# LukasHaas/PIGEON

Measured on AMD Instinct MI355X. Metric: images/sec end-to-end (ViT+head+refine), 4x336x336, higher is better.
Workload: dtype f16

## Files before the change

include/pigeon_hip.h:

```cpp
#ifndef PIGEON_HIP_H
#define PIGEON_HIP_H

#include <stddef.h>
#include <stdint.h>

#ifdef __cplusplus
extern "C" {
#endif

#define PG_OK            0
#define PG_EINVAL       -1
#define PG_ENOMEM       -2
#define PG_EHIP         -3
#define PG_ESTATE       -4

#define PG_DTYPE_F32     0
#define PG_DTYPE_BF16    1
#define PG_DTYPE_F16     2
#define PG_DTYPE_F64     3

#define PG_ABI_VERSION   7

const char* pg_last_error(void);
int pg_abi_version(void);
int pg_device_count(void);

typedef struct pg_vit pg_vit;

typedef struct pg_vit_cfg {
    int32_t layers;
    int32_t image_size;
    int32_t patch;
    int32_t hidden;
    int32_t heads;
    int32_t mlp;
    float   ln_eps;
    int32_t max_chunk;
    int32_t mma_dtype;
    int32_t precise;
} pg_vit_cfg;

int pg_vit_create(pg_vit** out, int device, const pg_vit_cfg* cfg);
int pg_vit_load_weight(pg_vit* h, const char* name, const void* data, int dtype,
                       const int64_t* shape, int ndim);
int pg_vit_finalize(pg_vit* h);
int pg_vit_workspace_bytes(const pg_vit* h, int n_images, size_t* bytes);
int pg_vit_forward(pg_vit* h, const void* pixels, int pix_dtype, int n_images, float* emb_out,
                   void* workspace, size_t workspace_bytes, void* stream);
int pg_vit_forward_hidden(pg_vit* h, const void* pixels, int pix_dtype, int n_images, float* emb_out,
                          float* hidden_out, void* workspace, size_t workspace_bytes, void* stream);
int pg_vit_precise_workspace_bytes(const pg_vit* h, int n_images, size_t* bytes);
int pg_vit_precise_plan(int n_images, int32_t out[8]);
int pg_vit_forward_precise(pg_vit* h, const void* pixels, int pix_dtype, int n_images, float* emb_out, float* hidden_out,
                           void* workspace, size_t workspace_bytes, void* stream);
int pg_vit_graph(pg_vit* h, int on, int64_t* replays, int64_t* captures);
int pg_vit_destroy(pg_vit* h);
int pg_vit_mma_dtype(const pg_vit* h);

int pg_fingerprint(const void* data, size_t bytes, uint64_t seed, uint64_t out[2], void* stream);
int pg_vit_fingerprint(const pg_vit* h, uint64_t out[2]);

#define PG_PROF_CLASSES 9
int pg_vit_profile_enable(pg_vit* h, int on);
int pg_vit_profile_read(pg_vit* h, int64_t* launches , double* ms );
int pg_vit_profile_reset(pg_vit* h);

int pg_tune_gemm_stagger(float fraction);
int pg_tune_gemm_tail_rows(int rows);
int pg_tune_gemm_tail_shape(int min_k, int min_n);
int pg_tune_gemm_raster(int gn);
int pg_tune_gemm_mid(int on);
int pg_gemm_plan(int variant, int epi, int M, int N, int K, int* kernel, int* rows_main, int* rest);
int pg_tune_exact_attention(int use_f32_mfma);
int pg_tune_exact_products(int n);
int pg_tune_exact_fusion(int on);
int pg_vit_saturation_check(pg_vit* h, int on);
int pg_vit_saturation_read(pg_vit* h, int64_t* count, int reset);
int pg_vit_range_alarm_read(pg_vit* h, int64_t* rows, int reset);

int pg_head_forward(const float* emb, int B, int P, const float* W, const float* bias,
                    const double* centroids, int C, int k, float* logits,
                    float* topk_val, int64_t* topk_idx, int64_t* argmax, double* pred_llh, void* stream);

int pg_head_margin(const float* logits, int B, int C, const float* emb, int P, const float* W, float* margin, float* sens,
                   int64_t* top2, void* stream);

int pg_head_certainty(const float* logits, int B, int C, const float* emb, int P, const float* W, const int64_t* topk_idx, int kx,
                      const float* beta, const float* wstats, float* tol, int32_t* code, float* margin, float* sens, void* stream);

int pg_aux_heads_forward(const float* emb, int B, int P, const float* W, const float* bias, int n_reg, int n_climate, int n_month,
                         const float* beta, float* preds, int64_t* cls, float* tol, int32_t* code, float* row_tol, void* stream);

typedef struct pg_bank {
    const float*   proto_emb;
    const int64_t* cell_off;
    const float*   proto_lnglat;
    const int32_t* proto_count;
    const int64_t* member_off;
    const int64_t* member_idx;
    const float*   train_emb;
    const float*   train_lnglat;
    int64_t num_cells;
    int64_t num_protos;
    int64_t num_train;
} pg_bank;

int pg_refine_forward(const pg_bank* bank, const float* q, int B, int P, const double* init_llh,
                      const int64_t* cand, const float* cand_prob, int k, int topk,
                      float temperature, double max_refine_km, float* scratch,
                      float* out_llh, int64_t* out_cell, int32_t* out_choice, void* stream);

int pg_refine_forward_ex(const pg_bank* bank, const float* q, int B, int P, const double* init_llh,
                         const int64_t* cand, const float* cand_prob, int k, int topk, int n_eval,
                         float temperature, double max_refine_km, float* scratch12,
                         float* out_llh, int64_t* out_cell, int32_t* out_choice, int32_t* out_refined, void* stream);

int pg_refine_certainty(const pg_bank* bank, const float* q, int B, int P, const int64_t* cand, const float* cand_prob, int k,
                        int topk, int n_eval, const float* scratch12, const float* W, int C, const float* beta,
                        const float* wstats, float temperature, const int32_t* refined, const int32_t* choice,
                        float* tol, int32_t* code, void* stream);

int pg_requeue_append(const float* head_tol, const float* refine_tol, const int32_t* refine_code, int B, float thr, int force_all,
                      int64_t dst_base, int64_t flushed, int64_t cap, int64_t* counters, int64_t* slot_dst, int32_t* row_slot,
                      uint8_t* certain, int32_t* cause, void* stream);
int pg_rows_to_slots(const void* src, int64_t row_bytes, const int32_t* row_slot, int B, void* dst, void* stream);
int pg_requeue_take(const int64_t* slot_dst, int64_t cap, int64_t head, int n_valid, int n_pad, int64_t* dst_out, void* stream);
int pg_scatter_rows(const void* src, int64_t row_bytes, const int64_t* dst_row, int n, void* dst, int64_t dst_rows,
                    int64_t remap_wb, int64_t remap_b, int64_t remap_off, void* stream);
int pg_head_wstats(const float* W, int C, const float* beta, float* out2, void* stream);

int pg_embedding_debias(float* emb, int64_t n, int dim, const float* bias, void* stream);

typedef struct pg_prep pg_prep;
int pg_prep_create(pg_prep** out, int device, int in_h, int in_w);
int pg_prep_destroy(pg_prep* h);
int pg_prep_geometry(const pg_prep* h, int32_t* out6);
int pg_prep_workspace_bytes(const pg_prep* h, int n_images, size_t* bytes);
int pg_prep_forward(pg_prep* h, const void* images_u8, int n_images, void* out, int out_dtype, void* workspace,
                    size_t workspace_bytes, void* stream);

#define PG_PREP_ITEM_BYTES 80
#define PG_PREP_RAGGED_MAX_IMAGES 65535
typedef struct pg_prep_item {
    uint64_t src_off;
    int32_t in_h, in_w;
    int32_t new_h, new_w, top, left;
    int32_t ksize_h, ksize_v;
    int32_t row0, nrows;
    int32_t tmp_row;
    uint32_t bounds_h_off, kk_h_off, bounds_v_off, kk_v_off;
    int32_t reserved[3];
} pg_prep_item;
int pg_prep_ragged_plan(int n, const int32_t* hw, pg_prep_item* items_out, size_t* packed_bytes, size_t* workspace_bytes);
typedef struct pg_prep_ragged pg_prep_ragged;
int pg_prep_ragged_create(pg_prep_ragged** out, int device);
int pg_prep_ragged_destroy(pg_prep_ragged* h);
int pg_prep_ragged_forward(pg_prep_ragged* h, const void* packed_dev, size_t packed_bytes, const pg_prep_item* items_host, int n,
                           void* out, int out_dtype, void* workspace, size_t workspace_bytes, void* stream);

#define PG_COMM_ID_BYTES 128
int pg_comm_unique_id(void* id_out );
int pg_comm_init_rank(void** comm, int nranks, const void* unique_id , int rank);
int pg_comm_count(void* comm, int* nranks);
int pg_allgather(void* comm, const void* send, void* recv, size_t bytes_per_rank, void* stream);
int pg_allgather_many(void* comm, int count, const void* const* send, void* const* recv, const size_t* bytes_per_rank,
                      void* stream);
int pg_comm_destroy(void* comm);
int pg_comm_rccl_version(void);

int pg_proto_build(const float* train_emb, int panels, int64_t num_train, const int64_t* member_off,
                   const int64_t* member_idx, int64_t num_protos, float* proto_emb, void* stream);
int pg_haversine_matrix(const void* x, int x_dtype, const double* y, int N, int M, double* out, void* stream);
int pg_haversine_pairs(const double* x, const void* y, int y_dtype, int64_t N, double* out, void* stream);
int pg_smooth_labels(const double* distances, int N, int M, double constant, double* out, void* stream);

int pg_haversine_blocks(const double* pts, const int64_t* cell_off, const int64_t* mat_off, int C, double zero_as, double* out,
                        void* stream);
int pg_optics_graph(const double* dist, const int64_t* cell_off, const int64_t* mat_off, int C, int min_samples, int64_t* ordering,
                    double* core, double* reach, int64_t* pred, void* stream);
int pg_optics_plan(int64_t n, int min_samples, int32_t out[4]);
int pg_tune_optics_lds_points(int max_points);

int pg_op_gemm16(int dtype, const void* A, int64_t lda, const void* W, const float* bias, void* out, int64_t ldc,
                 int M, int N, int K, int epi, float qscale, int qcols, const float* aux,
                 int variant, void* stream);
int pg_op_gemm16_ld(int dtype, const void* A, int64_t lda, const void* W, int64_t ldw, const float* bias, void* out,
                    int64_t ldc, int M, int N, int K, int epi, float qscale, int qcols, const float* aux,
                    int variant, void* stream);
int pg_op_rowstat_cast(const float* x, void* x16, int dtype, float* rowstat, int64_t rows, float eps, void* stream);
int pg_op_gemm16_resid_stat(int dtype, const void* A, int64_t lda, const void* W, int64_t ldw, const float* bias, float* X,
                            int64_t ldc, void* x16, int64_t ldx, float* statpart, int M, int N, int K, int variant, void* stream);
int pg_op_rowstat_finalize(const float* statpart, int slots, float* rowstat, int64_t rows, float eps, void* stream);
int pg_op_gemm16_ln(int dtype, const void* A, int64_t lda, const void* W, int64_t ldw, const float* bias, const float* colsum,
                    const float* rowstat, void* out, int64_t ldc, int M, int N, int K, int epi, float qscale, int qcols,
                    int variant, void* stream);
int pg_op_layernorm(const float* x, const float* gamma, const float* beta, void* y, int out_dtype,
                    int64_t rows, float eps, void* stream);
int pg_op_attention(int dtype, const void* qkv, void* out, int n_images, void* stream);
int pg_op_im2col(const void* pixels, int pix_dtype, void* out, int out_dtype, int n_images, void* stream);
int pg_op_token_mean(const float* x, float* out, int n_images, void* stream);
int pg_op_cast_f32(const float* x, void* y, int out_dtype, int64_t n, void* stream);
int pg_op_preln(float* x, const float* cls, const float* pos0, const float* gamma, const float* beta, int64_t rows, float eps,
                void* x16, int x16_dtype, float* rowstat, void* stream);
int pg_op_gemm16_parts(int dtype, const void* A, int64_t lda, const void* W, int64_t ldw, const float* bias, float* parts,
                       int M, int N, int Kp, int S, void* stream);
int pg_op_x3_split(const float* x, void* y3, int64_t rows, int cols, int gelu, void* stream);
int pg_op_x3_layernorm(const float* x, const float* gamma, const float* beta, void* y3, int64_t rows, float eps, void* stream);
int pg_op_attention_f32(const float* qkv, float* out, int n_images, void* stream);
int pg_op_attention_x3(const float* qkv, void* out3, int n_images, void* stream);
int pg_op_x3_im2col(const void* pixels, int pix_dtype, void* out3, int n_images, void* stream);
int pg_op_sum_parts(const float* parts, int S, int64_t part_elems, float* dst, int64_t n, int resid, void* stream);

#ifdef __cplusplus
}
#endif
#endif
```

pigeon_amd/_lib.py:

```python
from __future__ import annotations

import ctypes as C
import os

_HERE = os.path.dirname(os.path.abspath(__file__))
LIB_PATH = os.environ.get("PIGEON_HIP_LIB") or os.path.join(_HERE, "libpigeon_hip.so")

PG_DTYPE_F32, PG_DTYPE_BF16, PG_DTYPE_F16, PG_DTYPE_F64 = 0, 1, 2, 3
EPI_QKV, EPI_GELU, EPI_RESID, EPI_PATCH, EPI_F32, EPI_RESID_STAT, EPI_QKV_LN, EPI_GELU_LN, EPI_GELU_X3 = 0, 1, 2, 3, 4, 5, 6, 7, 8
PROF_CLASSES = ["gemm_qkv", "gemm_out", "gemm_fc1", "gemm_fc2", "gemm_patch", "attention", "layernorm",
                "im2col", "token_mean"]


class PigeonHipError(RuntimeError):
    pass


class VitCfg(C.Structure):
    _fields_ = [("layers", C.c_int32), ("image_size", C.c_int32), ("patch", C.c_int32), ("hidden", C.c_int32),
                ("heads", C.c_int32), ("mlp", C.c_int32), ("ln_eps", C.c_float), ("max_chunk", C.c_int32),
                ("mma_dtype", C.c_int32), ("precise", C.c_int32)]


class Bank(C.Structure):
    _fields_ = [("proto_emb", C.c_void_p), ("cell_off", C.c_void_p), ("proto_lnglat", C.c_void_p),
                ("proto_count", C.c_void_p), ("member_off", C.c_void_p), ("member_idx", C.c_void_p),
                ("train_emb", C.c_void_p), ("train_lnglat", C.c_void_p),
                ("num_cells", C.c_int64), ("num_protos", C.c_int64), ("num_train", C.c_int64)]


class PrepItem(C.Structure):
    _fields_ = [("src_off", C.c_uint64), ("in_h", C.c_int32), ("in_w", C.c_int32), ("new_h", C.c_int32), ("new_w", C.c_int32),
                ("top", C.c_int32), ("left", C.c_int32), ("ksize_h", C.c_int32), ("ksize_v", C.c_int32), ("row0", C.c_int32),
                ("nrows", C.c_int32), ("tmp_row", C.c_int32), ("bounds_h_off", C.c_uint32), ("kk_h_off", C.c_uint32),
                ("bounds_v_off", C.c_uint32), ("kk_v_off", C.c_uint32), ("reserved", C.c_int32 * 3)]


PREP_ITEM_BYTES = 80
assert C.sizeof(PrepItem) == PREP_ITEM_BYTES


_P, _I, _I64, _F, _D, _SZ = C.c_void_p, C.c_int, C.c_int64, C.c_float, C.c_double, C.c_size_t
SIGNATURES = {
    "pg_last_error": (C.c_char_p, []),
    "pg_abi_version": (_I, []),
    "pg_device_count": (_I, []),
    "pg_vit_create": (_I, [C.POINTER(_P), _I, C.POINTER(VitCfg)]),
    "pg_vit_load_weight": (_I, [_P, C.c_char_p, _P, _I, C.POINTER(_I64), _I]),
    "pg_vit_finalize": (_I, [_P]),
    "pg_vit_workspace_bytes": (_I, [_P, _I, C.POINTER(_SZ)]),
    "pg_vit_forward": (_I, [_P, _P, _I, _I, _P, _P, _SZ, _P]),
    "pg_vit_forward_hidden": (_I, [_P, _P, _I, _I, _P, _P, _P, _SZ, _P]),
    "pg_vit_precise_workspace_bytes": (_I, [_P, _I, C.POINTER(_SZ)]),
    "pg_vit_forward_precise": (_I, [_P, _P, _I, _I, _P, _P, _P, _SZ, _P]),
    "pg_vit_graph": (_I, [_P, _I, C.POINTER(_I64), C.POINTER(_I64)]),
    "pg_vit_destroy": (_I, [_P]),
    "pg_vit_mma_dtype": (_I, [_P]),
    "pg_fingerprint": (_I, [_P, _SZ, C.c_uint64, C.POINTER(C.c_uint64), _P]),
    "pg_vit_fingerprint": (_I, [_P, C.POINTER(C.c_uint64)]),
    "pg_vit_profile_enable": (_I, [_P, _I]),
    "pg_vit_profile_read": (_I, [_P, C.POINTER(_I64), C.POINTER(_D)]),
    "pg_vit_profile_reset": (_I, [_P]),
    "pg_tune_gemm_stagger": (_I, [_F]),
    "pg_tune_gemm_tail_rows": (_I, [_I]),
    "pg_tune_gemm_tail_shape": (_I, [_I, _I]),
    "pg_tune_gemm_raster": (_I, [_I]),
    "pg_tune_gemm_mid": (_I, [_I]),
    "pg_tune_exact_attention": (_I, [_I]),
    "pg_tune_exact_products": (_I, [_I]),
    "pg_tune_exact_fusion": (_I, [_I]),
    "pg_gemm_plan": (_I, [_I, _I, _I, _I, _I, _P, _P, _P]),
    "pg_vit_saturation_check": (_I, [_P, _I]),
    "pg_vit_saturation_read": (_I, [_P, C.POINTER(_I64), _I]),
    "pg_vit_range_alarm_read": (_I, [_P, C.POINTER(_I64), _I]),
    "pg_comm_unique_id": (_I, [_P]),
    "pg_comm_init_rank": (_I, [C.POINTER(_P), _I, _P, _I]),
    "pg_comm_count": (_I, [_P, C.POINTER(_I)]),
    "pg_allgather": (_I, [_P, _P, _P, _SZ, _P]),
    "pg_allgather_many": (_I, [_P, _I, C.POINTER(_P), C.POINTER(_P), C.POINTER(_SZ), _P]),
    "pg_comm_destroy": (_I, [_P]),
    "pg_comm_rccl_version": (_I, []),
    "pg_prep_create": (_I, [C.POINTER(_P), _I, _I, _I]),
    "pg_prep_destroy": (_I, [_P]),
    "pg_prep_geometry": (_I, [_P, C.POINTER(C.c_int32)]),
    "pg_prep_workspace_bytes": (_I, [_P, _I, C.POINTER(_SZ)]),
    "pg_prep_forward": (_I, [_P, _P, _I, _P, _I, _P, _SZ, _P]),
    "pg_prep_ragged_plan": (_I, [_I, C.POINTER(C.c_int32), C.POINTER(PrepItem), C.POINTER(_SZ), C.POINTER(_SZ)]),
    "pg_prep_ragged_create": (_I, [C.POINTER(_P), _I]),
    "pg_prep_ragged_destroy": (_I, [_P]),
    "pg_prep_ragged_forward": (_I, [_P, _P, _SZ, C.POINTER(PrepItem), _I, _P, _I, _P, _SZ, _P]),
    "pg_proto_build": (_I, [_P, _I, _I64, _P, _P, _I64, _P, _P]),
    "pg_haversine_matrix": (_I, [_P, _I, _P, _I, _I, _P, _P]),
    "pg_haversine_pairs": (_I, [_P, _P, _I, _I64, _P, _P]),
    "pg_smooth_labels": (_I, [_P, _I, _I, _D, _P, _P]),
    "pg_haversine_blocks": (_I, [_P, _P, _P, _I, _D, _P, _P]),
    "pg_optics_graph": (_I, [_P, _P, _P, _I, _I, _P, _P, _P, _P, _P]),
    "pg_optics_plan": (_I, [_I64, _I, C.POINTER(C.c_int32)]),
    "pg_tune_optics_lds_points": (_I, [_I]),
    "pg_head_forward": (_I, [_P, _I, _I, _P, _P, _P, _I, _I, _P, _P, _P, _P, _P, _P]),
    "pg_head_margin": (_I, [_P, _I, _I, _P, _I, _P, _P, _P, _P, _P]),
    "pg_head_certainty": (_I, [_P, _I, _I, _P, _I, _P, _P, _I, _P, _P, _P, _P, _P, _P, _P]),
    "pg_aux_heads_forward": (_I, [_P, _I, _I, _P, _P, _I, _I, _I, _P, _P, _P, _P, _P, _P, _P]),
    "pg_refine_forward": (_I, [C.POINTER(Bank), _P, _I, _I, _P, _P, _P, _I, _I, _F, _D, _P, _P, _P, _P, _P]),
    "pg_refine_forward_ex": (_I, [C.POINTER(Bank), _P, _I, _I, _P, _P, _P, _I, _I, _I, _F, _D, _P, _P, _P, _P, _P, _P]),
    "pg_refine_certainty": (_I, [C.POINTER(Bank), _P, _I, _I, _P, _P, _I, _I, _I, _P, _P, _I, _P, _P, _F, _P, _P, _P, _P, _P]),
    "pg_requeue_append": (_I, [_P, _P, _P, _I, _F, _I, _I64, _I64, _I64, _P, _P, _P, _P, _P, _P]),
    "pg_rows_to_slots": (_I, [_P, _I64, _P, _I, _P, _P]),
    "pg_requeue_take": (_I, [_P, _I64, _I64, _I, _I, _P, _P]),
    "pg_scatter_rows": (_I, [_P, _I64, _P, _I, _P, _I64, _I64, _I64, _I64, _P]),
    "pg_head_wstats": (_I, [_P, _I, _P, _P, _P]),
    "pg_embedding_debias": (_I, [_P, _I64, _I, _P, _P]),
    "pg_op_gemm16": (_I, [_I, _P, _I64, _P, _P, _P, _I64, _I, _I, _I, _I, _F, _I, _P, _I, _P]),
    "pg_op_gemm16_ld": (_I, [_I, _P, _I64, _P, _I64, _P, _P, _I64, _I, _I, _I, _I, _F, _I, _P, _I, _P]),
    "pg_op_rowstat_cast": (_I, [_P, _P, _I, _P, _I64, _F, _P]),
    "pg_op_gemm16_resid_stat": (_I, [_I, _P, _I64, _P, _I64, _P, _P, _I64, _P, _I64, _P, _I, _I, _I, _I, _P]),
    "pg_op_rowstat_finalize": (_I, [_P, _I, _P, _I64, _F, _P]),
    "pg_op_gemm16_ln": (_I, [_I, _P, _I64, _P, _I64, _P, _P, _P, _P, _I64, _I, _I, _I, _I, _F, _I, _I, _P]),
    "pg_op_layernorm": (_I, [_P, _P, _P, _P, _I, _I64, _F, _P]),
    "pg_op_attention": (_I, [_I, _P, _P, _I, _P]),
    "pg_op_im2col": (_I, [_P, _I, _P, _I, _I, _P]),
    "pg_op_token_mean": (_I, [_P, _P, _I, _P]),
    "pg_op_cast_f32": (_I, [_P, _P, _I, _I64, _P]),
    "pg_op_gemm16_parts": (_I, [_I, _P, _I64, _P, _I64, _P, _P, _I, _I, _I, _I, _P]),
    "pg_op_x3_split": (_I, [_P, _P, _I64, _I, _I, _P]),
    "pg_op_x3_layernorm": (_I, [_P, _P, _P, _P, _I64, _F, _P]),
    "pg_op_attention_f32": (_I, [_P, _P, _I, _P]),
    "pg_op_attention_x3": (_I, [_P, _P, _I, _P]),
    "pg_op_x3_im2col": (_I, [_P, _I, _P, _I, _P]),
    "pg_op_sum_parts": (_I, [_P, _I, _I64, _P, _I64, _I, _P]),
    "pg_op_preln": (_I, [_P, _P, _P, _P, _P, _I64, _F, _P, _I, _P, _P]),
    "pg_vit_precise_plan": (_I, [_I, C.POINTER(C.c_int32)]),
}

_lib = None


def load():
    global _lib
    if _lib is not None:
        return _lib
    if not os.path.exists(LIB_PATH):
        raise PigeonHipError(
            f"{LIB_PATH} not found: build it with `python -m pigeon_amd.build` (hipcc, gfx950). "
            "pigeon_amd has no CPU/PyTorch fallback for its hot path.")
    import torch
    lib = C.CDLL(LIB_PATH)
    for name, (res, args) in SIGNATURES.items():
        fn = getattr(lib, name)
        fn.restype = res
        fn.argtypes = args
    _lib = lib
    return lib


def check(rc: int, what: str = ""):
    if rc != 0:
        msg = load().pg_last_error()
        raise PigeonHipError(f"{what} failed (code {rc}): {msg.decode() if msg else ''}")


def require_gpu():
    lib = load()
    n = lib.pg_device_count()
    if n <= 0:
        raise PigeonHipError("pigeon_amd needs an AMD GPU (gfx950) visible to HIP; found none. "
                             "There is no CPU fallback for the hot path.")
    return n
```

pigeon_amd/csrc/abi.hip:

```cpp
#include "pigeon_internal.h"
#include <cstdarg>
#include <cstdio>

static thread_local char g_err[512] = "";

void pg_set_error(const char* fmt, ...) {
    va_list ap;
    va_start(ap, fmt);
    vsnprintf(g_err, sizeof(g_err), fmt, ap);
    va_end(ap);
}
int pg_check_launch(const char* what) {
    hipError_t e = hipGetLastError();
    if (e != hipSuccess) { pg_set_error("launch of %s failed: %s", what, hipGetErrorString(e)); return PG_EHIP; }
    return PG_OK;
}

extern "C" const char* pg_last_error(void) { return g_err; }
extern "C" int pg_abi_version(void) { return PG_ABI_VERSION; }
extern "C" int pg_device_count(void) {
    int n = 0;
    hipError_t e = hipGetDeviceCount(&n);
    if (e != hipSuccess) { pg_set_error("hipGetDeviceCount: %s", hipGetErrorString(e)); return PG_EHIP; }
    return n;
}

extern "C" int pg_op_gemm16(int dtype, const void* A, int64_t lda, const void* W, const float* bias, void* out, int64_t ldc,
                            int M, int N, int K, int epi, float qscale, int qcols, const float* aux, int variant,
                            void* stream) {
    if (!A || !W || !out) { pg_set_error("op_gemm16: null argument"); return PG_EINVAL; }
    return pg_gemm_launch(dtype, A, lda, W, K, bias, out, ldc, M, N, K, epi, qscale, qcols, aux, variant, (hipStream_t)stream);
}
extern "C" int pg_op_gemm16_ld(int dtype, const void* A, int64_t lda, const void* W, int64_t ldw, const float* bias, void* out,
                               int64_t ldc, int M, int N, int K, int epi, float qscale, int qcols, const float* aux,
                               int variant, void* stream) {
    if (!A || !W || !out) { pg_set_error("op_gemm16_ld: null argument"); return PG_EINVAL; }
    return pg_gemm_launch(dtype, A, lda, W, ldw, bias, out, ldc, M, N, K, epi, qscale, qcols, aux, variant, (hipStream_t)stream);
}
extern "C" int pg_op_rowstat_cast(const float* x, void* x16, int dtype, float* rowstat, int64_t rows, float eps, void* stream) {
    if (!x || !x16 || !rowstat) { pg_set_error("op_rowstat_cast: null argument"); return PG_EINVAL; }
    return pg_rowstat_cast_launch(x, x16, dtype, rowstat, rows, eps, (hipStream_t)stream);
}
extern "C" int pg_op_rowstat_finalize(const float* statpart, int slots, float* rowstat, int64_t rows, float eps, void* stream) {
    if (!statpart || !rowstat || slots <= 0) { pg_set_error("op_rowstat_finalize: bad argument"); return PG_EINVAL; }
    return pg_rowstat_finalize_launch(statpart, slots, rowstat, rows, eps, (hipStream_t)stream);
}
extern "C" int pg_op_gemm16_resid_stat(int dtype, const void* A, int64_t lda, const void* W, int64_t ldw, const float* bias, float* X,
                                       int64_t ldc, void* x16, int64_t ldx, float* statpart, int M, int N, int K, int variant,
                                       void* stream) {
    if (!A || !W || !X || !x16 || !statpart) { pg_set_error("op_gemm16_resid_stat: null argument"); return PG_EINVAL; }
    PgGemmExtra ex; ex.x16 = x16; ex.ldx = ldx; ex.statpart = statpart;
    return pg_gemm_launch(dtype, A, lda, W, ldw, bias, X, ldc, M, N, K, EPI_RESID_STAT, 1.f, 0, nullptr, variant ? variant : PG_GEMM_V_PP,
                          (hipStream_t)stream, &ex);
}
extern "C" int pg_op_gemm16_ln(int dtype, const void* A, int64_t lda, const void* W, int64_t ldw, const float* bias,
                               const float* colsum, const float* rowstat, void* out, int64_t ldc, int M, int N, int K, int epi,
                               float qscale, int qcols, int variant, void* stream) {
    if (!A || !W || !out || !colsum || !rowstat) { pg_set_error("op_gemm16_ln: null argument"); return PG_EINVAL; }
    if (epi != EPI_QKV_LN && epi != EPI_GELU_LN) { pg_set_error("op_gemm16_ln: epi must be 6 or 7"); return PG_EINVAL; }
    PgGemmExtra ex; ex.colsum = colsum; ex.rowstat = rowstat;
    return pg_gemm_launch(dtype, A, lda, W, ldw, bias, out, ldc, M, N, K, epi, qscale, qcols, nullptr, variant ? variant : PG_GEMM_V_PP,
                          (hipStream_t)stream, &ex);
}
extern "C" int pg_op_layernorm(const float* x, const float* gamma, const float* beta, void* y, int out_dtype,
                               int64_t rows, float eps, void* stream) {
    if (!x || !gamma || !beta || !y) { pg_set_error("op_layernorm: null argument"); return PG_EINVAL; }
    return pg_layernorm_launch(x, gamma, beta, y, out_dtype, rows, eps, (hipStream_t)stream);
}
extern "C" int pg_op_attention(int dtype, const void* qkv, void* out, int n_images, void* stream) {
    if (!qkv || !out) { pg_set_error("op_attention: null argument"); return PG_EINVAL; }
    return pg_attention_launch(dtype, qkv, out, n_images, (hipStream_t)stream);
}
extern "C" int pg_op_im2col(const void* pixels, int pix_dtype, void* out, int out_dtype, int n_images, void* stream) {
    if (!pixels || !out) { pg_set_error("op_im2col: null argument"); return PG_EINVAL; }
    return pg_im2col_launch(pixels, pix_dtype, out, out_dtype, n_images, (hipStream_t)stream);
}
extern "C" int pg_op_token_mean(const float* x, float* out, int n_images, void* stream) {
    if (!x || !out) { pg_set_error("op_token_mean: null argument"); return PG_EINVAL; }
    return pg_token_mean_launch(x, out, n_images, (hipStream_t)stream);
}
extern "C" int pg_op_cast_f32(const float* x, void* y, int out_dtype, int64_t n, void* stream) {
    if (!x || !y) { pg_set_error("op_cast_f32: null argument"); return PG_EINVAL; }
    return pg_cast_f32_launch(x, y, out_dtype, n, (hipStream_t)stream);
}

extern "C" int pg_op_gemm16_parts(int dtype, const void* A, int64_t lda, const void* W, int64_t ldw, const float* bias, float* parts,
                                  int M, int N, int Kp, int S, void* stream) {
    if (!A || !W || !parts) { pg_set_error("op_gemm16_parts: null argument"); return PG_EINVAL; }
    if (S < 1 || S > 8) { pg_set_error("op_gemm16_parts: 1 <= S <= 8"); return PG_EINVAL; }
    PgGemmExtra ex;
    ex.parts = S; ex.a_part = Kp; ex.w_part = Kp; ex.c_part = (int64_t)M * N;
    return pg_gemm_launch(dtype, A, lda, W, ldw, bias, parts, N, M, N, Kp, EPI_F32, 1.f, 0, nullptr, PG_GEMM_V_PP, (hipStream_t)stream, &ex);
}

extern "C" int pg_op_x3_split(const float* x, void* y3, int64_t rows, int cols, int gelu, void* stream) {
    if (!x || !y3) { pg_set_error("op_x3_split: null argument"); return PG_EINVAL; }
    return pg_x3_split_launch(x, y3, rows, cols, gelu, (hipStream_t)stream);
}
extern "C" int pg_op_x3_layernorm(const float* x, const float* gamma, const float* beta, void* y3, int64_t rows, float eps, void* stream) {
    if (!x || !gamma || !beta || !y3) { pg_set_error("op_x3_layernorm: null argument"); return PG_EINVAL; }
    return pg_x3_ln_launch(x, gamma, beta, y3, rows, eps, (hipStream_t)stream);
}
extern "C" int pg_op_attention_f32(const float* qkv, float* out, int n_images, void* stream) {
    if (!qkv || !out) { pg_set_error("op_attention_f32: null argument"); return PG_EINVAL; }
    return pg_attention_f32_launch(qkv, out, n_images, (hipStream_t)stream);
}
extern "C" int pg_op_x3_im2col(const void* pixels, int pix_dtype, void* out3, int n_images, void* stream) {
    if (!pixels || !out3 || n_images < 0) { pg_set_error("op_x3_im2col: bad argument"); return PG_EINVAL; }
    return pg_x3_im2col_launch(pixels, pix_dtype, out3, n_images, (hipStream_t)stream);
}
extern "C" int pg_op_sum_parts(const float* parts, int S, int64_t part_elems, float* dst, int64_t n, int resid, void* stream) {
    if (!parts || !dst) { pg_set_error("op_sum_parts: null argument"); return PG_EINVAL; }
    if (S < 1 || S > 8 || n < 0 || n > part_elems) { pg_set_error("op_sum_parts: 1 <= S <= 8, 0 <= n <= part_elems"); return PG_EINVAL; }
    return pg_sum_parts_launch(parts, S, part_elems, dst, n, resid, (hipStream_t)stream);
}
extern "C" int pg_op_preln(float* x, const float* cls, const float* pos0, const float* gamma, const float* beta, int64_t rows, float eps,
                           void* x16, int x16_dtype, float* rowstat, void* stream) {
    if (!x || !cls || !pos0 || !gamma || !beta) { pg_set_error("op_preln: null argument"); return PG_EINVAL; }
    if ((x16 == nullptr) != (rowstat == nullptr)) { pg_set_error("op_preln: x16 and rowstat go together"); return PG_EINVAL; }
    return pg_preln_launch(x, cls, pos0, gamma, beta, rows, eps, (hipStream_t)stream, x16, x16_dtype, rowstat);
}
extern "C" int pg_op_attention_x3(const float* qkv, void* out3, int n_images, void* stream) {
    if (!qkv || !out3) { pg_set_error("op_attention_x3: null argument"); return PG_EINVAL; }
    return pg_attention_x3out_launch(qkv, out3, n_images, (hipStream_t)stream);
}
```

pigeon_amd/csrc/gemm_device.h:

```cpp
#pragma once
#include "common.h"
#include "pigeon_internal.h"

#define BK 64
#define ROWB 128

struct GemmArgs {
    const uint16_t* A; int64_t lda;
    const uint16_t* W; int64_t ldw;
    const float* bias;
    void* out; int64_t ldc;
    int M, N, K;
    float qscale; int qcols;
    const float* aux;
    int tilesM, tilesN, ntiles;
    int part_tiles;
    int gn;
    int stagger;
    int xcd_stagger_ticks;
    PgGemmExtra ex;
};

int pg_gemm_one_tile_bn(int variant);
int pg_gemm_one_tile_launch(int dtype, GemmArgs g, int epi, int variant, hipStream_t s);
int pg_gemm_pp_launch(int dtype, GemmArgs g, int epi, int variant, hipStream_t s);
bool pg_gemm_pp6_supported(int epi, int N, int K);
int pg_gemm_pp6_launch(int dtype, GemmArgs g, int epi, hipStream_t s);
bool pg_gemm_tail_supported(int epi, int N, int K);
int pg_gemm_tail_launch(int dtype, GemmArgs g, int epi, int m_begin, hipStream_t s);
bool pg_gemm_mid_supported(int epi, int N, int K);
int pg_gemm_mid_launch(int dtype, GemmArgs g, int epi, hipStream_t s, int m_begin = 0);

constexpr bool epi_is_ln(int epi) { return epi == EPI_QKV_LN || epi == EPI_GELU_LN; }
constexpr bool epi_is_qkv(int epi) { return epi == EPI_QKV || epi == EPI_QKV_LN; }
constexpr bool epi_is_out16(int epi) { return epi == EPI_QKV || epi == EPI_GELU || epi_is_ln(epi); }
constexpr bool epi_is_resid(int epi) { return epi == EPI_RESID || epi == EPI_RESID_STAT; }

__device__ __forceinline__ void xcd_stagger_wait(int ticks) {
    if (ticks <= 0) return;
    const int xcd = blockIdx.x & 7;
    if (xcd == 0) return;
    const unsigned long long until = __builtin_amdgcn_s_memrealtime() + (unsigned long long)ticks * xcd / 8;
    while (__builtin_amdgcn_s_memrealtime() < until) __builtin_amdgcn_s_sleep(16);
}

#ifdef PIGEON_PROBES
#define PG_TS(g, iter, wave, slot)                                                                                             \
    do {                                                                                                                       \
        if ((g).stagger == -7 && (blockIdx.x == 0 || blockIdx.x == 100) && (threadIdx.x & 63) == 0 && (iter) < 16)             \
            ((unsigned long long*)(g).aux)[(((blockIdx.x ? 1 : 0) * 16 + (iter)) * 8 + (wave)) * 12 + (slot)] =                \
                __builtin_amdgcn_s_memrealtime();                                                                              \
    } while (0)
#else
#define PG_TS(g, iter, wave, slot) do {} while (0)
#endif

typedef __attribute__((address_space(3))) void lds_void;

__device__ __forceinline__ void glds16(const void* gptr, void* lds_base_uniform) {
    __builtin_amdgcn_global_load_lds((const __attribute__((address_space(1))) void*)gptr,
                                     (__attribute__((address_space(3))) void*)lds_base_uniform, 16, 0, 0);
}
__device__ __forceinline__ __amdgpu_buffer_rsrc_t make_rsrc(const void* base, uint32_t bytes) {
    return __builtin_amdgcn_make_buffer_rsrc(const_cast<void*>(base), (short)0, (int)bytes, 0x00020000);
}
__device__ __forceinline__ void dma16(__amdgpu_buffer_rsrc_t rsrc, char* lds_wave_uniform, int voff, int soff) {
    __builtin_amdgcn_raw_ptr_buffer_load_lds(rsrc, (lds_void*)lds_wave_uniform, 16, voff, soff, 0, 0);
}
__device__ __forceinline__ int wave_valid_rows(int left, int cap) {
    int rv = left; rv = rv < 0 ? 0 : (rv > cap ? cap : rv);
    rv = __builtin_amdgcn_readfirstlane(rv);
    return rv;
}

template <int OFF, typename V>
__device__ __forceinline__ void lds_read_b128(V& dst, uint32_t addr) {
    asm volatile("ds_read_b128 %0, %1 offset:%2" : "=v"(dst) : "v"(addr), "n"(OFF));
}

__device__ __forceinline__ void wait_lgkm0() {
    asm volatile("s_waitcnt lgkmcnt(0)" ::: "memory");
    __builtin_amdgcn_sched_barrier(0);
}
__device__ __forceinline__ void wait_vm0() {
    asm volatile("s_waitcnt vmcnt(0)" ::: "memory");
    __builtin_amdgcn_sched_barrier(0);
}
__device__ __forceinline__ void raw_barrier() {
    __builtin_amdgcn_sched_barrier(0);
    __builtin_amdgcn_s_barrier();
    __builtin_amdgcn_sched_barrier(0);
}
__device__ __forceinline__ void wave_lds_fence() {
    asm volatile("s_waitcnt lgkmcnt(0)" ::: "memory");
    __builtin_amdgcn_wave_barrier();
}

template <typename KFN>
static int launch_kernel(KFN kfn, bool& attr_set, size_t lds, dim3 grid, dim3 block, const GemmArgs& g, hipStream_t s,
                         const char* name, const char* attr_what) {
    if (!attr_set) {
        hipError_t e = hipFuncSetAttribute((const void*)kfn, hipFuncAttributeMaxDynamicSharedMemorySize, (int)lds);
        if (e != hipSuccess) { pg_set_error("%s: %s", attr_what, hipGetErrorString(e)); return PG_EHIP; }
        attr_set = true;
    }
    hipLaunchKernelGGL(kfn, grid, block, lds, s, g);
    return pg_check_launch(name);
}
static inline int pg_gemm_panel_check(const char* kernel, int64_t lda, int64_t ldw, int bm, int bn) {
    if ((int64_t)lda * 2 * bm >= (1ll << 31) || (int64_t)ldw * 2 * bn >= (1ll << 31)) {
        pg_set_error("%s: operand panel exceeds the 2 GB buffer-descriptor range", kernel);
        return PG_EINVAL;
    }
    return PG_OK;
}
```

pigeon_amd/csrc/gemm_plan.hip:

```cpp
#include "common.h"
#include "pigeon_internal.h"

#include "gemm_epi.h"

#include <cmath>
#include <cstdlib>
#include <type_traits>

#ifndef PG_DEFAULT_GEMM_STAGGER
#define PG_DEFAULT_GEMM_STAGGER 0.0f
#endif
#define PG_DEFAULT_GEMM_TAIL_ROWS 768
#define PG_DEFAULT_GEMM_TAIL_MIN_K 2048
#define PG_DEFAULT_GEMM_TAIL_MIN_N 4096
#ifndef PG_DEFAULT_GEMM_RESID6
#define PG_DEFAULT_GEMM_RESID6 1
#endif
#define PG_ROUTE_MAX_ROWS 40000
#ifndef PG_EXACT_MID_US_KT
#define PG_EXACT_MID_US_KT 0.6
#endif

static unsigned long long g_tune_epoch = 1;
unsigned long long pg_tune_epoch() { return g_tune_epoch; }

template <typename T>
static T env_knob(const char* name, T dflt) {
    const char* e = getenv(name);
    if (!e) return dflt;
    if constexpr (std::is_integral<T>::value) return (T)atoi(e);
    else if constexpr (std::is_floating_point<T>::value) return (T)atof(e);
    else return e;
}

int pg_default_gemm_variant() {
    static int v = -1;
    if (v < 0) {
        v = env_knob("PIGEON_GEMM_VARIANT", (int)PG_GEMM_V_PP6);
        if (v <= 0) v = PG_GEMM_V_PP6;
    }
    return v;
}
static int block_cap() {
    static int v = -1;
    if (v < 0) { v = env_knob("PIGEON_GEMM_BLOCKS", 0); if (v < 0) v = 0; }
    return v;
}
static int route_max_rows() {
    static int v = -1;
    if (v < 0) { v = env_knob("PIGEON_GEMM_ROUTE_MAX_ROWS", PG_ROUTE_MAX_ROWS); if (v < 0) v = 0; }
    return v;
}
static bool resid6_enabled(int K) {
    static int mask = -1;
    if (mask < 0) { mask = env_knob("PIGEON_GEMM_RESID6", PG_DEFAULT_GEMM_RESID6); if (mask < 0) mask = 0; }
    return (mask & (K >= 2048 ? 1 : 2)) != 0;
}
static double precise_mid_us_kt() {
    static double v = -1.0;
    if (v < 0.0) { v = env_knob("PIGEON_EXACT_MID_US", PG_EXACT_MID_US_KT); if (!(v > 0.0)) v = PG_EXACT_MID_US_KT; }
    return v;
}

static int g_raster_gn = -2;
int pg_gemm_raster_gn() {
    if (g_raster_gn == -2) { g_raster_gn = env_knob("PIGEON_GEMM_RASTER_GN", 0); if (g_raster_gn < -1) g_raster_gn = 0; }
    return g_raster_gn;
}
extern "C" int pg_tune_gemm_raster(int gn) {
    if (gn < -1 || gn > 64) { pg_set_error("tune_gemm_raster: gn must be -1 (all N tiles), 0 (default) or 1..64"); return PG_EINVAL; }
    g_raster_gn = gn; ++g_tune_epoch;
    return PG_OK;
}

static int g_tail_rows = -1, g_tail_min_k = -1, g_tail_min_n = -1;
static int env_count(const char* name, int dflt) { const int v = env_knob(name, dflt); return v < 0 ? 0 : v; }
static int tail_rows() { if (g_tail_rows < 0) g_tail_rows = env_count("PIGEON_GEMM_TAIL_ROWS", PG_DEFAULT_GEMM_TAIL_ROWS); return g_tail_rows; }
static int tail_min_k() { if (g_tail_min_k < 0) g_tail_min_k = env_count("PIGEON_GEMM_TAIL_MIN_K", PG_DEFAULT_GEMM_TAIL_MIN_K); return g_tail_min_k; }
static int tail_min_n() { if (g_tail_min_n < 0) g_tail_min_n = env_count("PIGEON_GEMM_TAIL_MIN_N", PG_DEFAULT_GEMM_TAIL_MIN_N); return g_tail_min_n; }
extern "C" int pg_tune_gemm_tail_rows(int rows) {
    if (rows < 0 || rows > (1 << 20)) { pg_set_error("tune_gemm_tail_rows: rows must be in [0, 2^20]"); return PG_EINVAL; }
    g_tail_rows = rows; ++g_tune_epoch;
    return PG_OK;
}
extern "C" int pg_tune_gemm_tail_shape(int min_k, int min_n) {
    if (min_k < 0 || min_n < 0) { pg_set_error("tune_gemm_tail_shape: negative threshold"); return PG_EINVAL; }
    g_tail_min_k = min_k; g_tail_min_n = min_n; ++g_tune_epoch;
    return PG_OK;
}

static int g_gemm_mid = -1;
static bool mid_on() {
    if (g_gemm_mid < 0) { const char* e = env_knob<const char*>("PIGEON_GEMM_MID", "1"); g_gemm_mid = e[0] == '0' ? 0 : (e[0] == '2' ? 2 : 1); }
    return g_gemm_mid != 0;
}
static bool route_pp256() { return mid_on() && g_gemm_mid != 2; }
extern "C" int pg_tune_gemm_mid(int on) {
    g_gemm_mid = on == 2 ? 2 : (on ? 1 : 0); ++g_tune_epoch;
    return PG_OK;
}

static float g_stagger = -1.f;
static float stagger_fraction() {
    if (g_stagger < 0.f) {
        g_stagger = env_knob("PIGEON_GEMM_STAGGER", PG_DEFAULT_GEMM_STAGGER);
        if (!(g_stagger >= 0.f && g_stagger <= 4.f)) g_stagger = 0.f;
    }
    return g_stagger;
}
extern "C" int pg_tune_gemm_stagger(float fraction) {
    if (!(fraction >= 0.f && fraction <= 4.f)) { pg_set_error("tune_gemm_stagger: fraction must be in [0, 4]"); return PG_EINVAL; }
    g_stagger = fraction; ++g_tune_epoch;
    return PG_OK;
}

static int num_cus() {
    static int n = 0;
    if (n == 0) {
        int dev = 0;
        hipDeviceProp_t p;
        if (hipGetDevice(&dev) == hipSuccess && hipGetDeviceProperties(&p, dev) == hipSuccess) n = p.multiProcessorCount;
        if (n <= 0) n = 256;
    }
    return n;
}
int pg_gemm_grid_cus() {
    const int ncu = num_cus(), cap = block_cap();
    return cap > 0 && cap < ncu ? cap : ncu;
}


struct PersistentFit { double ci, cf, e1_resid, e1_gelu, e1_other, e2; };
constexpr PersistentFit SMALL_PP6 = {1.6, 3.0, 7.0, 9.0, 6.0, 3.0};
constexpr PersistentFit SMALL_PP = {1.1, 1.8, 12.0, 9.0, 7.0, 6.0};
constexpr double SMALL_MID_US_KT = 0.44;
constexpr double SMALL_MID_EPI_RESID = 8.0, SMALL_MID_EPI = 5.5;
constexpr double SMALL_PP_MARGIN = 0.90;

static double gemm_model_us(int kernel, int M, int N, int K, int epi, int ncu) {
    const bool resid = epi == EPI_RESID || epi == EPI_RESID_STAT;
    const bool gelu = epi == EPI_GELU || epi == EPI_GELU_LN;
    const double kt = K / 64;
    if (kernel == PG_GK_MID) {
        const int64_t tiles = (int64_t)((M + 127) / 128) * (N / 128);
        return (double)((tiles + ncu - 1) / ncu) * (kt * SMALL_MID_US_KT + (resid ? SMALL_MID_EPI_RESID : SMALL_MID_EPI));
    }
    const PersistentFit& c = kernel == PG_GK_PP6 ? SMALL_PP6 : SMALL_PP;
    const int bm = kernel == PG_GK_PP6 ? 384 : 256;
    const double e1 = resid ? c.e1_resid : (gelu ? c.e1_gelu : c.e1_other);
    const int64_t tiles = (int64_t)((M + bm - 1) / bm) * (N / 256);
    const int64_t full = tiles / ncu;
    const double f = (double)(tiles % ncu) / (double)ncu;
    double t = 0.0;
    if (full > 0) t += kt * c.cf + e1 + (double)(full - 1) * (kt * c.cf + c.e2);
    if (f > 0.0) t += kt * (c.ci + (c.cf - c.ci) * f * f) + (full > 0 ? c.e2 : e1);
    return t;
}

constexpr double TAIL_US = 36.0;
constexpr double ROUND_US_KT_PP6 = 1.75, ROUND_US_KT_PP = 1.25;
constexpr double ROUND_EPI_PP6_RESID = 14.0, ROUND_EPI_PP6 = 9.0;
constexpr double ROUND_EPI_PP_RESID = 20.0, ROUND_EPI_PP = 8.0;
constexpr double TAIL_MID_EPI_RESID = 6.0, TAIL_MID_EPI = 5.0, TAIL_MID_LAUNCH_US = 3.0;

constexpr float STAGGER_PP6_EPI = 8.f, STAGGER_PP6_EPI_GELU = 12.f, STAGGER_PP6_US_KT = 2.44f;
constexpr float STAGGER_PP_EPI = 10.f, STAGGER_PP_EPI_RESID = 25.f, STAGGER_PP_US_KT = 1.63f;
constexpr float TICKS_PER_US = 100.f;

constexpr double EXACT_US_KT = 1.7;
constexpr double EXACT_EPI_RESID_WHOLE = 25.0, EXACT_EPI = 12.0;
constexpr double EXACT_SUM_LAUNCH_US = 4.0, EXACT_SUM_BYTES_PER_US = 4.0e6;
constexpr double EXACT_MID_EPI_RESID = 6.0, EXACT_MID_EPI = 5.0;

static int precise_parts(int M, int N, int Ktot, bool resid, const int* cand, int ncand, double* best_us_out) {
    const double ncu = (double)num_cus();
    const double tiles = (double)((M + 255) / 256) * (N / 256);
    int best = 1; double best_us = 1e30;
    for (int i = 0; i < ncand; ++i) {
        const int S = cand[i];
        if (Ktot % S || (Ktot / S) % 128) continue;
        const double rounds = ceil(S * tiles / ncu);
        const double epi = (S == 1 && resid) ? EXACT_EPI_RESID_WHOLE : EXACT_EPI;
        double us = rounds * ((Ktot / S / 64) * EXACT_US_KT + epi);
        if (S > 1) us += EXACT_SUM_LAUNCH_US + (double)(S + (resid ? 2 : 1)) * M * N * 4.0 / EXACT_SUM_BYTES_PER_US;
        if (us < best_us) { best_us = us; best = S; }
    }
    if (best_us_out) *best_us_out = best_us;
    return best;
}
int pg_gemm_precise_route(int M, int N, int Ktot, bool resid, const int* cand, int ncand) {
    double parts_us = 0.0;
    const int S = precise_parts(M, N, Ktot, resid, cand, ncand, &parts_us);
    if (mid_on() && N % 128 == 0) {
        const double rounds_m = ceil((double)((M + 127) / 128) * (N / 128) / (double)num_cus());
        const double mid_us = rounds_m * ((Ktot / 64) * precise_mid_us_kt() + (resid ? EXACT_MID_EPI_RESID : EXACT_MID_EPI));
        if (mid_us < parts_us) return 0;
    }
    return S;
}

struct GemmPlan {
    int kernel;
    int variant;
    int rows;
    int rest;
    int stagger_ticks;
};

static bool is_pp_variant(int v) { return v == 33 || v == PG_GEMM_V_PP; }
static bool use_pp6(int variant, int epi, int N, int K) {
    return variant == PG_GEMM_V_PP6 && pg_gemm_pp6_supported(epi, N, K) && (epi != EPI_RESID_STAT || resid6_enabled(K));
}

static int small_batch_route(int own, int epi, int M, int N, int K) {
    if (!(mid_on() && M <= route_max_rows() && epi != EPI_PATCH && epi >= EPI_QKV && epi <= EPI_GELU_LN)) return own;
    const int ncu = pg_gemm_grid_cus();
    const double t_own = gemm_model_us(own, M, N, K, epi, ncu);
    const double t_pp = (own == PG_GK_PP6 && route_pp256()) ? gemm_model_us(PG_GK_PP, M, N, K, epi, ncu) : 1e30;
    const double t_mid = pg_gemm_mid_supported(epi, N, K) ? gemm_model_us(PG_GK_MID, M, N, K, epi, ncu) : 1e30;
    if (t_pp < SMALL_PP_MARGIN * t_own && t_pp < SMALL_PP_MARGIN * t_mid) return PG_GK_PP;
    return t_mid < t_own ? PG_GK_MID : own;
}

static bool tail_split(int own, int epi, int M, int N, int K, GemmPlan& p) {
    const int tail_max = tail_rows();
    if (tail_max <= 0) return false;
    const bool six = own == PG_GK_PP6;
    const int bm = six ? 384 : 256;
    const int ncu = pg_gemm_grid_cus();
    const int tilesN = N / 256;
    const int64_t ntiles = (int64_t)((M + bm - 1) / bm) * tilesN;
    const int64_t rounds = ntiles / ncu;
    if (rounds < 1 || ntiles % ncu == 0) return false;
    const int64_t m_main = (rounds * ncu / tilesN) * bm;
    if (!(m_main > 0 && m_main < M && M - m_main <= tail_max)) return false;
    const bool resid = epi == EPI_RESID || epi == EPI_RESID_STAT;
    const double kt = K / 64;
    const double t_round = six ? kt * ROUND_US_KT_PP6 + (resid ? ROUND_EPI_PP6_RESID : ROUND_EPI_PP6)
                               : kt * ROUND_US_KT_PP + (resid ? ROUND_EPI_PP_RESID : ROUND_EPI_PP);
    const int64_t tiles_m = (int64_t)((M - m_main + 127) / 128) * (N / 128);
    const double t_mid = (double)((tiles_m + ncu - 1) / ncu) * (kt * SMALL_MID_US_KT + (resid ? TAIL_MID_EPI_RESID : TAIL_MID_EPI)) + TAIL_MID_LAUNCH_US;
    const bool cut = K >= tail_min_k() || N >= tail_min_n();
    const bool by_mid = cut && mid_on() && pg_gemm_mid_supported(epi, N, K) && t_mid < TAIL_US && t_mid < t_round;
    const bool by_tail = cut && !by_mid && pg_gemm_tail_supported(epi, N, K);
    if (!by_mid && !by_tail) return false;
    p.rows = (int)m_main;
    p.rest = by_mid ? PG_GK_MID : PG_GK_TAIL;
    return true;
}

static int stagger_ticks(bool six, int epi, int M, int K) {
    const float f = stagger_fraction();
    if (!(f > 0.f && M >= 256 * 64)) return 0;
    const float period_us = six ? ((epi == EPI_GELU || epi == EPI_GELU_LN ? STAGGER_PP6_EPI_GELU : STAGGER_PP6_EPI) + STAGGER_PP6_US_KT * (K / 64))
                                : ((epi == EPI_RESID || epi == EPI_RESID_STAT ? STAGGER_PP_EPI_RESID : STAGGER_PP_EPI) + STAGGER_PP_US_KT * (K / 64));
    return (int)(f * period_us * TICKS_PER_US);
}

static int gemm_plan(int variant, int epi, int M, int N, int K, GemmPlan& p) {
    if (epi < EPI_QKV || epi > EPI_GELU_X3) { pg_set_error("gemm: bad epilogue %d", epi); return PG_EINVAL; }
    if (variant == 0) variant = pg_default_gemm_variant();
    const bool six = use_pp6(variant, epi, N, K);
    const bool pp = !six && (variant == PG_GEMM_V_PP6 || is_pp_variant(variant)) && N % 256 == 0 && K % 128 == 0;
    const int own = six ? PG_GK_PP6 : PG_GK_PP;
    const int pp_variant = variant == PG_GEMM_V_PP6 ? PG_GEMM_V_PP : variant;
    p = GemmPlan{own, pp_variant, M, PG_GK_NONE, stagger_ticks(six, epi, M, K)};
    if (variant == PG_GEMM_V_MID || variant == PG_GEMM_V_TAIL) {
        const bool mid = variant == PG_GEMM_V_MID;
        if (!(mid ? pg_gemm_mid_supported(epi, N, K) : pg_gemm_tail_supported(epi, N, K))) {
            pg_set_error("gemm: variant %d (%s) does not support epi=%d N=%d K=%d", variant, mid ? "gemm_mid" : "gemm_tail", epi, N, K);
            return PG_EINVAL;
        }
        p.kernel = mid ? PG_GK_MID : PG_GK_TAIL;
        return PG_OK;
    }
    if (six || pp) {
        const int kind = small_batch_route(own, epi, M, N, K);
        if (kind != own) {
            p.kernel = kind;
            p.variant = PG_GEMM_V_PP;
            return PG_OK;
        }
        tail_split(own, epi, M, N, K, p);
        return PG_OK;
    }
    if (epi >= EPI_RESID_STAT) { pg_set_error("gemm: epilogue %d exists only in the persistent kernels (variants 33, 36, 56, N %% 256 == 0, K %% 128 == 0)", epi); return PG_EINVAL; }
    p.kernel = PG_GK_ONE_TILE;
    p.variant = (variant == PG_GEMM_V_PP6 || is_pp_variant(variant)) ? PG_GEMM_V_ONE_TILE : variant;
    const int bn = pg_gemm_one_tile_bn(p.variant);
    if (bn == 0) {
        pg_set_error("gemm: variant %d does not exist (variants: 8, 33, 36, 56, 70, 71)", p.variant);
        return PG_EINVAL;
    }
    if (N % bn != 0 || K % BK != 0) { pg_set_error("gemm: N %% %d or K %% 64 != 0 (N=%d K=%d)", bn, N, K); return PG_EINVAL; }
    return PG_OK;
}

extern "C" int pg_gemm_plan(int variant, int epi, int M, int N, int K, int* kernel, int* rows_main, int* rest) {
    if (!kernel || !rows_main || !rest || M <= 0 || N <= 0 || K <= 0) { pg_set_error("gemm_plan: bad argument"); return PG_EINVAL; }
    GemmPlan p;
    const int rc = gemm_plan(variant, epi, M, N, K, p);
    if (rc != PG_OK) return rc;
    *kernel = p.kernel; *rows_main = p.rows; *rest = p.rest;
    return PG_OK;
}

#ifdef PIGEON_PROBES
static void* g_dbg_ts = nullptr;
extern "C" int pg_dbg_timestamps(void* buf) { g_dbg_ts = buf; return PG_OK; }
#endif

static int launch_one(int kernel, int variant, int dtype, const GemmArgs& g, int epi, int m_begin, hipStream_t s) {
    switch (kernel) {
        case PG_GK_PP6: return pg_gemm_pp6_launch(dtype, g, epi, s);
        case PG_GK_PP: return pg_gemm_pp_launch(dtype, g, epi, variant, s);
        case PG_GK_MID: return pg_gemm_mid_launch(dtype, g, epi, s, m_begin);
        case PG_GK_TAIL: return pg_gemm_tail_launch(dtype, g, epi, m_begin, s);
        default: return pg_gemm_one_tile_launch(dtype, g, epi, variant, s);
    }
}

int pg_gemm_launch(int dtype, const void* A, int64_t lda, const void* W, int64_t ldw, const float* bias, void* out, int64_t ldc,
                   int M, int N, int K, int epi, float qscale, int qcols, const float* aux, int variant,
                   hipStream_t s, const PgGemmExtra* extra) {
    if (M <= 0) return PG_OK;
    GemmArgs g;
    g.A = (const uint16_t*)A; g.lda = lda; g.W = (const uint16_t*)W; g.ldw = ldw > 0 ? ldw : K; g.bias = bias; g.out = out; g.ldc = ldc;
    g.M = M; g.N = N; g.K = K; g.qscale = qscale; g.qcols = qcols; g.aux = aux;
    g.tilesM = 0; g.tilesN = 0; g.ntiles = 0; g.part_tiles = 0; g.gn = 0; g.stagger = 0; g.xcd_stagger_ticks = 0;
    if (extra) g.ex = *extra;
    if (g.ex.parts > 1) {
        if (epi != EPI_F32 || N % 256 != 0 || K % 128 != 0) { pg_set_error("gemm: parts > 1 needs EPI_F32, N %% 256 == 0, K %% 128 == 0"); return PG_EINVAL; }
        return pg_gemm_pp_launch(dtype, g, epi, PG_GEMM_V_PP, s);
    }
    if ((epi == EPI_GELU || epi == EPI_RESID || epi >= EPI_RESID_STAT) && !bias) { pg_set_error("gemm: epilogue %d needs a bias", epi); return PG_EINVAL; }
    if (epi == EPI_RESID_STAT && (!g.ex.x16 || !g.ex.statpart || g.ex.ldx != ldc)) { pg_set_error("gemm: EPI_RESID_STAT needs x16 / statpart and ldx == ldc"); return PG_EINVAL; }
    if (epi_is_ln(epi) && (!g.ex.colsum || !g.ex.rowstat)) { pg_set_error("gemm: LN epilogue needs colsum / rowstat"); return PG_EINVAL; }
    if (epi == EPI_PATCH && !aux) { pg_set_error("gemm: patch epilogue needs aux"); return PG_EINVAL; }
    if (epi == EPI_GELU_X3 && (ldc != 3 * (int64_t)N || dtype != PG_DTYPE_F16 || N % 256 != 0 || K % 128 != 0)) {
        pg_set_error("gemm: EPI_GELU_X3 writes the fp16 triple [M][3N]: ldc == 3 N, fp16 operands, N %% 256 == 0, K %% 128 == 0 (ldc=%lld N=%d K=%d)",
                     (long long)ldc, N, K);
        return PG_EINVAL;
    }
    if ((lda % 8) || (ldc % 8) || (qcols % 8) || (g.ldw % 8) || g.ldw < K) { pg_set_error("gemm: lda/ldw/ldc/qcols must be multiples of 8, ldw >= K"); return PG_EINVAL; }
    GemmPlan p;
    const int rc = gemm_plan(variant, epi, M, N, K, p);
    if (rc != PG_OK) return rc;
    g.xcd_stagger_ticks = p.stagger_ticks;
    if (g.ex.stat_rows <= 0) g.ex.stat_rows = M;
#ifdef PIGEON_PROBES
    if (g_dbg_ts && epi != EPI_PATCH) { g.aux = (const float*)g_dbg_ts; g.stagger = -7; }
#endif
    GemmArgs gm = g;
    gm.M = p.rows;
    const int rc_main = launch_one(p.kernel, p.variant, dtype, gm, epi, 0, s);
    if (rc_main != PG_OK || p.rest == PG_GK_NONE) return rc_main;
    return launch_one(p.rest, 0, dtype, g, epi, p.rows, s);
}
```

pigeon_amd/csrc/gemm_tail.hip:

```cpp
#include "gemm_epi.h"

namespace {

constexpr int TL_BM = 32, TL_BN = 64;
constexpr int TL_DEPTH = 8;

template <typename T> struct FragTL { typename T::v8 a[2], b[4]; };

template <typename T>
__device__ __forceinline__ void load_frag_tl(FragTL<T>& f, __amdgpu_buffer_rsrc_t ra, __amdgpu_buffer_rsrc_t rw,
                                             const int (&va)[2], const int (&vw)[4], int kbytes) {
#pragma unroll
    for (int i = 0; i < 2; ++i) f.a[i] = __builtin_bit_cast(typename T::v8, __builtin_amdgcn_raw_buffer_load_b128(ra, va[i], kbytes, 0));
#pragma unroll
    for (int j = 0; j < 4; ++j) f.b[j] = __builtin_bit_cast(typename T::v8, __builtin_amdgcn_raw_buffer_load_b128(rw, vw[j], kbytes, 0));
}

template <typename T, int EPI>
__global__ __launch_bounds__(64) void gemm_tail_kernel(GemmArgs g, int m_begin) {
    __shared__ __attribute__((aligned(16))) float slab[TL_BM * EPI_SLAB_ROWPF];
    const int lane = threadIdx.x;
    int tn, tm;
    if (g.tilesN % 8 == 0) {
        const int xcd = blockIdx.x & 7, idx = blockIdx.x >> 3, per = g.tilesN >> 3;
        tn = xcd + 8 * (idx % per); tm = idx / per;
    } else {
        tn = blockIdx.x % g.tilesN; tm = blockIdx.x / g.tilesN;
    }
    const int row0 = m_begin + tm * TL_BM, col0 = tn * TL_BN;
    const int l15 = lane & 15, lq = lane >> 4;
    const int rows = min(TL_BM, g.M - row0);
    const __amdgpu_buffer_rsrc_t ra = make_rsrc(g.A + (int64_t)row0 * g.lda, (uint32_t)rows * (uint32_t)g.lda * 2u);
    const __amdgpu_buffer_rsrc_t rw = make_rsrc(g.W + (int64_t)col0 * g.ldw, (uint32_t)TL_BN * (uint32_t)g.ldw * 2u);
    int va[2], vw[4];
#pragma unroll
    for (int i = 0; i < 2; ++i) va[i] = (i * 16 + l15) * (int)g.lda * 2 + lq * 16;
#pragma unroll
    for (int j = 0; j < 4; ++j) vw[j] = (j * 16 + l15) * (int)g.ldw * 2 + lq * 16;

    const int nks = g.K / 32;
    FragTL<T> fr[TL_DEPTH];
#pragma unroll
    for (int d = 0; d < TL_DEPTH; ++d) {
        load_frag_tl<T>(fr[d], ra, rw, va, vw, d * 64);
        __builtin_amdgcn_sched_barrier(0);
    }
    f32x4 acc[2][4];
#pragma unroll
    for (int i = 0; i < 2; ++i)
#pragma unroll
        for (int j = 0; j < 4; ++j) acc[i][j] = f32x4{0.f, 0.f, 0.f, 0.f};
    for (int ks = 0; ks < nks; ks += TL_DEPTH) {
#pragma unroll
        for (int d = 0; d < TL_DEPTH; ++d) {
#pragma unroll
            for (int i = 0; i < 2; ++i)
#pragma unroll
                for (int j = 0; j < 4; ++j) acc[i][j] = T::mfma16(fr[d].b[j], fr[d].a[i], acc[i][j]);
            const int kn = min(ks + d + TL_DEPTH, nks - 1);
            load_frag_tl<T>(fr[d], ra, rw, va, vw, kn * 64);
            __builtin_amdgcn_sched_barrier(0);
        }
    }

    constexpr bool OUT16 = epi_is_out16(EPI);
    constexpr bool LN = epi_is_ln(EPI);
    constexpr bool STAT = (EPI == EPI_RESID_STAT);
    constexpr bool RESID = epi_is_resid(EPI);
#pragma unroll
    for (int ib = 0; ib < 2; ++ib)
#pragma unroll
        for (int j = 0; j < 4; ++j) *(f32x4*)(slab + (ib * 16 + l15) * EPI_SLAB_ROWPF + j * 16 + 4 * lq) = acc[ib][j];
    wave_lds_fence();

    constexpr int HOFF = STAT ? 32 : 4;
    const int rr = lane >> 3, cc = STAT ? (lane & 7) * 4 : (lane & 7) * 8;
    const int col = col0 + cc;
    const f32x4 zero4 = {0.f, 0.f, 0.f, 0.f};
    f32x4 b_lo = zero4, b_hi = zero4, s_lo = zero4, s_hi = zero4;
    if (g.bias) { b_lo = *(const f32x4*)(g.bias + col); b_hi = *(const f32x4*)(g.bias + col + HOFF); }
    if constexpr (LN) { s_lo = *(const f32x4*)(g.ex.colsum + col); s_hi = *(const f32x4*)(g.ex.colsum + col + 4); }
    const float qsc = (epi_is_qkv(EPI) && col < g.qcols) ? g.qscale : 1.f;

#pragma unroll
    for (int it = 0; it < 4; ++it) {
        const int r = it * 8 + rr;
        const int row = row0 + r;
        if (row >= g.M) continue;
        f32x4 lo = *(const f32x4*)(slab + r * EPI_SLAB_ROWPF + cc);
        f32x4 hi = *(const f32x4*)(slab + r * EPI_SLAB_ROWPF + cc + HOFF);
        if constexpr (OUT16) {
            float rstd = 0.f, mrs = 0.f;
            if constexpr (LN) {
                const u32x2 rs = *(const u32x2*)(g.ex.rowstat + (int64_t)row * 2);
                asm("v_mov_b32 %0, %1" : "=v"(rstd) : "v"(rs[0]));
                asm("v_mov_b32 %0, %1" : "=v"(mrs) : "v"(rs[1]));
            }
            *(u32x4*)((uint16_t*)g.out + (int64_t)row * g.ldc + col) =
                epi16_finish<T, EPI>(lo, hi, b_lo, b_hi, s_lo, s_hi, rstd, mrs, col0 < g.qcols, qsc);
        } else if constexpr (RESID) {
            float* p = (float*)g.out + (int64_t)row * g.ldc + col;
            const f32x4 x = epi_resid4(*(const f32x4*)p, lo, b_lo);
            const f32x4 y = epi_resid4(*(const f32x4*)(p + HOFF), hi, b_hi);
            *(f32x4*)p = x;
            *(f32x4*)(p + HOFF) = y;
            if constexpr (STAT) {
                uint16_t* p16 = (uint16_t*)g.ex.x16 + (int64_t)row * g.ldc + col;
                *(u32x2*)p16 = epi_copy16x4<T>(x);
                *(u32x2*)(p16 + HOFF) = epi_copy16x4<T>(y);
                float s1, s2;
                epi_stat8(x, y, s1, s2);
                s1 = row8_sum(s1);
                s2 = row8_sum(s2);
                if ((lane & 7) == 0) {
                    float* sp = g.ex.statpart + ((int64_t)(col0 / 64) * g.ex.stat_rows + row) * 2;
                    sp[0] = s1; sp[1] = s2;
                }
            }
        } else {
            float* p = (float*)g.out + (int64_t)row * g.ldc + col;
            *(f32x4*)p = lo + b_lo;
            *(f32x4*)(p + 4) = hi + b_hi;
        }
    }
}

template <typename T, int EPI>
int launch_tail(const GemmArgs& g, int m_begin, int nblk, hipStream_t s) {
    hipLaunchKernelGGL((gemm_tail_kernel<T, EPI>), dim3(nblk), dim3(64), 0, s, g, m_begin);
    return pg_check_launch("gemm_tail");
}

template <typename T>
int dispatch_tail(const GemmArgs& g, int epi, int m_begin, int nblk, hipStream_t s) {
    switch (epi) {
        case EPI_QKV: return launch_tail<T, EPI_QKV>(g, m_begin, nblk, s);
        case EPI_GELU: return launch_tail<T, EPI_GELU>(g, m_begin, nblk, s);
        case EPI_RESID: return launch_tail<T, EPI_RESID>(g, m_begin, nblk, s);
        case EPI_F32: return launch_tail<T, EPI_F32>(g, m_begin, nblk, s);
        case EPI_RESID_STAT: return launch_tail<T, EPI_RESID_STAT>(g, m_begin, nblk, s);
        case EPI_QKV_LN: return launch_tail<T, EPI_QKV_LN>(g, m_begin, nblk, s);
        case EPI_GELU_LN: return launch_tail<T, EPI_GELU_LN>(g, m_begin, nblk, s);
        default: pg_set_error("gemm_tail: epilogue %d not supported", epi); return PG_EINVAL;
    }
}

}

bool pg_gemm_tail_supported(int epi, int N, int K) {
    return epi != EPI_PATCH && epi >= EPI_QKV && epi <= EPI_GELU_LN && N % TL_BN == 0 && K % (32 * TL_DEPTH) == 0;
}

int pg_gemm_tail_launch(int dtype, GemmArgs g, int epi, int m_begin, hipStream_t s) {
    if (!pg_gemm_tail_supported(epi, g.N, g.K)) { pg_set_error("gemm_tail: unsupported epilogue / shape (epi=%d N=%d K=%d)", epi, g.N, g.K); return PG_EINVAL; }
    if (m_begin < 0 || m_begin >= g.M) return PG_OK;
    if (int rc = pg_gemm_panel_check("gemm_tail", g.lda, g.ldw, TL_BM, TL_BN)) return rc;
    g.tilesM = (g.M - m_begin + TL_BM - 1) / TL_BM;
    g.tilesN = g.N / TL_BN;
    g.ntiles = g.tilesM * g.tilesN;
    if (dtype == PG_DTYPE_F16) return dispatch_tail<T_F16>(g, epi, m_begin, g.ntiles, s);
    if (dtype == PG_DTYPE_BF16) return dispatch_tail<T_BF16>(g, epi, m_begin, g.ntiles, s);
    pg_set_error("gemm_tail: operand dtype must be PG_DTYPE_F16 or PG_DTYPE_BF16 (got %d)", dtype);
    return PG_EINVAL;
}
```

pigeon_amd/csrc/pigeon_internal.h:

```cpp
#pragma once
#include <hip/hip_runtime.h>
#include <stdint.h>
#include "../../include/pigeon_hip.h"

enum { EPI_QKV = 0, EPI_GELU = 1, EPI_RESID = 2, EPI_PATCH = 3, EPI_F32 = 4, EPI_RESID_STAT = 5, EPI_QKV_LN = 6, EPI_GELU_LN = 7,
       EPI_GELU_X3 = 8 };

struct PgGemmExtra {
    const float* colsum = nullptr;
    const float* rowstat = nullptr;
    void* x16 = nullptr;
    int64_t ldx = 0;
    float* statpart = nullptr;
    int64_t stat_rows = 0;
    int parts = 1;
    int64_t a_part = 0, w_part = 0, c_part = 0;
};

void pg_set_error(const char* fmt, ...) __attribute__((format(printf, 1, 2)));
int pg_check_launch(const char* what);
int pg_default_gemm_variant();
int pg_gemm_grid_cus();
int pg_gemm_raster_gn();
unsigned long long pg_tune_epoch();
int pg_gemm_precise_route(int M, int N, int Ktot, bool resid, const int* cand, int ncand);

enum { PG_GEMM_V_ONE_TILE = 8, PG_GEMM_V_PP = 36, PG_GEMM_V_PP6 = 56, PG_GEMM_V_TAIL = 70, PG_GEMM_V_MID = 71 };
enum PgGemmKernel { PG_GK_NONE = -1, PG_GK_PP6 = 0, PG_GK_PP = 1, PG_GK_MID = 2, PG_GK_TAIL = 3, PG_GK_ONE_TILE = 4 };

#define PG_HIP(call)                                                                          \
    do {                                                                                      \
        hipError_t e__ = (call);                                                              \
        if (e__ != hipSuccess) {                                                              \
            pg_set_error("%s failed: %s (%s:%d)", #call, hipGetErrorString(e__), __FILE__, __LINE__); \
            return PG_EHIP;                                                                   \
        }                                                                                     \
    } while (0)

struct PgFpBuf { const void* data; size_t bytes; uint64_t seed; };
int pg_fingerprint_many(const PgFpBuf* bufs, int n, uint64_t* out, hipStream_t stream);
void pg_fingerprint_host(const void* data, size_t bytes, uint64_t seed, uint64_t out[2]);

int pg_gemm_launch(int dtype, const void* A, int64_t lda, const void* W, int64_t ldw, const float* bias, void* out, int64_t ldc,
                   int M, int N, int K, int epi, float qscale, int qcols, const float* aux, int variant,
                   hipStream_t s, const PgGemmExtra* extra = nullptr);
int pg_layernorm_launch(const float* x, const float* gamma, const float* beta, void* y, int out_dtype,
                        int64_t rows, float eps, hipStream_t s);
int pg_preln_launch(float* x, const float* cls, const float* pos0, const float* gamma, const float* beta,
                    int64_t rows, float eps, hipStream_t s, void* x16 = nullptr, int x16_dtype = 0, float* rowstat = nullptr);
int pg_im2col_launch(const void* pixels, int pix_dtype, void* out, int out_dtype, int n_images, hipStream_t s);
int pg_token_mean_launch(const float* x, float* out, int n_images, hipStream_t s);
int pg_cast_f32_launch(const float* x, void* y, int out_dtype, int64_t n, hipStream_t s);
int pg_rowstat_cast_launch(const float* x, void* x16, int out_dtype, float* rowstat, int64_t rows, float eps, hipStream_t s);
int pg_rowstat_finalize_launch(const float* statpart, int slots, float* rowstat, int64_t rows, float eps, hipStream_t s,
                               unsigned long long* alarm = nullptr, float alarm_sumsq = 0.f);
int pg_count_sat16_launch(const void* buf, int64_t rows, int cols, int64_t ld, int dtype, unsigned long long* counter, hipStream_t s);
int pg_attention_launch(int dtype, const void* qkv, void* out, int n_images, hipStream_t s);
int pg_x3_ln_launch(const float* x, const float* gamma, const float* beta, void* y3, int64_t rows, float eps, hipStream_t s);
int pg_x3_split_launch(const float* x, void* y3, int64_t rows, int C, int gelu, hipStream_t s);
int pg_x3_im2col_launch(const void* pixels, int pix_dtype, void* out3, int n_images, hipStream_t s);
int pg_attention_f32_launch(const float* qkv, float* out, int n_images, hipStream_t s);
bool pg_attention_x3out_available();
int pg_attention_x3out_launch(const float* qkv, void* out3, int n_images, hipStream_t s);
int pg_sum_parts_launch(const float* parts, int S, int64_t part_elems, float* dst, int64_t n, int resid, hipStream_t s);
```

pigeon_amd/csrc/rowops.hip:

```cpp
#include "common.h"
#include "pigeon_internal.h"

template <int OUT>
__global__ __launch_bounds__(256) void layernorm_kernel(const float* __restrict__ x, const float* __restrict__ gamma,
                                                        const float* __restrict__ beta, void* __restrict__ y,
                                                        int64_t rows, float eps) {
    const int lane = threadIdx.x & 63;
    const int64_t row = (int64_t)blockIdx.x * 4 + (threadIdx.x >> 6);
    if (row >= rows) return;
    const float* xr = x + row * VIT_HIDDEN;
    f32x4 v[4];
#pragma unroll
    for (int i = 0; i < 4; ++i) v[i] = *(const f32x4*)(xr + i * 256 + lane * 4);
    float s = 0.f;
#pragma unroll
    for (int i = 0; i < 4; ++i) s += (v[i][0] + v[i][1]) + (v[i][2] + v[i][3]);
    const float mean = wave_sum(s) * (1.0f / VIT_HIDDEN);
    float q = 0.f;
#pragma unroll
    for (int i = 0; i < 4; ++i)
#pragma unroll
        for (int e = 0; e < 4; ++e) { const float d = v[i][e] - mean; q += d * d; }
    const float var = wave_sum(q) * (1.0f / VIT_HIDDEN);
    const float rstd = 1.0f / sqrtf(var + eps);
#pragma unroll
    for (int i = 0; i < 4; ++i) {
        const int c = i * 256 + lane * 4;
        const f32x4 g4 = *(const f32x4*)(gamma + c);
        const f32x4 b4 = *(const f32x4*)(beta + c);
        f32x4 o;
#pragma unroll
        for (int e = 0; e < 4; ++e) o[e] = (v[i][e] - mean) * rstd * g4[e] + b4[e];
        if (OUT != 0) {
            u32x2 pk;
            if (OUT == 1) { pk[0] = pack16x2<T_BF16>(o[0], o[1]); pk[1] = pack16x2<T_BF16>(o[2], o[3]); }
            else { pk[0] = pack16x2<T_F16>(o[0], o[1]); pk[1] = pack16x2<T_F16>(o[2], o[3]); }
            *(u32x2*)((uint16_t*)y + row * VIT_HIDDEN + c) = pk;
        } else {
            *(f32x4*)((float*)y + row * VIT_HIDDEN + c) = o;
        }
    }
}

int pg_layernorm_launch(const float* x, const float* gamma, const float* beta, void* y, int out_dtype,
                        int64_t rows, float eps, hipStream_t s) {
    if (rows <= 0) return PG_OK;
    dim3 grid((unsigned)((rows + 3) / 4)), block(256);
    if (out_dtype == PG_DTYPE_BF16) hipLaunchKernelGGL(layernorm_kernel<1>, grid, block, 0, s, x, gamma, beta, y, rows, eps);
    else if (out_dtype == PG_DTYPE_F16) hipLaunchKernelGGL(layernorm_kernel<2>, grid, block, 0, s, x, gamma, beta, y, rows, eps);
    else if (out_dtype == PG_DTYPE_F32) hipLaunchKernelGGL(layernorm_kernel<0>, grid, block, 0, s, x, gamma, beta, y, rows, eps);
    else { pg_set_error("layernorm: bad output dtype %d", out_dtype); return PG_EINVAL; }
    return pg_check_launch("layernorm");
}

template <typename T, bool STAT>
__global__ __launch_bounds__(256) void preln_kernel(float* __restrict__ x, const float* __restrict__ cls,
                                                    const float* __restrict__ pos0, const float* __restrict__ gamma,
                                                    const float* __restrict__ beta, int64_t rows, float eps,
                                                    uint16_t* __restrict__ x16, float* __restrict__ rowstat) {
    const int lane = threadIdx.x & 63;
    const int64_t row = (int64_t)blockIdx.x * 4 + (threadIdx.x >> 6);
    if (row >= rows) return;
    const bool is_cls = (row % VIT_TOKENS) == 0;
    float* xr = x + row * VIT_HIDDEN;
    f32x4 v[4];
#pragma unroll
    for (int i = 0; i < 4; ++i) {
        const int c = i * 256 + lane * 4;
        if (is_cls) v[i] = *(const f32x4*)(cls + c) + *(const f32x4*)(pos0 + c);
        else v[i] = *(const f32x4*)(xr + c);
    }
    float s = 0.f;
#pragma unroll
    for (int i = 0; i < 4; ++i) s += (v[i][0] + v[i][1]) + (v[i][2] + v[i][3]);
    const float mean = wave_sum(s) * (1.0f / VIT_HIDDEN);
    float q = 0.f;
#pragma unroll
    for (int i = 0; i < 4; ++i)
#pragma unroll
        for (int e = 0; e < 4; ++e) { const float d = v[i][e] - mean; q += d * d; }
    const float rstd = 1.0f / sqrtf(wave_sum(q) * (1.0f / VIT_HIDDEN) + eps);
#pragma unroll
    for (int i = 0; i < 4; ++i) {
        const int c = i * 256 + lane * 4;
        const f32x4 g4 = *(const f32x4*)(gamma + c);
        const f32x4 b4 = *(const f32x4*)(beta + c);
        f32x4 o;
#pragma unroll
        for (int e = 0; e < 4; ++e) o[e] = (v[i][e] - mean) * rstd * g4[e] + b4[e];
        *(f32x4*)(xr + c) = o;
        v[i] = o;
    }
    if (STAT) {
        float s2 = 0.f;
#pragma unroll
        for (int i = 0; i < 4; ++i) s2 += (v[i][0] + v[i][1]) + (v[i][2] + v[i][3]);
        const float mean2 = wave_sum(s2) * (1.0f / VIT_HIDDEN);
        float q2 = 0.f;
#pragma unroll
        for (int i = 0; i < 4; ++i)
#pragma unroll
            for (int e = 0; e < 4; ++e) { const float d = v[i][e] - mean2; q2 += d * d; }
        const float rstd2 = 1.0f / sqrtf(wave_sum(q2) * (1.0f / VIT_HIDDEN) + eps);
#pragma unroll
        for (int i = 0; i < 4; ++i) {
            u32x2 pk;
            pk[0] = pack16x2<T>(v[i][0], v[i][1]); pk[1] = pack16x2<T>(v[i][2], v[i][3]);
            *(u32x2*)(x16 + row * VIT_HIDDEN + i * 256 + lane * 4) = pk;
        }
        if (lane == 0) { rowstat[2 * row] = rstd2; rowstat[2 * row + 1] = mean2 * rstd2; }
    }
}

int pg_preln_launch(float* x, const float* cls, const float* pos0, const float* gamma, const float* beta,
                    int64_t rows, float eps, hipStream_t s, void* x16, int x16_dtype, float* rowstat) {
    if (rows <= 0) return PG_OK;
    dim3 grid((unsigned)((rows + 3) / 4)), block(256);
    if (!x16) hipLaunchKernelGGL((preln_kernel<T_F16, false>), grid, block, 0, s, x, cls, pos0, gamma, beta, rows, eps, nullptr, nullptr);
    else if (!rowstat) { pg_set_error("pre_layernorm: x16 without rowstat"); return PG_EINVAL; }
    else if (x16_dtype == PG_DTYPE_F16) hipLaunchKernelGGL((preln_kernel<T_F16, true>), grid, block, 0, s, x, cls, pos0, gamma, beta, rows, eps, (uint16_t*)x16, rowstat);
    else if (x16_dtype == PG_DTYPE_BF16) hipLaunchKernelGGL((preln_kernel<T_BF16, true>), grid, block, 0, s, x, cls, pos0, gamma, beta, rows, eps, (uint16_t*)x16, rowstat);
    else { pg_set_error("pre_layernorm: bad 16-bit dtype %d", x16_dtype); return PG_EINVAL; }
    return pg_check_launch("pre_layernorm");
}

template <typename T>
__global__ __launch_bounds__(256) void rowstat_cast_kernel(const float* __restrict__ x, uint16_t* __restrict__ x16,
                                                           float* __restrict__ rowstat, int64_t rows, float eps) {
    const int lane = threadIdx.x & 63;
    const int64_t row = (int64_t)blockIdx.x * 4 + (threadIdx.x >> 6);
    if (row >= rows) return;
    const float* xr = x + row * VIT_HIDDEN;
    f32x4 v[4];
#pragma unroll
    for (int i = 0; i < 4; ++i) v[i] = *(const f32x4*)(xr + i * 256 + lane * 4);
    float s = 0.f;
#pragma unroll
    for (int i = 0; i < 4; ++i) s += (v[i][0] + v[i][1]) + (v[i][2] + v[i][3]);
    const float mean = wave_sum(s) * (1.0f / VIT_HIDDEN);
    float q = 0.f;
#pragma unroll
    for (int i = 0; i < 4; ++i)
#pragma unroll
        for (int e = 0; e < 4; ++e) { const float d = v[i][e] - mean; q += d * d; }
    const float rstd = 1.0f / sqrtf(wave_sum(q) * (1.0f / VIT_HIDDEN) + eps);
#pragma unroll
    for (int i = 0; i < 4; ++i) {
        u32x2 pk;
        pk[0] = pack16x2<T>(v[i][0], v[i][1]); pk[1] = pack16x2<T>(v[i][2], v[i][3]);
        *(u32x2*)(x16 + row * VIT_HIDDEN + i * 256 + lane * 4) = pk;
    }
    if (lane == 0) { rowstat[2 * row] = rstd; rowstat[2 * row + 1] = mean * rstd; }
}

int pg_rowstat_cast_launch(const float* x, void* x16, int out_dtype, float* rowstat, int64_t rows, float eps, hipStream_t s) {
    if (rows <= 0) return PG_OK;
    dim3 grid((unsigned)((rows + 3) / 4)), block(256);
    if (out_dtype == PG_DTYPE_F16) hipLaunchKernelGGL(rowstat_cast_kernel<T_F16>, grid, block, 0, s, x, (uint16_t*)x16, rowstat, rows, eps);
    else if (out_dtype == PG_DTYPE_BF16) hipLaunchKernelGGL(rowstat_cast_kernel<T_BF16>, grid, block, 0, s, x, (uint16_t*)x16, rowstat, rows, eps);
    else { pg_set_error("rowstat_cast: bad dtype %d", out_dtype); return PG_EINVAL; }
    return pg_check_launch("rowstat_cast");
}

__global__ __launch_bounds__(256) void rowstat_finalize_kernel(const float* __restrict__ part, int slots, float* __restrict__ rowstat,
                                                               int64_t rows, float eps, unsigned long long* __restrict__ alarm,
                                                               float alarm_sumsq) {
    const int64_t row = (int64_t)blockIdx.x * 256 + threadIdx.x;
    if (row >= rows) return;
    float s1 = 0.f, s2 = 0.f;
    for (int i = 0; i < slots; ++i) {
        const f32x2 v = *(const f32x2*)(part + ((int64_t)i * rows + row) * 2);
        s1 += v[0]; s2 += v[1];
    }
    const float mean = s1 * (1.0f / VIT_HIDDEN);
    const float var = fmaxf(s2 * (1.0f / VIT_HIDDEN) - mean * mean, 0.f);
    const float rstd = 1.0f / sqrtf(var + eps);
    rowstat[2 * row] = rstd;
    rowstat[2 * row + 1] = mean * rstd;
    if (alarm && !(s2 < alarm_sumsq)) atomicAdd(alarm, 1ull);
}

int pg_rowstat_finalize_launch(const float* statpart, int slots, float* rowstat, int64_t rows, float eps, hipStream_t s,
                               unsigned long long* alarm, float alarm_sumsq) {
    if (rows <= 0) return PG_OK;
    hipLaunchKernelGGL(rowstat_finalize_kernel, dim3((unsigned)((rows + 255) / 256)), dim3(256), 0, s, statpart, slots, rowstat, rows, eps,
                       alarm, alarm_sumsq);
    return pg_check_launch("rowstat_finalize");
}

template <typename PIX, typename T, bool PIX_F16 = false>
__global__ __launch_bounds__(256) void im2col_kernel(const PIX* __restrict__ pix, uint16_t* __restrict__ out) {
    const int img = blockIdx.x / 24, py = blockIdx.x % 24;
    const PIX* src = pix + (int64_t)img * 3 * VIT_IMG * VIT_IMG;
    uint16_t* dst = out + ((int64_t)img * VIT_PATCHES + py * 24) * VIT_PATCH_KPAD;
    for (int idx = threadIdx.x; idx < 42 * VIT_IMG; idx += 256) {
        const int line = idx / VIT_IMG, xcol = idx - line * VIT_IMG;
        const int c = line / 14, ky = line - c * 14;
        const int px = xcol / 14, kx = xcol - px * 14;
        float v;
        if (sizeof(PIX) == 4) v = (float)src[((int64_t)c * VIT_IMG + py * 14 + ky) * VIT_IMG + xcol];
        else if (PIX_F16) v = f16_bits_to_f32((uint16_t)src[((int64_t)c * VIT_IMG + py * 14 + ky) * VIT_IMG + xcol]);
        else v = bf16_bits_to_f32((uint16_t)src[((int64_t)c * VIT_IMG + py * 14 + ky) * VIT_IMG + xcol]);
        dst[px * VIT_PATCH_KPAD + c * 196 + ky * 14 + kx] = T::bits(v);
    }
    for (int idx = threadIdx.x; idx < 24 * (VIT_PATCH_KPAD - VIT_PATCH_K); idx += 256) {
        const int px = idx / (VIT_PATCH_KPAD - VIT_PATCH_K), k = idx % (VIT_PATCH_KPAD - VIT_PATCH_K);
        dst[px * VIT_PATCH_KPAD + VIT_PATCH_K + k] = 0;
    }
}

int pg_im2col_launch(const void* pixels, int pix_dtype, void* out, int out_dtype, int n_images, hipStream_t s) {
    if (n_images <= 0) return PG_OK;
    dim3 grid(n_images * 24), block(256);
    if (out_dtype != PG_DTYPE_F16 && out_dtype != PG_DTYPE_BF16) { pg_set_error("im2col: bad output dtype %d", out_dtype); return PG_EINVAL; }
    const bool h = out_dtype == PG_DTYPE_F16;
    if (pix_dtype == PG_DTYPE_F32) {
        if (h) hipLaunchKernelGGL((im2col_kernel<float, T_F16>), grid, block, 0, s, (const float*)pixels, (uint16_t*)out);
        else hipLaunchKernelGGL((im2col_kernel<float, T_BF16>), grid, block, 0, s, (const float*)pixels, (uint16_t*)out);
    } else if (pix_dtype == PG_DTYPE_BF16) {
        if (h) hipLaunchKernelGGL((im2col_kernel<uint16_t, T_F16>), grid, block, 0, s, (const uint16_t*)pixels, (uint16_t*)out);
        else hipLaunchKernelGGL((im2col_kernel<uint16_t, T_BF16>), grid, block, 0, s, (const uint16_t*)pixels, (uint16_t*)out);
    } else if (pix_dtype == PG_DTYPE_F16) {
        if (h) hipLaunchKernelGGL((im2col_kernel<uint16_t, T_F16, true>), grid, block, 0, s, (const uint16_t*)pixels, (uint16_t*)out);
        else hipLaunchKernelGGL((im2col_kernel<uint16_t, T_BF16, true>), grid, block, 0, s, (const uint16_t*)pixels, (uint16_t*)out);
    } else { pg_set_error("im2col: unsupported pixel dtype %d", pix_dtype); return PG_EINVAL; }
    return pg_check_launch("im2col");
}

__global__ __launch_bounds__(256) void token_mean_kernel(const float* __restrict__ x, float* __restrict__ out) {
    const int img = blockIdx.x >> 2, col = (blockIdx.x & 3) * 256 + threadIdx.x;
    const float* p = x + (int64_t)img * VIT_TOKENS * VIT_HIDDEN + col;
    float s0 = 0.f, s1 = 0.f, s2 = 0.f, s3 = 0.f;
    int t = 0;
    for (; t + 16 <= VIT_TOKENS; t += 16) {
        float v[16];
#pragma unroll
        for (int i = 0; i < 16; ++i) v[i] = p[(int64_t)(t + i) * VIT_HIDDEN];
#pragma unroll
        for (int i = 0; i < 16; i += 4) { s0 += v[i]; s1 += v[i + 1]; s2 += v[i + 2]; s3 += v[i + 3]; }
    }
    for (; t + 4 <= VIT_TOKENS; t += 4) {
        s0 += p[(int64_t)(t + 0) * VIT_HIDDEN];
        s1 += p[(int64_t)(t + 1) * VIT_HIDDEN];
        s2 += p[(int64_t)(t + 2) * VIT_HIDDEN];
        s3 += p[(int64_t)(t + 3) * VIT_HIDDEN];
    }
    for (; t < VIT_TOKENS; ++t) s0 += p[(int64_t)t * VIT_HIDDEN];
    out[(int64_t)img * VIT_HIDDEN + col] = ((s0 + s1) + (s2 + s3)) / (float)VIT_TOKENS;
}

int pg_token_mean_launch(const float* x, float* out, int n_images, hipStream_t s) {
    if (n_images <= 0) return PG_OK;
    hipLaunchKernelGGL(token_mean_kernel, dim3(n_images * 4), dim3(256), 0, s, x, out);
    return pg_check_launch("token_mean");
}

template <typename T>
__global__ __launch_bounds__(256) void f32_to_16_kernel(const float* __restrict__ x, uint16_t* __restrict__ y, int64_t n) {
    int64_t i = ((int64_t)blockIdx.x * 256 + threadIdx.x) * 4;
    const int64_t stride = (int64_t)gridDim.x * 256 * 4;
    for (; i + 3 < n; i += stride) {
        const f32x4 v = *(const f32x4*)(x + i);
        u32x2 pk;
        pk[0] = pack16x2<T>(v[0], v[1]);
        pk[1] = pack16x2<T>(v[2], v[3]);
        *(u32x2*)(y + i) = pk;
    }
    if (i < n) for (int64_t j = i; j < n; ++j) y[j] = T::bits(x[j]);
}

int pg_cast_f32_launch(const float* x, void* y, int out_dtype, int64_t n, hipStream_t s) {
    if (n <= 0) return PG_OK;
    int64_t blocks = (n / 4 + 255) / 256;
    if (blocks > 4096) blocks = 4096;
    if (blocks < 1) blocks = 1;
    if (out_dtype == PG_DTYPE_F16) hipLaunchKernelGGL(f32_to_16_kernel<T_F16>, dim3((unsigned)blocks), dim3(256), 0, s, x, (uint16_t*)y, n);
    else if (out_dtype == PG_DTYPE_BF16) hipLaunchKernelGGL(f32_to_16_kernel<T_BF16>, dim3((unsigned)blocks), dim3(256), 0, s, x, (uint16_t*)y, n);
    else { pg_set_error("cast: bad output dtype %d", out_dtype); return PG_EINVAL; }
    return pg_check_launch("cast_f32");
}

__global__ __launch_bounds__(256) void count_sat16_kernel(const uint16_t* __restrict__ buf, int64_t rows, int cols, int64_t ld,
                                                          int is_f16, unsigned long long* __restrict__ counter) {
    const int64_t vec_per_row = cols / 8;
    const int64_t total = rows * vec_per_row;
    unsigned long long n = 0;
    for (int64_t i = (int64_t)blockIdx.x * 256 + threadIdx.x; i < total; i += (int64_t)gridDim.x * 256) {
        const int64_t r = i / vec_per_row, c = (i - r * vec_per_row) * 8;
        const u32x4 v = *(const u32x4*)(buf + r * ld + c);
#pragma unroll
        for (int e = 0; e < 4; ++e) {
            const uint32_t lo = v[e] & 0x7fffu, hi = (v[e] >> 16) & 0x7fffu;
            if (is_f16) { n += (lo == 0x7bffu) + (hi == 0x7bffu); }
            else { n += (lo == 0x7f80u) + (hi == 0x7f80u); }
        }
    }
#pragma unroll
    for (int o = 32; o >= 1; o >>= 1) n += __shfl_xor(n, o, 64);
    if ((threadIdx.x & 63) == 0 && n) atomicAdd(counter, n);
}

int pg_count_sat16_launch(const void* buf, int64_t rows, int cols, int64_t ld, int dtype, unsigned long long* counter, hipStream_t s) {
    if (rows <= 0 || cols <= 0) return PG_OK;
    if (cols % 8 || ld % 8) { pg_set_error("count_sat16: cols / ld must be multiples of 8"); return PG_EINVAL; }
    hipLaunchKernelGGL(count_sat16_kernel, dim3(2048), dim3(256), 0, s, (const uint16_t*)buf, rows, cols, ld,
                       dtype == PG_DTYPE_F16 ? 1 : 0, counter);
    return pg_check_launch("count_sat16");
}
```

pigeon_amd/csrc/vit.hip:

```cpp
#include "vit_handle.h"

static const float kQScale = 0.125f * 1.4426950408889634f;
static size_t ws_bytes_for(int chunk, bool ln_fold) { return fast_ws((size_t)chunk * VIT_TOKENS, ln_fold).total; }
static size_t part_ws_bytes(const pg_vit* h, int n_images, int* parts) {
    *parts = (h->streams > 1 && n_images >= 32 * h->streams) ? h->streams : 1;
    const int per = (n_images + *parts - 1) / *parts;
    const int chunk = per < h->cfg.max_chunk ? per : h->cfg.max_chunk;
    return align_up(ws_bytes_for(chunk > 0 ? chunk : 1, h->ln_fold), 256);
}
extern "C" int pg_vit_workspace_bytes(const pg_vit* h, int n_images, size_t* bytes) {
    if (!h || !bytes || n_images < 0) { pg_set_error("vit_workspace_bytes: bad argument"); return PG_EINVAL; }
    int parts = 1;
    const size_t per_part = part_ws_bytes(h, n_images, &parts);
    *bytes = (size_t)parts * per_part;
    return PG_OK;
}
#define SAT(buf, rows, cols, ld) do { if (h->sat_check) RC(pg_count_sat16_launch((buf), (rows), (cols), (ld), dt, h->sat_counter, s)); } while (0)

static int vit_forward_body(pg_vit* h, int n, char* ws, hipStream_t s) {
    const int64_t M = (int64_t)n * VIT_TOKENS;
    const FastWs w = fast_ws((size_t)M, h->ln_fold);
    float* X = (float*)(ws + w.X);
    uint16_t *Xn = (uint16_t*)(ws + w.Xn), *big = (uint16_t*)(ws + w.big);
    const float eps = h->cfg.ln_eps;
    const int dt = h->cfg.mma_dtype, D = VIT_HIDDEN, F = VIT_MLP;
    auto gemm = [&](const void* A, const uint16_t* W, const float* bias, void* out, int N, int K, int epi, const PgGemmExtra* ex = nullptr) -> int {
        const bool qkv = epi == EPI_QKV || epi == EPI_QKV_LN;
        return pg_gemm_launch(dt, A, K, W, K, bias, out, N, (int)M, N, K, epi, qkv ? kQScale : 1.f, qkv ? D : 0, nullptr, 0, s, ex);
    };
    SAT(big, (int64_t)n * VIT_PATCHES, VIT_PATCH_KPAD, VIT_PATCH_KPAD);
    { ProfScope p(h, s, PROF_GEMM_PATCH);
      RC(pg_gemm_launch(dt, big, VIT_PATCH_KPAD, h->wpatch, VIT_PATCH_KPAD, nullptr, X, VIT_HIDDEN, n * VIT_PATCHES, VIT_HIDDEN, VIT_PATCH_KPAD,
                        EPI_PATCH, 1.f, 0, h->pos, 0, s)); }
    if (!h->ln_fold) { ProfScope p(h, s, PROF_LAYERNORM); RC(pg_preln_launch(X, h->cls, h->pos, h->preg, h->preb, M, eps, s)); }
    if (h->ln_fold) {
        uint16_t* Xn2 = (uint16_t*)(ws + w.Xn2);
        float *statpart = (float*)(ws + w.statpart), *rsA = (float*)(ws + w.rsA), *rsB = (float*)(ws + w.rsB);
        const int slots = VIT_HIDDEN / 64;
        { ProfScope p(h, s, PROF_LAYERNORM); RC(pg_preln_launch(X, h->cls, h->pos, h->preg, h->preb, M, eps, s, Xn, dt, rsA)); }
        SAT(Xn, M, VIT_HIDDEN, VIT_HIDDEN);
        for (int l = 0; l < h->cfg.layers; ++l) {
            const LayerW& L = h->layers[l];
            const bool last = l + 1 == h->cfg.layers;
            PgGemmExtra ex;
            { ProfScope p(h, s, PROF_GEMM_QKV); ex = PgGemmExtra(); ex.colsum = L.sqkv; ex.rowstat = rsA;
              RC(gemm(Xn, L.wqkv, L.bqkv, big, 3 * D, D, EPI_QKV_LN, &ex)); }
            SAT(big, M, 3 * VIT_HIDDEN, 3 * VIT_HIDDEN);
            { ProfScope p(h, s, PROF_ATTENTION); RC(pg_attention_launch(dt, big, Xn, n, s)); }
            SAT(Xn, M, VIT_HIDDEN, VIT_HIDDEN);
            { ProfScope p(h, s, PROF_GEMM_OUT); ex = PgGemmExtra(); ex.x16 = Xn2; ex.ldx = VIT_HIDDEN; ex.statpart = statpart;
              RC(gemm(Xn, L.wo, L.bo, X, D, D, EPI_RESID_STAT, &ex)); }
            SAT(Xn2, M, VIT_HIDDEN, VIT_HIDDEN);
            { ProfScope p(h, s, PROF_LAYERNORM); RC(pg_rowstat_finalize_launch(statpart, slots, rsB, M, eps, s, h->range_alarm, h->range_alarm_sumsq)); }
            { ProfScope p(h, s, PROF_GEMM_FC1); ex = PgGemmExtra(); ex.colsum = L.s1; ex.rowstat = rsB;
              RC(gemm(Xn2, L.w1, L.b1, big, F, D, EPI_GELU_LN, &ex)); }
            SAT(big, M, VIT_MLP, VIT_MLP);
            { ProfScope p(h, s, PROF_GEMM_FC2);
              if (last) RC(gemm(big, L.w2, L.b2, X, D, F, EPI_RESID));
              else { ex = PgGemmExtra(); ex.x16 = Xn; ex.ldx = VIT_HIDDEN; ex.statpart = statpart;
                     RC(gemm(big, L.w2, L.b2, X, D, F, EPI_RESID_STAT, &ex)); } }
            if (!last) SAT(Xn, M, VIT_HIDDEN, VIT_HIDDEN);
            if (!last) { ProfScope p(h, s, PROF_LAYERNORM); RC(pg_rowstat_finalize_launch(statpart, slots, rsA, M, eps, s, h->range_alarm, h->range_alarm_sumsq)); }
        }
    } else
    for (int l = 0; l < h->cfg.layers; ++l) {
        const LayerW& L = h->layers[l];
        { ProfScope p(h, s, PROF_LAYERNORM); RC(pg_layernorm_launch(X, L.ln1g, L.ln1b, Xn, dt, M, eps, s)); }
        SAT(Xn, M, VIT_HIDDEN, VIT_HIDDEN);
        { ProfScope p(h, s, PROF_GEMM_QKV); RC(gemm(Xn, L.wqkv, L.bqkv, big, 3 * D, D, EPI_QKV)); }
        SAT(big, M, 3 * VIT_HIDDEN, 3 * VIT_HIDDEN);
        { ProfScope p(h, s, PROF_ATTENTION); RC(pg_attention_launch(dt, big, Xn, n, s)); }
        SAT(Xn, M, VIT_HIDDEN, VIT_HIDDEN);
        { ProfScope p(h, s, PROF_GEMM_OUT); RC(gemm(Xn, L.wo, L.bo, X, D, D, EPI_RESID)); }
        { ProfScope p(h, s, PROF_LAYERNORM); RC(pg_layernorm_launch(X, L.ln2g, L.ln2b, Xn, dt, M, eps, s)); }
        SAT(Xn, M, VIT_HIDDEN, VIT_HIDDEN);
        { ProfScope p(h, s, PROF_GEMM_FC1); RC(gemm(Xn, L.w1, L.b1, big, F, D, EPI_GELU)); }
        SAT(big, M, VIT_MLP, VIT_MLP);
        { ProfScope p(h, s, PROF_GEMM_FC2); RC(gemm(big, L.w2, L.b2, X, D, F, EPI_RESID)); }
    }
    return PG_OK;
}

void vit_graph_entry_free(pg_vit::GraphEntry& e) {
    if (e.done) { (void)hipEventSynchronize(e.done); (void)hipEventDestroy(e.done); }
    if (e.exec) (void)hipGraphExecDestroy(e.exec);
    if (e.graph) (void)hipGraphDestroy(e.graph);
    e.exec = nullptr; e.graph = nullptr; e.done = nullptr;
}
static int graph_replay(pg_vit* h, pg_vit::GraphEntry* ent, hipStream_t s) {
    PG_HIP(hipGraphLaunch(ent->exec, s));
    if (ent->done) (void)hipEventRecord(ent->done, s);
    ++h->graph_replays;
    return PG_OK;
}
static int vit_forward_body_graphed(pg_vit* h, int n, char* ws, hipStream_t s) {
    const bool ok = h->use_graph && !h->prof && !h->sat_check && h->streams == 1;
    if (!ok) return vit_forward_body(h, n, ws, s);
    pg_vit::GraphEntry* ent = nullptr;
    for (auto& e : h->graphs) if (e.ws == ws && e.n == n) { ent = &e; break; }
    if (!ent) {
        if (h->graphs.size() >= 8) {
            size_t lru = 0;
            for (size_t i = 1; i < h->graphs.size(); ++i) if (h->graphs[i].last_use < h->graphs[lru].last_use) lru = i;
            vit_graph_entry_free(h->graphs[lru]);
            h->graphs.erase(h->graphs.begin() + lru);
        }
        h->graphs.push_back({ws, n, 0, nullptr, nullptr, 0, pg_tune_epoch(), nullptr});
        ent = &h->graphs.back();
    }
    ent->last_use = ++h->graph_clock;
    if (ent->exec && ent->epoch != pg_tune_epoch()) {
        vit_graph_entry_free(*ent);
        ent->seen = 1;
    }
    if (ent->exec) return graph_replay(h, ent, s);
    if (ent->seen++ == 0) return vit_forward_body(h, n, ws, s);
    if (!h->capture_stream) PG_HIP(hipStreamCreateWithFlags(&h->capture_stream, hipStreamNonBlocking));
    hipGraph_t graph = nullptr;
    hipError_t e = hipStreamBeginCapture(h->capture_stream, hipStreamCaptureModeThreadLocal);
    if (e != hipSuccess) { (void)hipGetLastError(); h->use_graph = false; return vit_forward_body(h, n, ws, s); }
    const int rc = vit_forward_body(h, n, ws, h->capture_stream);
    e = hipStreamEndCapture(h->capture_stream, &graph);
    if (rc != PG_OK || e != hipSuccess || !graph) {
        (void)hipGetLastError();
        if (graph) (void)hipGraphDestroy(graph);
        h->use_graph = false;
        return vit_forward_body(h, n, ws, s);
    }
    hipGraphExec_t exec = nullptr;
    e = hipGraphInstantiate(&exec, graph, nullptr, nullptr, 0);
    if (e != hipSuccess || !exec) { (void)hipGetLastError(); (void)hipGraphDestroy(graph); h->use_graph = false; return vit_forward_body(h, n, ws, s); }
    ent->graph = graph; ent->exec = exec; ent->epoch = pg_tune_epoch();
    if (!ent->done) (void)hipEventCreateWithFlags(&ent->done, hipEventDisableTiming);
    ++h->graph_captures;
    return graph_replay(h, ent, s);
}

static int vit_forward_chunk(pg_vit* h, const void* pixels, int pix_dtype, int n, float* emb_out, float* hidden_out, char* ws, hipStream_t s) {
    const int64_t M = (int64_t)n * VIT_TOKENS;
    const FastWs w = fast_ws((size_t)M, h->ln_fold);
    float* X = (float*)(ws + w.X);
    uint16_t* big = (uint16_t*)(ws + w.big);
    { ProfScope p(h, s, PROF_IM2COL); RC(pg_im2col_launch(pixels, pix_dtype, big, h->cfg.mma_dtype, n, s)); }
    RC(vit_forward_body_graphed(h, n, ws, s));
    { ProfScope p(h, s, PROF_TOKEN_MEAN); RC(pg_token_mean_launch(X, emb_out, n, s)); }
    if (hidden_out) PG_HIP(hipMemcpyAsync(hidden_out, X, (size_t)M * VIT_HIDDEN * 4, hipMemcpyDeviceToDevice, s));
    return PG_OK;
}

extern "C" int pg_vit_forward_hidden(pg_vit* h, const void* pixels, int pix_dtype, int n_images, float* emb_out,
                                     float* hidden_out, void* workspace, size_t workspace_bytes, void* stream) {
    int parts = 1;
    const size_t wsp = (h && n_images > 0) ? part_ws_bytes(h, n_images, &parts) : 0;
    RC(vit_forward_check("vit_forward", h, false, pixels, pix_dtype, n_images, emb_out, workspace, workspace_bytes, (size_t)parts * wsp));
    if (n_images == 0) return PG_OK;
    hipStream_t s = (hipStream_t)stream;
    auto run_range = [&](int first, int last, char* ws, hipStream_t st) -> int {
        for (int s0 = first; s0 < last; s0 += h->cfg.max_chunk) {
            const int n = (last - s0) < h->cfg.max_chunk ? (last - s0) : h->cfg.max_chunk;
            const ChunkIO io = chunk_io(pixels, pix_dtype, emb_out, hidden_out, s0);
            RC(vit_forward_chunk(h, io.pixels, pix_dtype, n, io.emb, io.hidden, ws, st));
        }
        return PG_OK;
    };
    if (parts > 1) {
        const int per = (n_images + parts - 1) / parts;
        PG_HIP(hipEventRecord(h->ev_fork, s));
        for (int i = 0; i + 1 < parts; ++i) PG_HIP(hipStreamWaitEvent(h->sx[i], h->ev_fork, 0));
        int rc = PG_OK;
        for (int i = 0; i < parts && rc == PG_OK; ++i) {
            const int first = i * per, last = (i + 1) * per < n_images ? (i + 1) * per : n_images;
            if (first >= last) continue;
            rc = run_range(first, last, (char*)workspace + (size_t)i * wsp, i == 0 ? s : h->sx[i - 1]);
        }
        for (int i = 0; i + 1 < parts; ++i) {
            hipError_t e = hipEventRecord(h->ev_join[i], h->sx[i]);
            if (e == hipSuccess) e = hipStreamWaitEvent(s, h->ev_join[i], 0);
            if (e != hipSuccess && rc == PG_OK) { pg_set_error("vit_forward: joining side stream %d failed: %s", i, hipGetErrorString(e)); rc = PG_EHIP; }
        }
        return rc;
    }
    return run_range(0, n_images, (char*)workspace, s);
}

extern "C" int pg_vit_forward(pg_vit* h, const void* pixels, int pix_dtype, int n_images, float* emb_out, void* workspace, size_t workspace_bytes, void* stream) {
    return pg_vit_forward_hidden(h, pixels, pix_dtype, n_images, emb_out, nullptr, workspace, workspace_bytes, stream);
}

static int read_counter(pg_vit* h, unsigned long long* ptr, int reset, const char* who, int64_t* out) {
    if (!h || !out) { pg_set_error("%s: null argument", who); return PG_EINVAL; }
    *out = 0;
    if (!ptr) return PG_OK;
    int cur = 0; PG_HIP(hipGetDevice(&cur));
    PG_HIP(hipSetDevice(h->device));
    hipError_t e = hipDeviceSynchronize();
    unsigned long long v = 0;
    if (e == hipSuccess) e = hipMemcpy(&v, ptr, sizeof(v), hipMemcpyDeviceToHost);
    if (e == hipSuccess && reset) e = hipMemset(ptr, 0, sizeof(v));
    (void)hipSetDevice(cur);
    if (e != hipSuccess) { pg_set_error("%s: %s", who, hipGetErrorString(e)); return PG_EHIP; }
    *out = (int64_t)v;
    return PG_OK;
}
extern "C" int pg_vit_range_alarm_read(pg_vit* h, int64_t* rows, int reset) {
    return read_counter(h, h ? h->range_alarm : nullptr, reset, "range_alarm_read", rows);
}
extern "C" int pg_vit_saturation_check(pg_vit* h, int on) {
    if (!h) { pg_set_error("saturation_check: null handle"); return PG_EINVAL; }
    if (on && !h->sat_counter) {
        PG_HIP(hipSetDevice(h->device));
        PG_HIP(hipMalloc((void**)&h->sat_counter, sizeof(unsigned long long)));
        h->allocs.push_back(h->sat_counter);
        PG_HIP(hipMemset(h->sat_counter, 0, sizeof(unsigned long long)));
    }
    h->sat_check = on != 0;
    return PG_OK;
}
extern "C" int pg_vit_saturation_read(pg_vit* h, int64_t* count, int reset) {
    return read_counter(h, h ? h->sat_counter : nullptr, reset, "saturation_read", count);
}
extern "C" int pg_vit_graph(pg_vit* h, int on, int64_t* replays, int64_t* captures) {
    if (!h) { pg_set_error("vit_graph: null handle"); return PG_EINVAL; }
    if (on == 0 || on == 1) h->use_graph = on != 0;
    if (replays) *replays = h->graph_replays;
    if (captures) *captures = h->graph_captures;
    return PG_OK;
}

extern "C" int pg_vit_profile_enable(pg_vit* h, int on) {
    if (!h) { pg_set_error("profile_enable: null handle"); return PG_EINVAL; }
    h->prof = on != 0;
    h->prof_mask = (on == 1 || on == 0) ? 0xFFFFFFFFu : ((unsigned)on >> 1);
    return PG_OK;
}
static int prof_drain(pg_vit* h) {
    for (auto& e : h->evs) {
        PG_HIP(hipEventSynchronize(e.b));
        float ms = 0.f;
        PG_HIP(hipEventElapsedTime(&ms, e.a, e.b));
        h->prof_ms[e.cls] += ms;
        h->prof_launches[e.cls] += 1;
        (void)hipEventDestroy(e.a); (void)hipEventDestroy(e.b);
    }
    h->evs.clear();
    return PG_OK;
}
extern "C" int pg_vit_profile_read(pg_vit* h, int64_t* launches, double* ms) {
    if (!h || !launches || !ms) { pg_set_error("profile_read: null argument"); return PG_EINVAL; }
    RC(prof_drain(h));
    for (int i = 0; i < PG_PROF_CLASSES; ++i) { launches[i] = h->prof_launches[i]; ms[i] = h->prof_ms[i]; }
    return PG_OK;
}
extern "C" int pg_vit_profile_reset(pg_vit* h) {
    if (!h) { pg_set_error("profile_reset: null handle"); return PG_EINVAL; }
    RC(prof_drain(h));
    for (int i = 0; i < PG_PROF_CLASSES; ++i) { h->prof_launches[i] = 0; h->prof_ms[i] = 0; }
    return PG_OK;
}
```

pigeon_amd/csrc/vit_handle.h:

```cpp
#pragma once
#include "common.h"
#include "pigeon_internal.h"
#include <map>
#include <string>
#include <vector>

struct LayerW {
    uint16_t *wqkv = nullptr, *wo = nullptr, *w1 = nullptr, *w2 = nullptr;
    float *bqkv = nullptr, *bo = nullptr, *b1 = nullptr, *b2 = nullptr;
    float *ln1g = nullptr, *ln1b = nullptr, *ln2g = nullptr, *ln2b = nullptr;
    float *sqkv = nullptr, *s1 = nullptr;
    uint16_t *wqkv3 = nullptr, *wo3 = nullptr, *w13 = nullptr, *w23 = nullptr;
    float *bqkv_raw = nullptr, *b1_raw = nullptr;
};

struct pg_vit {
    pg_vit_cfg cfg;
    int device = 0;
    bool finalized = false;
    bool ln_fold = true;
    std::map<std::string, std::vector<float>> host;
    std::vector<void*> allocs;
    std::map<const void*, size_t> alloc_bytes;
    uint16_t* wpatch = nullptr;
    uint16_t* wpatch3 = nullptr;
    float *cls = nullptr, *pos = nullptr, *preg = nullptr, *preb = nullptr;
    std::vector<LayerW> layers;
    int streams = 1;
    hipStream_t sx[3] = {nullptr, nullptr, nullptr};
    hipEvent_t ev_fork = nullptr, ev_join[3] = {nullptr, nullptr, nullptr};
    bool sat_check = false;
    unsigned long long* sat_counter = nullptr;
    unsigned long long* range_alarm = nullptr;
    float range_alarm_sumsq = 0.f;
    struct GraphEntry { const void* ws; int n; int seen; hipGraph_t graph; hipGraphExec_t exec; unsigned long long last_use, epoch; hipEvent_t done; };
    std::vector<GraphEntry> graphs;
    bool use_graph = true;
    hipStream_t capture_stream = nullptr;
    unsigned long long graph_clock = 0;
    long long graph_replays = 0, graph_captures = 0;
    bool prof = false;
    unsigned prof_mask = 0xFFFFFFFFu;
    struct Ev { hipEvent_t a, b; int cls; };
    std::vector<Ev> evs;
    int64_t prof_launches[PG_PROF_CLASSES] = {0};
    double prof_ms[PG_PROF_CLASSES] = {0};
};

void vit_graph_entry_free(pg_vit::GraphEntry& e);
#define RC(x) do { int rc__ = (x); if (rc__) return rc__; } while (0)
static inline size_t align_up(size_t x, size_t a) { return (x + a - 1) / a * a; }

enum ProfClass { PROF_GEMM_QKV = 0, PROF_GEMM_OUT = 1, PROF_GEMM_FC1 = 2, PROF_GEMM_FC2 = 3, PROF_GEMM_PATCH = 4, PROF_ATTENTION = 5,
                 PROF_LAYERNORM = 6, PROF_IM2COL = 7, PROF_TOKEN_MEAN = 8 };
static_assert(PROF_TOKEN_MEAN + 1 == PG_PROF_CLASSES, "one name per profile class");
struct ProfScope {
    pg_vit* h; hipStream_t s; int cls; hipEvent_t a = nullptr, b = nullptr;
    ProfScope(pg_vit* h_, hipStream_t s_, ProfClass c) : h(h_), s(s_), cls(c) {
        if (h->prof && ((h->prof_mask >> c) & 1u)) { (void)hipEventCreate(&a); (void)hipEventCreate(&b); (void)hipEventRecord(a, s); }
    }
    ~ProfScope() { if (a) { (void)hipEventRecord(b, s); h->evs.push_back({a, b, cls}); } }
};
static inline size_t ws_take(size_t* at, size_t bytes) { const size_t o = *at; *at += align_up(bytes, 256); return o; }

struct FastWs {
    size_t X;
    size_t Xn;
    size_t big;
    size_t Xn2, statpart, rsA, rsB;
    size_t total;
};
static inline FastWs fast_ws(size_t M, bool ln_fold) {
    FastWs w = {}; size_t at = 0;
    w.X = ws_take(&at, M * VIT_HIDDEN * 4); w.Xn = ws_take(&at, M * VIT_HIDDEN * 2); w.big = ws_take(&at, M * VIT_MLP * 2);
    if (ln_fold) {
        w.Xn2 = ws_take(&at, M * VIT_HIDDEN * 2); w.statpart = ws_take(&at, M * (VIT_HIDDEN / 64) * 8);
        w.rsA = ws_take(&at, M * 8); w.rsB = ws_take(&at, M * 8);
    }
    w.total = at + 256;
    return w;
}
struct PreciseWs {
    size_t X;
    size_t T3;
    size_t F;
    size_t G3;
    size_t PP;
    size_t total;
};
static inline PreciseWs precise_ws(size_t M) {
    PreciseWs w = {}; size_t at = 0;
    w.X = ws_take(&at, M * VIT_HIDDEN * 4); w.T3 = ws_take(&at, M * 3 * VIT_HIDDEN * 2); w.F = ws_take(&at, M * VIT_MLP * 4);
    w.G3 = ws_take(&at, M * 3 * VIT_MLP * 2); w.PP = ws_take(&at, M * 3 * VIT_MLP * 4);
    w.total = at + 256;
    return w;
}

static inline int vit_forward_check(const char* who, const pg_vit* h, bool precise, const void* pixels, int pix_dtype, int n_images,
                                    const float* emb_out, const void* workspace, size_t workspace_bytes, size_t needb) {
    if (!h) { pg_set_error("%s: null handle", who); return PG_EINVAL; }
    if (!h->finalized) { pg_set_error("%s: handle not finalized", who); return PG_ESTATE; }
    if (precise && !h->cfg.precise) { pg_set_error("%s: the handle was created without cfg.precise (no split-weight copy)", who); return PG_ESTATE; }
    if (n_images < 0) { pg_set_error("%s: n_images = %d", who, n_images); return PG_EINVAL; }
    if (n_images == 0) return PG_OK;
    if (!pixels || !emb_out || !workspace) { pg_set_error("%s: null argument", who); return PG_EINVAL; }
    if (pix_dtype != PG_DTYPE_F32 && pix_dtype != PG_DTYPE_BF16 && pix_dtype != PG_DTYPE_F16) { pg_set_error("%s: bad pixel dtype", who); return PG_EINVAL; }
    if (workspace_bytes < needb) { pg_set_error("%s: workspace %zu < required %zu bytes", who, workspace_bytes, needb); return PG_ENOMEM; }
    if (((uintptr_t)workspace & 255) != 0) { pg_set_error("%s: workspace must be 256-byte aligned", who); return PG_EINVAL; }
    return PG_OK;
}

struct ChunkIO { const void* pixels; float *emb, *hidden; };
static inline ChunkIO chunk_io(const void* pixels, int pix_dtype, float* emb_out, float* hidden_out, int first) {
    const size_t img_bytes = (size_t)3 * VIT_IMG * VIT_IMG * (pix_dtype == PG_DTYPE_F32 ? 4 : 2);
    return {(const char*)pixels + (size_t)first * img_bytes, emb_out + (size_t)first * VIT_HIDDEN,
            hidden_out ? hidden_out + (size_t)first * VIT_TOKENS * VIT_HIDDEN : nullptr};
}
```

pigeon_amd/csrc/vit_weights.hip:

```cpp
#include "vit_handle.h"
#include <cstdlib>
#include <cstring>
#include <type_traits>
#ifndef PG_DEFAULT_VIT_STREAMS
#define PG_DEFAULT_VIT_STREAMS 1
#endif

static std::string canon(const char* name) {
    std::string s(name);
    const std::string pre = "vision_model.";
    if (s.compare(0, pre.size(), pre) == 0) s = s.substr(pre.size());
    return s;
}

extern "C" int pg_vit_create(pg_vit** out, int device, const pg_vit_cfg* cfg) {
    if (!out || !cfg) { pg_set_error("vit_create: null argument"); return PG_EINVAL; }
    if (cfg->image_size != 336 || cfg->patch != 14 || cfg->hidden != 1024 || cfg->heads != 16 || cfg->mlp != 4096 ||
        cfg->layers < 1) {
        pg_set_error("vit_create: only the ViT-L/14-336 geometry is supported (336/14/1024/16/4096, layers>=1)");
        return PG_EINVAL;
    }
    int n = 0;
    PG_HIP(hipGetDeviceCount(&n));
    if (device < 0 || device >= n) { pg_set_error("vit_create: device %d of %d", device, n); return PG_EINVAL; }
    pg_vit* h = new pg_vit();
    h->cfg = *cfg;
    if (h->cfg.ln_eps <= 0) h->cfg.ln_eps = 1e-5f;
    if (h->cfg.max_chunk <= 0) h->cfg.max_chunk = 512;
    if (h->cfg.mma_dtype == 0) {
        const char* e = getenv("PIGEON_MMA_DTYPE");
        h->cfg.mma_dtype = (e && (!strcmp(e, "bf16") || !strcmp(e, "BF16"))) ? PG_DTYPE_BF16 : PG_DTYPE_F16;
    }
    if (h->cfg.mma_dtype != PG_DTYPE_F16 && h->cfg.mma_dtype != PG_DTYPE_BF16) {
        delete h;
        pg_set_error("vit_create: mma_dtype must be 0 (default), PG_DTYPE_F16 or PG_DTYPE_BF16");
        return PG_EINVAL;
    }
    h->device = device;
    { const char* e = getenv("PIGEON_LN_FOLD"); h->ln_fold = !(e && e[0] == '0'); }
    if (pg_default_gemm_variant() < 30) h->ln_fold = false;
    h->layers.resize(cfg->layers);
    if (h->ln_fold && h->cfg.mma_dtype == PG_DTYPE_F16) {
        PG_HIP(hipSetDevice(device));
        PG_HIP(hipMalloc((void**)&h->range_alarm, sizeof(unsigned long long)));
        h->allocs.push_back(h->range_alarm);
        PG_HIP(hipMemset(h->range_alarm, 0, sizeof(unsigned long long)));
        h->range_alarm_sumsq = 65504.0f * 65504.0f;
    }
    { const char* e = getenv("PIGEON_VIT_GRAPH"); h->use_graph = !(e && e[0] == '0'); }
    { const char* e = getenv("PIGEON_VIT_STREAMS"); h->streams = e ? atoi(e) : PG_DEFAULT_VIT_STREAMS; }
    if (h->streams < 1 || h->streams > 4) h->streams = 1;
    if (h->streams > 1) {
        PG_HIP(hipSetDevice(device));
        PG_HIP(hipEventCreateWithFlags(&h->ev_fork, hipEventDisableTiming));
        for (int i = 0; i + 1 < h->streams; ++i) {
            PG_HIP(hipStreamCreateWithFlags(&h->sx[i], hipStreamNonBlocking));
            PG_HIP(hipEventCreateWithFlags(&h->ev_join[i], hipEventDisableTiming));
        }
    }
    *out = h;
    return PG_OK;
}

extern "C" int pg_vit_load_weight(pg_vit* h, const char* name, const void* data, int dtype, const int64_t* shape, int ndim) {
    if (!h || !name || !data || !shape) { pg_set_error("vit_load_weight: null argument"); return PG_EINVAL; }
    if (dtype != PG_DTYPE_F32) { pg_set_error("vit_load_weight: only fp32 host data is accepted"); return PG_EINVAL; }
    if (h->finalized) { pg_set_error("vit_load_weight: handle already finalized"); return PG_ESTATE; }
    int64_t n = 1;
    for (int i = 0; i < ndim; ++i) n *= shape[i];
    std::string key = canon(name);
    const float* f = (const float*)data;
    h->host[key] = std::vector<float>(f, f + n);
    return PG_OK;
}

static uint16_t host_bf16(float f) {
    uint32_t u;
    memcpy(&u, &f, 4);
    if ((u & 0x7fffffffu) > 0x7f800000u) return (uint16_t)((u >> 16) | 0x40);
    u += 0x7fffu + ((u >> 16) & 1u);
    return (uint16_t)(u >> 16);
}
static uint16_t host_f16(float f) {
    if (f > 65504.f) f = 65504.f;
    if (f < -65504.f) f = -65504.f;
    _Float16 h = (_Float16)f;
    uint16_t b;
    memcpy(&b, &h, 2);
    return b;
}
static uint16_t host_cvt(int dtype, float f) { return dtype == PG_DTYPE_F16 ? host_f16(f) : host_bf16(f); }
static float host_uncvt(int dtype, uint16_t b) {
    if (dtype == PG_DTYPE_F16) { _Float16 h; memcpy(&h, &b, 2); return (float)h; }
    uint32_t u = (uint32_t)b << 16; float f; memcpy(&f, &u, 4); return f;
}
static void fold_ln(int dt, const float* W, const float* b, const float* gamma, const float* beta, size_t N, size_t K,
                    std::vector<uint16_t>& w16, std::vector<float>& colsum, std::vector<float>& cbias) {
    w16.resize(N * K); colsum.resize(N); cbias.resize(N);
    for (size_t n = 0; n < N; ++n) {
        double s = 0.0, c = 0.0;
        for (size_t k = 0; k < K; ++k) {
            const uint16_t q = host_cvt(dt, W[n * K + k] * gamma[k]);
            w16[n * K + k] = q;
            s += (double)host_uncvt(dt, q);
            c += (double)beta[k] * (double)W[n * K + k];
        }
        colsum[n] = (float)s;
        cbias[n] = (float)(c + (double)b[n]);
    }
}

static void pack_x3(const float* W, size_t N, size_t K, size_t Kpad, std::vector<uint16_t>& w3) {
    w3.assign(N * 3 * Kpad, 0);
    for (size_t n = 0; n < N; ++n) {
        uint16_t* r = w3.data() + n * 3 * Kpad;
        for (size_t k = 0; k < K; ++k) {
            const float w = W[n * K + k];
            const uint16_t hb = host_f16(w);
            const float hf = host_uncvt(PG_DTYPE_F16, hb);
            r[k] = hb; r[Kpad + k] = hb;
            r[2 * Kpad + k] = host_f16((w - hf) * 256.0f);
        }
    }
}

static int need(pg_vit* h, const std::string& k, size_t n, const std::vector<float>** out) {
    auto it = h->host.find(k);
    if (it == h->host.end()) { pg_set_error("vit_finalize: missing parameter %s", k.c_str()); return PG_ESTATE; }
    if (it->second.size() != n) {
        pg_set_error("vit_finalize: parameter %s has %zu elements, expected %zu", k.c_str(), it->second.size(), n);
        return PG_EINVAL;
    }
    *out = &it->second;
    return PG_OK;
}

template <class T> static int upload(pg_vit* h, const T* src, size_t n, T** dst) {
    PG_HIP(hipMalloc((void**)dst, n * sizeof(T)));
    h->allocs.push_back(*dst);
    h->alloc_bytes[*dst] = n * sizeof(T);
    PG_HIP(hipMemcpy(*dst, src, n * sizeof(T), hipMemcpyHostToDevice));
    return PG_OK;
}
static int upload(pg_vit* h, const std::vector<uint16_t>& src, uint16_t** dst) { return upload(h, src.data(), src.size(), dst); }

template <class T> static int put(pg_vit* h, const std::string& k, size_t N, size_t K, T** dst, bool x3 = false) {
    const std::vector<float>* q;
    RC(need(h, k, N * K, &q));
    if constexpr (std::is_same<T, float>::value) {
        return upload(h, q->data(), N * K, dst);
    } else {
        std::vector<uint16_t> w(x3 ? 0 : N * K);
        if (x3) pack_x3(q->data(), N, K, K, w);
        else for (size_t i = 0; i < N * K; ++i) w[i] = host_cvt(h->cfg.mma_dtype, (*q)[i]);
        return upload(h, w, dst);
    }
}

extern "C" int pg_vit_finalize(pg_vit* h) {
    if (!h) { pg_set_error("vit_finalize: null handle"); return PG_EINVAL; }
    if (h->finalized) return PG_OK;
    PG_HIP(hipSetDevice(h->device));
    const size_t D = VIT_HIDDEN, F = VIT_MLP;
    const int dt = h->cfg.mma_dtype;
    const std::vector<float>* p;
    RC(need(h, "embeddings.patch_embedding.weight", D * VIT_PATCH_K, &p));
    {
        std::vector<uint16_t> w(D * VIT_PATCH_KPAD, 0);
        for (size_t n = 0; n < D; ++n)
            for (size_t k = 0; k < VIT_PATCH_K; ++k) w[n * VIT_PATCH_KPAD + k] = host_cvt(dt, (*p)[n * VIT_PATCH_K + k]);
        RC(upload(h, w, &h->wpatch));
        if (h->cfg.precise) { std::vector<uint16_t> w3; pack_x3(p->data(), D, VIT_PATCH_K, VIT_PATCH_KPAD, w3); RC(upload(h, w3, &h->wpatch3)); }
    }
    RC(put(h, "embeddings.class_embedding", 1, D, &h->cls));
    RC(put(h, "embeddings.position_embedding.weight", VIT_TOKENS, D, &h->pos));
    RC(put(h, "pre_layrnorm.weight", 1, D, &h->preg));
    RC(put(h, "pre_layrnorm.bias", 1, D, &h->preb));
    for (int l = 0; l < h->cfg.layers; ++l) {
        LayerW& L = h->layers[l];
        const std::string pre = "encoder.layers." + std::to_string(l) + ".";
        const std::vector<float>*wq, *wk, *wv, *bq, *bk, *bv;
        RC(need(h, pre + "self_attn.q_proj.weight", D * D, &wq)); RC(need(h, pre + "self_attn.k_proj.weight", D * D, &wk));
        RC(need(h, pre + "self_attn.v_proj.weight", D * D, &wv)); RC(need(h, pre + "self_attn.q_proj.bias", D, &bq));
        RC(need(h, pre + "self_attn.k_proj.bias", D, &bk));       RC(need(h, pre + "self_attn.v_proj.bias", D, &bv));
        const std::vector<float>*g1, *be1, *g2, *be2;
        RC(need(h, pre + "layer_norm1.weight", D, &g1)); RC(need(h, pre + "layer_norm1.bias", D, &be1));
        RC(need(h, pre + "layer_norm2.weight", D, &g2)); RC(need(h, pre + "layer_norm2.bias", D, &be2));
        {
            std::vector<float> wf(3 * D * D), b(3 * D);
            for (size_t i = 0; i < D * D; ++i) { wf[i] = (*wq)[i]; wf[D * D + i] = (*wk)[i]; wf[2 * D * D + i] = (*wv)[i]; }
            for (size_t i = 0; i < D; ++i) { b[i] = (*bq)[i]; b[D + i] = (*bk)[i]; b[2 * D + i] = (*bv)[i]; }
            if (h->cfg.precise) {
                std::vector<uint16_t> w3; pack_x3(wf.data(), 3 * D, D, D, w3);
                RC(upload(h, w3, &L.wqkv3)); RC(upload(h, b.data(), 3 * D, &L.bqkv_raw));
            }
            if (h->ln_fold) {
                std::vector<uint16_t> w; std::vector<float> cs, cb;
                fold_ln(dt, wf.data(), b.data(), g1->data(), be1->data(), 3 * D, D, w, cs, cb);
                RC(upload(h, w, &L.wqkv)); RC(upload(h, cb.data(), 3 * D, &L.bqkv)); RC(upload(h, cs.data(), 3 * D, &L.sqkv));
            } else {
// ... 76 lines not shown
```

pigeon_amd/hip_ops.py:

```python
from __future__ import annotations

import ctypes as C
from typing import Dict, Optional

import torch

from . import _lib
from ._lib import Bank, VitCfg, check, load

TOKENS, HIDDEN, MLP, PATCHES, KPAD = 577, 1024, 4096, 576, 640


def _p(t: Optional[torch.Tensor]):
    return C.c_void_p(0) if t is None else C.c_void_p(t.data_ptr())


def _stream():
    return C.c_void_p(torch.cuda.current_stream().cuda_stream)


_T16 = {torch.float16: _lib.PG_DTYPE_F16, torch.bfloat16: _lib.PG_DTYPE_BF16}
_PIXDT = {torch.float32: _lib.PG_DTYPE_F32, torch.float16: _lib.PG_DTYPE_F16, torch.bfloat16: _lib.PG_DTYPE_BF16}
_PG2T = {_lib.PG_DTYPE_F16: torch.float16, _lib.PG_DTYPE_BF16: torch.bfloat16, _lib.PG_DTYPE_F32: torch.float32}


def _dt16(t: torch.Tensor) -> int:
    if t.dtype not in _T16:
        raise _lib.PigeonHipError(f"expected a float16 or bfloat16 tensor, got {t.dtype}")
    return _T16[t.dtype]


def _dev(t: torch.Tensor, dtype=None) -> torch.Tensor:
    if not t.is_cuda:
        raise _lib.PigeonHipError("expected a device tensor")
    if dtype is not None and t.dtype != dtype:
        raise _lib.PigeonHipError(f"expected dtype {dtype}, got {t.dtype}")
    if not t.is_contiguous():
        raise _lib.PigeonHipError("expected a contiguous tensor")
    return t


def _shape(t: torch.Tensor, name: str, *dims):
    if t.dim() != len(dims) or any(d is not None and int(s) != int(d) for s, d in zip(t.shape, dims)):
        want = "(" + ",".join("*" if d is None else str(int(d)) for d in dims) + ")"
        raise _lib.PigeonHipError(f"{name} must have shape {want}, got {tuple(t.shape)}")
    return t


def gemm16(A: torch.Tensor, W: torch.Tensor, bias: Optional[torch.Tensor], out: torch.Tensor, epi: int,
           qscale: float = 1.0, qcols: int = 0, aux: Optional[torch.Tensor] = None, variant: int = 0,
           M: Optional[int] = None):
    for t in (A, W, out):
        if not t.is_cuda or t.stride(1) != 1:
            raise _lib.PigeonHipError("gemm16 expects device tensors with unit inner stride")
    if W.dtype != A.dtype:
        raise _lib.PigeonHipError("gemm16: A and W must have the same 16-bit dtype")
    M = A.shape[0] if M is None else M
    K = A.shape[1]
    N = W.shape[0]
    dst = out
    if epi == _lib.EPI_RESID:
        have = out.untyped_storage().nbytes() - out.storage_offset() * out.element_size()
        if have < (M + 384) * out.stride(0) * out.element_size():
            dst = torch.zeros((max(M, out.shape[0]) + 384, out.shape[1]), dtype=out.dtype, device=out.device)[:out.shape[0]]
            dst.copy_(out)
    check(load().pg_op_gemm16_ld(_dt16(A), _p(A), A.stride(0), _p(W), W.stride(0), _p(bias), _p(dst), dst.stride(0), M, N, K,
                                 epi, float(qscale), int(qcols), _p(aux), variant, _stream()), "pg_op_gemm16_ld")
    if dst is not out:
        out.copy_(dst)
    return out


def tune_gemm_tail_rows(rows: int) -> None:
    check(load().pg_tune_gemm_tail_rows(int(rows)), "pg_tune_gemm_tail_rows")


def tune_gemm_tail_shape(min_k: int, min_n: int) -> None:
    check(load().pg_tune_gemm_tail_shape(int(min_k), int(min_n)), "pg_tune_gemm_tail_shape")


def rowstat_cast(x: torch.Tensor, out_dtype: torch.dtype = torch.float16, eps: float = 1e-5):
    _dev(x, torch.float32)
    rows = x.numel() // HIDDEN
    x16 = torch.empty(x.shape, dtype=out_dtype, device=x.device)
    rs = torch.empty((rows, 2), dtype=torch.float32, device=x.device)
    check(load().pg_op_rowstat_cast(_p(x), _p(x16), _dt16(x16), _p(rs), rows, float(eps), _stream()), "pg_op_rowstat_cast")
    return x16, rs


def gemm16_resid_stat(A: torch.Tensor, W: torch.Tensor, bias: torch.Tensor, X: torch.Tensor, variant: int = 0):
    M, K = A.shape
    N = W.shape[0]
    x16 = torch.empty((M, N), dtype=A.dtype, device=A.device)
    part = torch.empty((N // 64, M, 2), dtype=torch.float32, device=A.device)
    have = X.untyped_storage().nbytes() - X.storage_offset() * X.element_size()
    Xr = X
    if have < (M + 384) * X.stride(0) * X.element_size():
        Xr = torch.zeros((M + 384, N), dtype=X.dtype, device=X.device)[:M]
        Xr.copy_(X)
    check(load().pg_op_gemm16_resid_stat(_dt16(A), _p(A), A.stride(0), _p(W), W.stride(0), _p(bias), _p(Xr), Xr.stride(0), _p(x16),
                                         x16.stride(0), _p(part), M, N, K, variant, _stream()), "pg_op_gemm16_resid_stat")
    if Xr is not X:
        X.copy_(Xr)
    return x16, part


def rowstat_finalize(part: torch.Tensor, eps: float = 1e-5) -> torch.Tensor:
    slots, rows = part.shape[0], part.shape[1]
    rs = torch.empty((rows, 2), dtype=torch.float32, device=part.device)
    check(load().pg_op_rowstat_finalize(_p(part), slots, _p(rs), rows, float(eps), _stream()), "pg_op_rowstat_finalize")
    return rs


def gemm16_ln(A: torch.Tensor, W: torch.Tensor, bias: torch.Tensor, colsum: torch.Tensor, rowstat: torch.Tensor, epi: int,
              qscale: float = 1.0, qcols: int = 0, variant: int = 0) -> torch.Tensor:
    M, K = A.shape
    N = W.shape[0]
    out = torch.empty((M, N), dtype=A.dtype, device=A.device)
    check(load().pg_op_gemm16_ln(_dt16(A), _p(A), A.stride(0), _p(W), W.stride(0), _p(bias), _p(colsum), _p(rowstat), _p(out),
                                 out.stride(0), M, N, K, epi, float(qscale), int(qcols), variant, _stream()), "pg_op_gemm16_ln")
    return out


def layernorm(x: torch.Tensor, gamma: torch.Tensor, beta: torch.Tensor, eps: float = 1e-5,
              out_dtype: torch.dtype = torch.float16, out: Optional[torch.Tensor] = None) -> torch.Tensor:
    _dev(x, torch.float32)
    rows = x.numel() // HIDDEN
    if out is None:
        out = torch.empty(x.shape, dtype=out_dtype, device=x.device)
    pg = _lib.PG_DTYPE_F32 if out.dtype == torch.float32 else _dt16(out)
    check(load().pg_op_layernorm(_p(x), _p(gamma), _p(beta), _p(out), pg, rows, float(eps), _stream()), "pg_op_layernorm")
    return out


def attention(qkv: torch.Tensor, n_images: int) -> torch.Tensor:
    _dev(qkv)
    out = torch.empty((n_images * TOKENS, HIDDEN), dtype=qkv.dtype, device=qkv.device)
    check(load().pg_op_attention(_dt16(qkv), _p(qkv), _p(out), n_images, _stream()), "pg_op_attention")
    return out


def im2col(pixels: torch.Tensor, out_dtype: torch.dtype = torch.float16) -> torch.Tensor:
    _dev(pixels)
    n = pixels.shape[0]
    dt = _PIXDT[pixels.dtype]
    out = torch.empty((n * PATCHES, KPAD), dtype=out_dtype, device=pixels.device)
    check(load().pg_op_im2col(_p(pixels), dt, _p(out), _dt16(out), n, _stream()), "pg_op_im2col")
    return out


def token_mean(x: torch.Tensor) -> torch.Tensor:
    _dev(x, torch.float32)
    n = x.shape[0]
    out = torch.empty((n, HIDDEN), dtype=torch.float32, device=x.device)
    check(load().pg_op_token_mean(_p(x), _p(out), n, _stream()), "pg_op_token_mean")
    return out


def cast_f32(x: torch.Tensor, out_dtype: torch.dtype = torch.float16) -> torch.Tensor:
    _dev(x, torch.float32)
    y = torch.empty(x.shape, dtype=out_dtype, device=x.device)
    check(load().pg_op_cast_f32(_p(x), _p(y), _dt16(y), x.numel(), _stream()), "pg_op_cast_f32")
    return y


def proto_build(train_emb: torch.Tensor, member_off: torch.Tensor, member_idx: torch.Tensor) -> torch.Tensor:
    _dev(train_emb, torch.float32); _dev(member_off, torch.int64); _dev(member_idx, torch.int64)
    if train_emb.dim() not in (2, 3) or train_emb.shape[-1] != HIDDEN:
        raise _lib.PigeonHipError(f"proto_build: embeddings must be (Ntr,{HIDDEN}) or (Ntr,panels,{HIDDEN}), got {tuple(train_emb.shape)}")
    panels = 1 if train_emb.dim() == 2 else int(train_emb.shape[1])
    if member_off.dim() != 1 or member_off.numel() < 1 or member_idx.dim() != 1:
        raise _lib.PigeonHipError("proto_build: member_off (P+1,) and member_idx (n,) expected")
    P = member_off.numel() - 1
    off = member_off.cpu()
    if int(off[0]) != 0 or int(off[-1]) != member_idx.numel() or bool((off[1:] < off[:-1]).any()):
        raise _lib.PigeonHipError("proto_build: member_off must rise from 0 to len(member_idx)")
    if member_idx.numel() and (int(member_idx.min()) < 0 or int(member_idx.max()) >= train_emb.shape[0]):
        raise _lib.PigeonHipError(f"proto_build: member index outside the {train_emb.shape[0]} training rows")
    out = torch.empty((P, HIDDEN), dtype=torch.float32, device=train_emb.device)
    check(load().pg_proto_build(_p(train_emb), panels, train_emb.shape[0], _p(member_off), _p(member_idx), P, _p(out),
                                _stream()), "pg_proto_build")
    return out


def haversine_matrix(x: torch.Tensor, y_rows: torch.Tensor) -> torch.Tensor:
    _dev(x); _dev(y_rows, torch.float64)
    if x.dtype not in (torch.float32, torch.float64):
        raise _lib.PigeonHipError("haversine_matrix: x must be fp32 or fp64")
    _shape(x, "x", None, 2); _shape(y_rows, "y_rows", None, 2)
    N, M = x.shape[0], y_rows.shape[0]
    out = torch.empty((N, M), dtype=torch.float64, device=x.device)
    check(load().pg_haversine_matrix(_p(x), _lib.PG_DTYPE_F64 if x.dtype == torch.float64 else _lib.PG_DTYPE_F32, _p(y_rows),
                                     N, M, _p(out), _stream()), "pg_haversine_matrix")
    return out


def haversine_pairs(x: torch.Tensor, y: torch.Tensor) -> torch.Tensor:
    _dev(x, torch.float64); _dev(y)
    if y.dtype not in (torch.float32, torch.float64) or x.shape != y.shape or x.dim() != 2 or x.shape[1] != 2:
        raise _lib.PigeonHipError("haversine_pairs: x (N,2) fp64 and y (N,2) fp32/fp64 expected")
    out = torch.empty((x.shape[0],), dtype=torch.float64, device=x.device)
    check(load().pg_haversine_pairs(_p(x), _p(y), _lib.PG_DTYPE_F64 if y.dtype == torch.float64 else _lib.PG_DTYPE_F32,
                                    x.shape[0], _p(out), _stream()), "pg_haversine_pairs")
    return out


def smooth_labels(distances: torch.Tensor, constant: float) -> torch.Tensor:
    _dev(distances, torch.float64)
    _shape(distances, "distances", None, None)
    N, M = distances.shape
    out = torch.empty_like(distances)
    check(load().pg_smooth_labels(_p(distances), N, M, float(constant), _p(out), _stream()), "pg_smooth_labels")
    return out


def _cell_tables(who: str, cell_off: torch.Tensor, mat_off: Optional[torch.Tensor]):
    if cell_off.dtype != torch.int64 or cell_off.dim() != 1 or cell_off.numel() < 1:
        raise _lib.PigeonHipError(f"{who}: cell_off must be an int64 vector of C + 1 entries")
    off = cell_off.cpu().contiguous()
    n = off[1:] - off[:-1]
    if int(off[0]) != 0 or bool((n < 0).any()):
        raise _lib.PigeonHipError(f"{who}: cell_off must rise from 0")
    if mat_off is None:
        mo = torch.zeros_like(off)
        torch.cumsum(n * n, 0, out=mo[1:])
    else:
        if mat_off.dtype != torch.int64 or mat_off.shape != cell_off.shape:
            raise _lib.PigeonHipError(f"{who}: mat_off must be an int64 vector as long as cell_off")
        mo = mat_off.cpu().contiguous()
        if int(mo[0]) < 0 or bool(((mo[1:] - mo[:-1]) < n * n).any()):
            raise _lib.PigeonHipError(f"{who}: mat_off must leave every cell room for its n x n matrix")
    return off, mo


def haversine_blocks(pts: torch.Tensor, cell_off: torch.Tensor, zero_as: float = 1e-5):
    _dev(pts, torch.float64)
    _shape(pts, "pts", None, 2)
    off, mo = _cell_tables("haversine_blocks", cell_off, None)
    if int(off[-1]) != pts.shape[0]:
        raise _lib.PigeonHipError(f"haversine_blocks: cell_off ends at {int(off[-1])}, pts has {pts.shape[0]} rows")
    out = torch.empty((int(mo[-1]),), dtype=torch.float64, device=pts.device)
    check(load().pg_haversine_blocks(_p(pts), _p(off), _p(mo), off.numel() - 1, float(zero_as), _p(out), _stream()),
          "pg_haversine_blocks")
    return out, mo


def optics_graph(dist: torch.Tensor, cell_off: torch.Tensor, mat_off: torch.Tensor, min_samples: int) -> Dict[str, torch.Tensor]:
    _dev(dist, torch.float64)
    if dist.dim() != 1:
        raise _lib.PigeonHipError(f"optics_graph: dist must be the flat packed matrices, got shape {tuple(dist.shape)}")
    off, mo = _cell_tables("optics_graph", cell_off, mat_off)
    if int(mo[-1]) > dist.numel():
        raise _lib.PigeonHipError(f"optics_graph: mat_off ends at {int(mo[-1])}, dist has {dist.numel()} elements")
    min_samples = int(min_samples)
    n = off[1:] - off[:-1]
    if min_samples < 2:
        raise _lib.PigeonHipError(f"optics_graph: min_samples must be at least 2 (got {min_samples})")
# ... 101 lines not shown
        if packed_u8.dim() != 1 or packed_u8.numel() != plan.packed_bytes:
            raise _lib.PigeonHipError(f"packed buffer must be 1-D uint8 of {plan.packed_bytes} bytes, got {tuple(packed_u8.shape)}")
        if packed_u8.device.index != self.device:
            raise _lib.PigeonHipError(f"packed buffer is on {packed_u8.device}, the preprocessor on cuda:{self.device}")
        if out_dtype not in (torch.float32, torch.float16):
            raise _lib.PigeonHipError("preprocess output dtype must be float32 or float16")
        out = torch.empty((plan.n, 3, 336, 336), dtype=out_dtype, device=packed_u8.device)
        if plan.n == 0:
            return out
        if self._ws is None or self._ws.numel() < plan.workspace_bytes:
            self._ws = torch.empty(plan.workspace_bytes, dtype=torch.uint8, device=packed_u8.device)
        if not header_written:
            packed_u8[:plan.header_bytes].copy_(torch.from_numpy(plan.header().copy()))
        check(load().pg_prep_ragged_forward(self._h, _p(packed_u8), plan.packed_bytes, plan.items, plan.n, _p(out), _PIXDT[out_dtype],
                                            _p(self._ws), self._ws.numel(), _stream()), "pg_prep_ragged_forward")
        return out

    __call__ = forward

    def close(self):
        if self._h:
            load().pg_prep_ragged_destroy(self._h)
            self._h = C.c_void_p()

    def __del__(self):
        try:
            self.close()
        except Exception:
            pass


class VitEncoder:

    def __init__(self, state_dict: Dict[str, torch.Tensor], device: int = 0, max_chunk: int = 0,
                 layers: Optional[int] = None, mma_dtype: Optional[str] = None, precise: bool = False):
        _lib.require_gpu()
        lib = load()
        keys = [k[len("vision_model."):] if k.startswith("vision_model.") else k for k in state_dict]
        if layers is None:
            layers = 0
            while f"encoder.layers.{layers}.layer_norm1.weight" in keys:
                layers += 1
        if layers < 1:
            raise _lib.PigeonHipError("state dict holds no encoder layers")
        self.layers = layers
        self.device = device
        pgdt = {None: 0, "f16": _lib.PG_DTYPE_F16, "fp16": _lib.PG_DTYPE_F16, "bf16": _lib.PG_DTYPE_BF16}[mma_dtype]
        cfg = VitCfg(layers, 336, 14, 1024, 16, 4096, 1e-5, max_chunk, pgdt, 1 if precise else 0)
        self.precise = bool(precise)
        self._ws_precise = None
        h = C.c_void_p()
        torch.cuda.set_device(device)
        check(lib.pg_vit_create(C.byref(h), device, C.byref(cfg)), "pg_vit_create")
        self._h = h
        for name, t in state_dict.items():
            if not torch.is_tensor(t) or not t.is_floating_point():
                continue
            a = t.detach().to("cpu", torch.float32).contiguous()
            shape = (C.c_int64 * max(a.dim(), 1))(*(list(a.shape) or [1]))
            check(lib.pg_vit_load_weight(h, name.encode(), C.c_void_p(a.data_ptr()), _lib.PG_DTYPE_F32, shape,
                                         max(a.dim(), 1)), f"pg_vit_load_weight({name})")
        check(lib.pg_vit_finalize(h), "pg_vit_finalize")
        self.mma_dtype = {_lib.PG_DTYPE_F16: "f16", _lib.PG_DTYPE_BF16: "bf16"}[lib.pg_vit_mma_dtype(h)]
        self._ws = None
        self.max_chunk = max_chunk if max_chunk > 0 else 512

    def _workspace(self, n: int) -> torch.Tensor:
        need = C.c_size_t()
        check(load().pg_vit_workspace_bytes(self._h, n, C.byref(need)), "pg_vit_workspace_bytes")
        if self._ws is None or self._ws.numel() < need.value:
            self._ws = None
            self._ws = torch.empty(need.value + 256, dtype=torch.uint8, device=f"cuda:{self.device}")
        return self._ws

    def forward(self, pixels: torch.Tensor, return_hidden: bool = False):
        _dev(pixels)
        if pixels.dim() != 4 or tuple(pixels.shape[1:]) != (3, 336, 336):
            raise _lib.PigeonHipError(f"pixels must be (N,3,336,336), got {tuple(pixels.shape)}")
        if pixels.dtype not in _PIXDT:
            raise _lib.PigeonHipError("pixels must be fp32, fp16 or bf16")
        n = pixels.shape[0]
        ws = self._workspace(n)
        off = (-ws.data_ptr()) % 256
        emb = torch.empty((n, HIDDEN), dtype=torch.float32, device=pixels.device)
        hid = torch.empty((n, TOKENS, HIDDEN), dtype=torch.float32, device=pixels.device) if return_hidden else None
        dt = _PIXDT[pixels.dtype]
        check(load().pg_vit_forward_hidden(self._h, _p(pixels), dt, n, _p(emb), _p(hid),
                                           C.c_void_p(ws.data_ptr() + off), ws.numel() - off, _stream()),
              "pg_vit_forward")
        return (emb, hid) if return_hidden else emb

    __call__ = forward

    def forward_precise(self, pixels: torch.Tensor, return_hidden: bool = False, out: Optional[torch.Tensor] = None):
        if not self.precise:
            raise _lib.PigeonHipError("forward_precise: the encoder was built without precise=True (no split-weight copy)")
        _dev(pixels)
        if pixels.dim() != 4 or tuple(pixels.shape[1:]) != (3, 336, 336):
            raise _lib.PigeonHipError(f"pixels must be (N,3,336,336), got {tuple(pixels.shape)}")
        if pixels.dtype not in _PIXDT:
            raise _lib.PigeonHipError("pixels must be fp32, fp16 or bf16")
        n = pixels.shape[0]
        need = C.c_size_t()
        check(load().pg_vit_precise_workspace_bytes(self._h, n, C.byref(need)), "pg_vit_precise_workspace_bytes")
        if self._ws_precise is None or self._ws_precise.numel() < need.value + 256:
            self._ws_precise = None
            self._ws_precise = torch.empty(need.value + 256, dtype=torch.uint8, device=f"cuda:{self.device}")
        ws = self._ws_precise
        off = (-ws.data_ptr()) % 256
        if out is not None:
            _dev(out, torch.float32); _shape(out, "out", n, HIDDEN)
        emb = out if out is not None else torch.empty((n, HIDDEN), dtype=torch.float32, device=pixels.device)
        hid = torch.empty((n, TOKENS, HIDDEN), dtype=torch.float32, device=pixels.device) if return_hidden else None
        check(load().pg_vit_forward_precise(self._h, _p(pixels), _PIXDT[pixels.dtype], n, _p(emb), _p(hid),
                                            C.c_void_p(ws.data_ptr() + off), ws.numel() - off, _stream()), "pg_vit_forward_precise")
        return (emb, hid) if return_hidden else emb

    def fingerprint(self):
        out = (C.c_uint64 * 2)()
        check(load().pg_vit_fingerprint(self._h, out), "pg_vit_fingerprint")
        return int(out[0]), int(out[1])

    def graph(self, on: Optional[bool] = None):
        r, c = C.c_int64(), C.c_int64()
        check(load().pg_vit_graph(self._h, -1 if on is None else int(bool(on)), C.byref(r), C.byref(c)), "pg_vit_graph")
        return int(r.value), int(c.value)

    def profile_enable(self, on: bool = True, classes=None):
        v = 1 if on else 0
        if on and classes is not None:
            v = 0
            for c in classes:
                v |= 1 << (_lib.PROF_CLASSES.index(c) + 1)
        check(load().pg_vit_profile_enable(self._h, v), "pg_vit_profile_enable")

    def profile_reset(self):
        check(load().pg_vit_profile_reset(self._h), "pg_vit_profile_reset")

    def profile_read(self):
        n = len(_lib.PROF_CLASSES)
        launches = (C.c_int64 * n)()
        ms = (C.c_double * n)()
        check(load().pg_vit_profile_read(self._h, launches, ms), "pg_vit_profile_read")
        return {name: (int(launches[i]), float(ms[i])) for i, name in enumerate(_lib.PROF_CLASSES)}

    def saturation_check(self, on: bool = True):
        check(load().pg_vit_saturation_check(self._h, 1 if on else 0), "pg_vit_saturation_check")

    def saturation_read(self, reset: bool = True) -> int:
        n = C.c_int64()
        check(load().pg_vit_saturation_read(self._h, C.byref(n), 1 if reset else 0), "pg_vit_saturation_read")
        return int(n.value)

    def range_alarm_read(self, reset: bool = True) -> int:
        n = C.c_int64()
        check(load().pg_vit_range_alarm_read(self._h, C.byref(n), 1 if reset else 0), "pg_vit_range_alarm_read")
        return int(n.value)

    def close(self):
        if getattr(self, "_h", None) is not None and self._h.value:
            load().pg_vit_destroy(self._h)
            self._h = C.c_void_p()

    def __del__(self):
        try:
            self.close()
        except Exception:
            pass


def head_forward(emb: torch.Tensor, W: torch.Tensor, bias: torch.Tensor, centroids: torch.Tensor, k: int):
    _dev(emb, torch.float32); _dev(W, torch.float32); _dev(bias, torch.float32); _dev(centroids, torch.float64)
    if emb.dim() not in (2, 3):
        raise _lib.PigeonHipError(f"emb must be (B,{HIDDEN}) or (B,P,{HIDDEN}), got {tuple(emb.shape)}")
    B = emb.shape[0]
    P = emb.shape[1] if emb.dim() == 3 else 1
    _shape(emb, "emb", *((B, P, HIDDEN) if emb.dim() == 3 else (B, HIDDEN)))
    Cn = W.shape[0]
    _shape(W, "W", Cn, HIDDEN); _shape(bias, "bias", Cn); _shape(centroids, "centroids", Cn, 2)
    if not 1 <= int(k) <= Cn:
        raise _lib.PigeonHipError(f"head: k = {k} candidates of {Cn} geocells")
    dev = emb.device
    logits = torch.empty((B, Cn), dtype=torch.float32, device=dev)
    tv = torch.empty((B, k), dtype=torch.float32, device=dev)
    ti = torch.empty((B, k), dtype=torch.int64, device=dev)
    am = torch.empty((B,), dtype=torch.int64, device=dev)
    llh = torch.empty((B, 2), dtype=torch.float64, device=dev)
    check(load().pg_head_forward(_p(emb), B, P, _p(W), _p(bias), _p(centroids), Cn, k, _p(logits), _p(tv), _p(ti),
                                 _p(am), _p(llh), _stream()), "pg_head_forward")
    return dict(logits=logits, topk_values=tv, topk_indices=ti, preds_geocell=am, preds_LLH=llh)


def head_margin(logits: torch.Tensor, emb: torch.Tensor, W: torch.Tensor):
    _dev(logits, torch.float32); _dev(emb, torch.float32); _dev(W, torch.float32)
    B, Cn = logits.shape
    P = emb.shape[1] if emb.dim() == 3 else 1
    _shape(emb, "emb", *((B, P, HIDDEN) if emb.dim() == 3 else (B, HIDDEN)))
    _shape(W, "W", Cn, HIDDEN)
    margin = torch.empty((B,), dtype=torch.float32, device=logits.device)
    sens = torch.empty((B,), dtype=torch.float32, device=logits.device)
    top2 = torch.empty((B,), dtype=torch.int64, device=logits.device)
    check(load().pg_head_margin(_p(logits), B, Cn, _p(emb), P, _p(W), _p(margin), _p(sens), _p(top2), _stream()), "pg_head_margin")
    return margin, sens, top2


def head_certainty(logits: torch.Tensor, emb: torch.Tensor, W: torch.Tensor, topk_idx: torch.Tensor,
                   drift: Optional[torch.Tensor], wstats: torch.Tensor):
    _dev(logits, torch.float32); _dev(emb, torch.float32); _dev(W, torch.float32); _dev(topk_idx, torch.int64)
    _dev(wstats, torch.float32)
    B, Cn = logits.shape
    P = emb.shape[1] if emb.dim() == 3 else 1
    _shape(emb, "emb", *((B, P, HIDDEN) if emb.dim() == 3 else (B, HIDDEN)))
    _shape(W, "W", Cn, HIDDEN); _shape(topk_idx, "topk_idx", B, None); _shape(wstats, "wstats", 2)
    kx = topk_idx.shape[1]
    if drift is not None:
        _dev(drift, torch.float32); _shape(drift, "drift", HIDDEN)
    dev = logits.device
    tol = torch.empty((B,), dtype=torch.float32, device=dev)
    code = torch.empty((B,), dtype=torch.int32, device=dev)
    margin = torch.empty((B,), dtype=torch.float32, device=dev)
    sens = torch.empty((B,), dtype=torch.float32, device=dev)
    check(load().pg_head_certainty(_p(logits), B, Cn, _p(emb), P, _p(W), _p(topk_idx), kx, _p(drift), _p(wstats), _p(tol), _p(code),
                                   _p(margin), _p(sens), _stream()), "pg_head_certainty")
    return tol, code, margin, sens


def aux_heads_forward(emb: torch.Tensor, W: torch.Tensor, bias: torch.Tensor, n_reg: int, n_climate: int, n_month: int,
                      drift: Optional[torch.Tensor] = None, row_tol: Optional[torch.Tensor] = None):
    _dev(emb, torch.float32); _dev(W, torch.float32); _dev(bias, torch.float32)
    if emb.dim() not in (2, 3):
        raise _lib.PigeonHipError(f"emb must be (B,{HIDDEN}) or (B,P,{HIDDEN}), got {tuple(emb.shape)}")
    B = emb.shape[0]
    P = emb.shape[1] if emb.dim() == 3 else 1
    _shape(emb, "emb", *((B, P, HIDDEN) if emb.dim() == 3 else (B, HIDDEN)))
    n_reg, n_climate, n_month = int(n_reg), int(n_climate), int(n_month)
    if min(n_reg, n_climate, n_month) < 0:
        raise _lib.PigeonHipError(f"aux_heads: negative output count (n_reg={n_reg} n_climate={n_climate} n_month={n_month})")
    A = n_reg + n_climate + n_month
    _shape(W, "W", A, HIDDEN); _shape(bias, "bias", A)
    if drift is not None:
        _dev(drift, torch.float32); _shape(drift, "drift", HIDDEN)
    if row_tol is not None:
        _dev(row_tol, torch.float32); _shape(row_tol, "row_tol", B)
    dev = emb.device
    preds = torch.empty((B, A), dtype=torch.float32, device=dev)
    cls = torch.empty((B, 2), dtype=torch.int64, device=dev)
    tol = torch.empty((B,), dtype=torch.float32, device=dev)
    code = torch.empty((B,), dtype=torch.int32, device=dev)
    check(load().pg_aux_heads_forward(_p(emb), B, P, _p(W), _p(bias), n_reg, n_climate, n_month, _p(drift), _p(preds), _p(cls),
                                      _p(tol), _p(code), _p(row_tol), _stream()), "pg_aux_heads_forward")
    return dict(preds=preds, cls=cls, tol=tol, code=code)


def embedding_debias(emb: torch.Tensor, bias: torch.Tensor) -> torch.Tensor:
    _dev(emb, torch.float32); _dev(bias, torch.float32); _shape(bias, "bias", HIDDEN)
    if emb.dim() < 1 or emb.shape[-1] != HIDDEN or not emb.is_contiguous():
        raise ValueError(f"embedding_debias: emb must be contiguous (..., {HIDDEN}), got {tuple(emb.shape)}")
    n = emb.numel() // HIDDEN
    check(load().pg_embedding_debias(_p(emb), n, HIDDEN, _p(bias), _stream()), "pg_embedding_debias")
    return emb


def fingerprint(t: torch.Tensor, seed: int = 0):
    _dev(t)
    out = (C.c_uint64 * 2)()
    with torch.cuda.device(t.device):
        check(load().pg_fingerprint(_p(t), t.numel() * t.element_size(), C.c_uint64(int(seed) & 0xFFFFFFFFFFFFFFFF), out, _stream()),
              "pg_fingerprint")
    return int(out[0]), int(out[1])


def head_wstats(W: torch.Tensor, drift: Optional[torch.Tensor]) -> torch.Tensor:
    _dev(W, torch.float32); _shape(W, "W", None, HIDDEN)
    if drift is not None:
        _dev(drift, torch.float32); _shape(drift, "drift", HIDDEN)
    out = torch.empty((2,), dtype=torch.float32, device=W.device)
    check(load().pg_head_wstats(_p(W), W.shape[0], _p(drift), _p(out), _stream()), "pg_head_wstats")
    return out


def requeue_append(head_tol: torch.Tensor, refine_tol: Optional[torch.Tensor], refine_code: Optional[torch.Tensor], thr: float,
                   force_all: bool = False, dst_base: int = 0, flushed: int = 0, cap: int = 0,
                   counters: Optional[torch.Tensor] = None, slot_dst: Optional[torch.Tensor] = None):
    _dev(head_tol, torch.float32)
    B = head_tol.numel()
    if refine_tol is not None:
        _dev(refine_tol, torch.float32); _shape(refine_tol, "refine_tol", B)
    if refine_code is not None:
        _dev(refine_code, torch.int32); _shape(refine_code, "refine_code", B)
    dev = head_tol.device
    certain = torch.empty((B,), dtype=torch.uint8, device=dev)
    cause = torch.empty((B,), dtype=torch.int32, device=dev)
    row_slot = None
    if cap > 0:
        _dev(counters, torch.int64); _shape(counters, "counters", 2)
        _dev(slot_dst, torch.int64); _shape(slot_dst, "slot_dst", cap)
        row_slot = torch.empty((B,), dtype=torch.int32, device=dev)
    check(load().pg_requeue_append(_p(head_tol), _p(refine_tol), _p(refine_code), B, float(thr), 1 if force_all else 0, int(dst_base),
                                   int(flushed), int(cap), _p(counters), _p(slot_dst), _p(row_slot), _p(certain), _p(cause), _stream()),
          "pg_requeue_append")
    return certain, cause, row_slot


def rows_to_slots(src: torch.Tensor, row_slot: torch.Tensor, dst: torch.Tensor) -> None:
    _dev(src); _dev(dst); _dev(row_slot, torch.int32)
    if src.dtype != dst.dtype or tuple(src.shape[1:]) != tuple(dst.shape[1:]):
# ... 253 lines not shown
```

Measured before the change: 2533.

## Fuse rowstat finalize into the residual GEMM tail via arrival counters

Adds a seam path for the residual-plus-row-statistics GEMM. The tail kernel, which takes the last rows or all rows, now finalizes the per-row LayerNorm statistics itself, using per-strip arrival counters once every column tile of a strip has landed. This removes the separate rowstat_finalize launch and its re-read of statpart. The planner can also force a tail split where it would not cut before. The cost is atomic counters that must reset correctly across graph replays, plus extra work in the tail kernel.

```diff
diff --git a/include/pigeon_hip.h b/include/pigeon_hip.h
--- a/include/pigeon_hip.h
+++ b/include/pigeon_hip.h
@@ -71,12 +71,15 @@
 int pg_tune_gemm_raster(int gn);
 int pg_tune_gemm_mid(int on);
 int pg_gemm_plan(int variant, int epi, int M, int N, int K, int* kernel, int* rows_main, int* rest);
+int pg_tune_gemm_seam(int on);
+int pg_gemm_seam_plan(int variant, int M, int N, int K, int* kernel, int* rows_main, int* seam);
 int pg_tune_exact_attention(int use_f32_mfma);
 int pg_tune_exact_products(int n);
 int pg_tune_exact_fusion(int on);
 int pg_vit_saturation_check(pg_vit* h, int on);
 int pg_vit_saturation_read(pg_vit* h, int64_t* count, int reset);
 int pg_vit_range_alarm_read(pg_vit* h, int64_t* rows, int reset);
+int pg_vit_seam_pending(pg_vit* h, int64_t* nonzero);
 
 int pg_head_forward(const float* emb, int B, int P, const float* W, const float* bias,
                     const double* centroids, int C, int k, float* logits,
@@ -191,6 +194,9 @@
 int pg_op_gemm16_resid_stat(int dtype, const void* A, int64_t lda, const void* W, int64_t ldw, const float* bias, float* X,
                             int64_t ldc, void* x16, int64_t ldx, float* statpart, int M, int N, int K, int variant, void* stream);
 int pg_op_rowstat_finalize(const float* statpart, int slots, float* rowstat, int64_t rows, float eps, void* stream);
+int pg_op_gemm16_resid_stat_seam(int dtype, const void* A, int64_t lda, const void* W, int64_t ldw, const float* bias, float* X,
+                                 int64_t ldc, void* x16, int64_t ldx, float* statpart, float* rowstat, float eps, void* alarm,
+                                 float alarm_sumsq, void* arrive, int M, int N, int K, int variant, int all_tail, void* stream);
 int pg_op_gemm16_ln(int dtype, const void* A, int64_t lda, const void* W, int64_t ldw, const float* bias, const float* colsum,
                     const float* rowstat, void* out, int64_t ldc, int M, int N, int K, int epi, float qscale, int qcols,
                     int variant, void* stream);
diff --git a/pigeon_amd/_lib.py b/pigeon_amd/_lib.py
--- a/pigeon_amd/_lib.py
+++ b/pigeon_amd/_lib.py
@@ -66,6 +66,9 @@
     "pg_tune_gemm_tail_shape": (_I, [_I, _I]),
     "pg_tune_gemm_raster": (_I, [_I]),
     "pg_tune_gemm_mid": (_I, [_I]),
+    "pg_tune_gemm_seam": (_I, [_I]),
+    "pg_gemm_seam_plan": (_I, [_I, _I, _I, _I, _P, _P, _P]),
+    "pg_vit_seam_pending": (_I, [_P, C.POINTER(_I64)]),
     "pg_tune_exact_attention": (_I, [_I]),
     "pg_tune_exact_products": (_I, [_I]),
     "pg_tune_exact_fusion": (_I, [_I]),
@@ -115,6 +118,7 @@
     "pg_op_rowstat_cast": (_I, [_P, _P, _I, _P, _I64, _F, _P]),
     "pg_op_gemm16_resid_stat": (_I, [_I, _P, _I64, _P, _I64, _P, _P, _I64, _P, _I64, _P, _I, _I, _I, _I, _P]),
     "pg_op_rowstat_finalize": (_I, [_P, _I, _P, _I64, _F, _P]),
+    "pg_op_gemm16_resid_stat_seam": (_I, [_I, _P, _I64, _P, _I64, _P, _P, _I64, _P, _I64, _P, _P, _F, _P, _F, _P, _I, _I, _I, _I, _I, _P]),
     "pg_op_gemm16_ln": (_I, [_I, _P, _I64, _P, _I64, _P, _P, _P, _P, _I64, _I, _I, _I, _I, _F, _I, _I, _P]),
     "pg_op_layernorm": (_I, [_P, _P, _P, _P, _I, _I64, _F, _P]),
     "pg_op_attention": (_I, [_I, _P, _P, _I, _P]),
diff --git a/pigeon_amd/csrc/abi.hip b/pigeon_amd/csrc/abi.hip
--- a/pigeon_amd/csrc/abi.hip
+++ b/pigeon_amd/csrc/abi.hip
@@ -52,6 +52,14 @@
     PgGemmExtra ex; ex.x16 = x16; ex.ldx = ldx; ex.statpart = statpart;
     return pg_gemm_launch(dtype, A, lda, W, ldw, bias, X, ldc, M, N, K, EPI_RESID_STAT, 1.f, 0, nullptr, variant ? variant : PG_GEMM_V_PP,
                           (hipStream_t)stream, &ex);
+}
+extern "C" int pg_op_gemm16_resid_stat_seam(int dtype, const void* A, int64_t lda, const void* W, int64_t ldw, const float* bias, float* X,
+                                            int64_t ldc, void* x16, int64_t ldx, float* statpart, float* rowstat, float eps, void* alarm,
+                                            float alarm_sumsq, void* arrive, int M, int N, int K, int variant, int all_tail, void* stream) {
+    if (!A || !W || !X || !x16 || !statpart || !rowstat || !arrive) { pg_set_error("op_gemm16_resid_stat_seam: null argument"); return PG_EINVAL; }
+    PgGemmExtra ex; ex.x16 = x16; ex.ldx = ldx; ex.statpart = statpart;
+    return pg_gemm_resid_stat_launch(dtype, A, lda, W, ldw, bias, X, ldc, M, N, K, variant ? variant : PG_GEMM_V_PP, (hipStream_t)stream, ex,
+                                     rowstat, eps, (unsigned long long*)alarm, alarm_sumsq, (unsigned*)arrive, all_tail != 0);
 }
 extern "C" int pg_op_gemm16_ln(int dtype, const void* A, int64_t lda, const void* W, int64_t ldw, const float* bias,
                                const float* colsum, const float* rowstat, void* out, int64_t ldc, int M, int N, int K, int epi,
diff --git a/pigeon_amd/csrc/gemm_device.h b/pigeon_amd/csrc/gemm_device.h
--- a/pigeon_amd/csrc/gemm_device.h
+++ b/pigeon_amd/csrc/gemm_device.h
@@ -28,6 +28,9 @@
 int pg_gemm_pp6_launch(int dtype, GemmArgs g, int epi, hipStream_t s);
 bool pg_gemm_tail_supported(int epi, int N, int K);
 int pg_gemm_tail_launch(int dtype, GemmArgs g, int epi, int m_begin, hipStream_t s);
+bool pg_gemm_seam_supported(int N, int K);
+int pg_gemm_seam_launch(int dtype, GemmArgs g, int m_begin, float* rowstat, float eps, unsigned long long* alarm, float alarm_sumsq,
+                        unsigned* arrive, hipStream_t s);
 bool pg_gemm_mid_supported(int epi, int N, int K);
 int pg_gemm_mid_launch(int dtype, GemmArgs g, int epi, hipStream_t s, int m_begin = 0);
 
diff --git a/pigeon_amd/csrc/gemm_plan.hip b/pigeon_amd/csrc/gemm_plan.hip
--- a/pigeon_amd/csrc/gemm_plan.hip
+++ b/pigeon_amd/csrc/gemm_plan.hip
@@ -97,6 +97,17 @@
 static bool route_pp256() { return mid_on() && g_gemm_mid != 2; }
 extern "C" int pg_tune_gemm_mid(int on) {
     g_gemm_mid = on == 2 ? 2 : (on ? 1 : 0); ++g_tune_epoch;
+    return PG_OK;
+}
+
+#ifndef PG_DEFAULT_GEMM_SEAM
+#define PG_DEFAULT_GEMM_SEAM 3
+#endif
+static int g_gemm_seam = -1;
+static int seam_mask() { if (g_gemm_seam < 0) g_gemm_seam = env_knob("PIGEON_GEMM_SEAM", PG_DEFAULT_GEMM_SEAM) & 3; return g_gemm_seam; }
+extern "C" int pg_tune_gemm_seam(int on) {
+    if (on < 0 || on > 3) { pg_set_error("tune_gemm_seam: 0 (off), 1 (merge an existing tail), 2 (cut where the plan does not), 3 (both)"); return PG_EINVAL; }
+    g_gemm_seam = on; ++g_tune_epoch;
     return PG_OK;
 }
 
@@ -222,7 +233,7 @@
     return t_mid < t_own ? PG_GK_MID : own;
 }
 
-static bool tail_split(int own, int epi, int M, int N, int K, GemmPlan& p) {
+static bool tail_split(int own, int epi, int M, int N, int K, GemmPlan& p, bool force_tail = false) {
     const int tail_max = tail_rows();
     if (tail_max <= 0) return false;
     const bool six = own == PG_GK_PP6;
@@ -240,9 +251,9 @@
                                : kt * ROUND_US_KT_PP + (resid ? ROUND_EPI_PP_RESID : ROUND_EPI_PP);
     const int64_t tiles_m = (int64_t)((M - m_main + 127) / 128) * (N / 128);
     const double t_mid = (double)((tiles_m + ncu - 1) / ncu) * (kt * SMALL_MID_US_KT + (resid ? TAIL_MID_EPI_RESID : TAIL_MID_EPI)) + TAIL_MID_LAUNCH_US;
-    const bool cut = K >= tail_min_k() || N >= tail_min_n();
-    const bool by_mid = cut && mid_on() && pg_gemm_mid_supported(epi, N, K) && t_mid < TAIL_US && t_mid < t_round;
-    const bool by_tail = cut && !by_mid && pg_gemm_tail_supported(epi, N, K);
+    const bool cut = force_tail || K >= tail_min_k() || N >= tail_min_n();
+    const bool by_mid = cut && !force_tail && mid_on() && pg_gemm_mid_supported(epi, N, K) && t_mid < TAIL_US && t_mid < t_round;
+    const bool by_tail = cut && !by_mid && (force_tail ? pg_gemm_seam_supported(N, K) : pg_gemm_tail_supported(epi, N, K));
     if (!by_mid && !by_tail) return false;
     p.rows = (int)m_main;
     p.rest = by_mid ? PG_GK_MID : PG_GK_TAIL;
@@ -320,40 +331,108 @@
     }
 }
 
-int pg_gemm_launch(int dtype, const void* A, int64_t lda, const void* W, int64_t ldw, const float* bias, void* out, int64_t ldc,
-                   int M, int N, int K, int epi, float qscale, int qcols, const float* aux, int variant,
-                   hipStream_t s, const PgGemmExtra* extra) {
-    if (M <= 0) return PG_OK;
+static GemmArgs gemm_args(const void* A, int64_t lda, const void* W, int64_t ldw, const float* bias, void* out, int64_t ldc, int M, int N, int K,
+                          float qscale, int qcols, const float* aux, const PgGemmExtra* extra) {
     GemmArgs g;
     g.A = (const uint16_t*)A; g.lda = lda; g.W = (const uint16_t*)W; g.ldw = ldw > 0 ? ldw : K; g.bias = bias; g.out = out; g.ldc = ldc;
     g.M = M; g.N = N; g.K = K; g.qscale = qscale; g.qcols = qcols; g.aux = aux;
     g.tilesM = 0; g.tilesN = 0; g.ntiles = 0; g.part_tiles = 0; g.gn = 0; g.stagger = 0; g.xcd_stagger_ticks = 0;
     if (extra) g.ex = *extra;
+    return g;
+}
+static int gemm_check(const GemmArgs& g, int dtype, int epi) {
+    const int N = g.N, K = g.K;
+    if ((epi == EPI_GELU || epi == EPI_RESID || epi >= EPI_RESID_STAT) && !g.bias) { pg_set_error("gemm: epilogue %d needs a bias", epi); return PG_EINVAL; }
+    if (epi == EPI_RESID_STAT && (!g.ex.x16 || !g.ex.statpart || g.ex.ldx != g.ldc)) { pg_set_error("gemm: EPI_RESID_STAT needs x16 / statpart and ldx == ldc"); return PG_EINVAL; }
+    if (epi_is_ln(epi) && (!g.ex.colsum || !g.ex.rowstat)) { pg_set_error("gemm: LN epilogue needs colsum / rowstat"); return PG_EINVAL; }
+    if (epi == EPI_PATCH && !g.aux) { pg_set_error("gemm: patch epilogue needs aux"); return PG_EINVAL; }
+    if (epi == EPI_GELU_X3 && (g.ldc != 3 * (int64_t)N || dtype != PG_DTYPE_F16 || N % 256 != 0 || K % 128 != 0)) {
+        pg_set_error("gemm: EPI_GELU_X3 writes the fp16 triple [M][3N]: ldc == 3 N, fp16 operands, N %% 256 == 0, K %% 128 == 0 (ldc=%lld N=%d K=%d)",
+                     (long long)g.ldc, N, K);
+        return PG_EINVAL;
+    }
+    if ((g.lda % 8) || (g.ldc % 8) || (g.qcols % 8) || (g.ldw % 8) || g.ldw < K) { pg_set_error("gemm: lda/ldw/ldc/qcols must be multiples of 8, ldw >= K"); return PG_EINVAL; }
+    return PG_OK;
+}
+static void gemm_args_planned(GemmArgs& g, const GemmPlan& p, int epi) {
+    g.xcd_stagger_ticks = p.stagger_ticks;
+    if (g.ex.stat_rows <= 0) g.ex.stat_rows = g.M;
+#ifdef PIGEON_PROBES
+    if (g_dbg_ts && epi != EPI_PATCH) { g.aux = (const float*)g_dbg_ts; g.stagger = -7; }
+#endif
+}
+
+int pg_gemm_launch(int dtype, const void* A, int64_t lda, const void* W, int64_t ldw, const float* bias, void* out, int64_t ldc,
+                   int M, int N, int K, int epi, float qscale, int qcols, const float* aux, int variant,
+                   hipStream_t s, const PgGemmExtra* extra) {
+    if (M <= 0) return PG_OK;
+    GemmArgs g = gemm_args(A, lda, W, ldw, bias, out, ldc, M, N, K, qscale, qcols, aux, extra);
     if (g.ex.parts > 1) {
         if (epi != EPI_F32 || N % 256 != 0 || K % 128 != 0) { pg_set_error("gemm: parts > 1 needs EPI_F32, N %% 256 == 0, K %% 128 == 0"); return PG_EINVAL; }
         return pg_gemm_pp_launch(dtype, g, epi, PG_GEMM_V_PP, s);
     }
-    if ((epi == EPI_GELU || epi == EPI_RESID || epi >= EPI_RESID_STAT) && !bias) { pg_set_error("gemm: epilogue %d needs a bias", epi); return PG_EINVAL; }
-    if (epi == EPI_RESID_STAT && (!g.ex.x16 || !g.ex.statpart || g.ex.ldx != ldc)) { pg_set_error("gemm: EPI_RESID_STAT needs x16 / statpart and ldx == ldc"); return PG_EINVAL; }
-    if (epi_is_ln(epi) && (!g.ex.colsum || !g.ex.rowstat)) { pg_set_error("gemm: LN epilogue needs colsum / rowstat"); return PG_EINVAL; }
-    if (epi == EPI_PATCH && !aux) { pg_set_error("gemm: patch epilogue needs aux"); return PG_EINVAL; }
-    if (epi == EPI_GELU_X3 && (ldc != 3 * (int64_t)N || dtype != PG_DTYPE_F16 || N % 256 != 0 || K % 128 != 0)) {
-        pg_set_error("gemm: EPI_GELU_X3 writes the fp16 triple [M][3N]: ldc == 3 N, fp16 operands, N %% 256 == 0, K %% 128 == 0 (ldc=%lld N=%d K=%d)",
-                     (long long)ldc, N, K);
-        return PG_EINVAL;
-    }
-    if ((lda % 8) || (ldc % 8) || (qcols % 8) || (g.ldw % 8) || g.ldw < K) { pg_set_error("gemm: lda/ldw/ldc/qcols must be multiples of 8, ldw >= K"); return PG_EINVAL; }
+    if (int rc = gemm_check(g, dtype, epi)) return rc;
     GemmPlan p;
     const int rc = gemm_plan(variant, epi, M, N, K, p);
     if (rc != PG_OK) return rc;
-    g.xcd_stagger_ticks = p.stagger_ticks;
-    if (g.ex.stat_rows <= 0) g.ex.stat_rows = M;
-#ifdef PIGEON_PROBES
-    if (g_dbg_ts && epi != EPI_PATCH) { g.aux = (const float*)g_dbg_ts; g.stagger = -7; }
-#endif
+    gemm_args_planned(g, p, epi);
     GemmArgs gm = g;
     gm.M = p.rows;
     const int rc_main = launch_one(p.kernel, p.variant, dtype, gm, epi, 0, s);
     if (rc_main != PG_OK || p.rest == PG_GK_NONE) return rc_main;
     return launch_one(p.rest, 0, dtype, g, epi, p.rows, s);
 }
+
+static bool seam_plan(int variant, int M, int N, int K, bool all_tail, GemmPlan& p) {
+    if (gemm_plan(variant, EPI_RESID_STAT, M, N, K, p) != PG_OK) return false;
+    if (!pg_gemm_seam_supported(N, K)) return false;
+    bool seam = false;
+    int rows = p.rows;
+    if (all_tail) { seam = true; rows = 0; }
+    else if (p.kernel == PG_GK_PP6 || p.kernel == PG_GK_PP) {
+        const int mask = seam_mask();
+        if (p.rest == PG_GK_TAIL) seam = (mask & 1) != 0;
+        else if (mask & 2) {
+            GemmPlan q = p;
+            const int bm = p.kernel == PG_GK_PP6 ? 384 : 256;
+            const int64_t ntiles = (int64_t)((M + bm - 1) / bm) * (N / 256);
+            if (tail_split(p.kernel, EPI_RESID_STAT, M, N, K, q, true)) { seam = true; rows = q.rows; }
+            else if (ntiles < pg_gemm_grid_cus() && M <= tail_rows()) { seam = true; rows = 0; }
+        }
+    }
+    if (!seam || M - rows > PG_SEAM_MAX_ROWS) return false;
+    p.rows = rows; p.rest = PG_GK_TAIL;
+    return true;
+}
+extern "C" int pg_gemm_seam_plan(int variant, int M, int N, int K, int* kernel, int* rows_main, int* seam) {
+    if (!kernel || !rows_main || !seam || M <= 0 || N <= 0 || K <= 0) { pg_set_error("gemm_seam_plan: bad argument"); return PG_EINVAL; }
+    GemmPlan p;
+    *seam = seam_plan(variant, M, N, K, false, p) ? 1 : 0;
+    if (!*seam) { const int rc = gemm_plan(variant, EPI_RESID_STAT, M, N, K, p); if (rc != PG_OK) return rc; }
+    *kernel = p.kernel; *rows_main = p.rows;
+    return PG_OK;
+}
+
+int pg_gemm_resid_stat_launch(int dtype, const void* A, int64_t lda, const void* W, int64_t ldw, const float* bias, float* X, int64_t ldc,
+                              int M, int N, int K, int variant, hipStream_t s, const PgGemmExtra& ex, float* rowstat, float eps,
+                              unsigned long long* alarm, float alarm_sumsq, unsigned* arrive, bool all_tail) {
+    if (M <= 0) return PG_OK;
+    GemmPlan p;
+    if (!rowstat || N % 64 != 0) { pg_set_error("gemm_resid_stat: rowstat missing or N %% 64 != 0"); return PG_EINVAL; }
+    if (!arrive || !seam_plan(variant, M, N, K, all_tail, p)) {
+        if (all_tail) { pg_set_error("gemm_resid_stat: the seam launch does not take M=%d N=%d K=%d", M, N, K); return PG_EINVAL; }
+        if (int rc = pg_gemm_launch(dtype, A, lda, W, ldw, bias, X, ldc, M, N, K, EPI_RESID_STAT, 1.f, 0, nullptr, variant, s, &ex)) return rc;
+        return pg_rowstat_finalize_launch(ex.statpart, N / 64, rowstat, M, eps, s, alarm, alarm_sumsq);
+    }
+    GemmArgs g = gemm_args(A, lda, W, ldw, bias, X, ldc, M, N, K, 1.f, 0, nullptr, &ex);
+    if (g.ex.parts > 1) { pg_set_error("gemm_resid_stat: one product per launch"); return PG_EINVAL; }
+    if (int rc = gemm_check(g, dtype, EPI_RESID_STAT)) return rc;
+    if (g.ex.stat_rows > 0 && g.ex.stat_rows != M) { pg_set_error("gemm_resid_stat: the finalize reads statpart with stat_rows == M"); return PG_EINVAL; }
+    gemm_args_planned(g, p, EPI_RESID_STAT);
+    if (p.rows > 0) {
+        GemmArgs gm = g;
+        gm.M = p.rows;
+        if (int rc = launch_one(p.kernel, p.variant, dtype, gm, EPI_RESID_STAT, 0, s)) return rc;
+    }
+    return pg_gemm_seam_launch(dtype, g, p.rows, rowstat, eps, alarm, alarm_sumsq, arrive, s);
+}
diff --git a/pigeon_amd/csrc/gemm_tail.hip b/pigeon_amd/csrc/gemm_tail.hip
--- a/pigeon_amd/csrc/gemm_tail.hip
+++ b/pigeon_amd/csrc/gemm_tail.hip
@@ -1,4 +1,5 @@
 #include "gemm_epi.h"
+#include "rowstat.h"
 
 namespace {
 
@@ -16,17 +17,18 @@
     for (int j = 0; j < 4; ++j) f.b[j] = __builtin_bit_cast(typename T::v8, __builtin_amdgcn_raw_buffer_load_b128(rw, vw[j], kbytes, 0));
 }
 
-template <typename T, int EPI>
-__global__ __launch_bounds__(64) void gemm_tail_kernel(GemmArgs g, int m_begin) {
-    __shared__ __attribute__((aligned(16))) float slab[TL_BM * EPI_SLAB_ROWPF];
-    const int lane = threadIdx.x;
-    int tn, tm;
+__device__ __forceinline__ void tail_tile_coords(const GemmArgs& g, unsigned bid, int& tn, int& tm) {
     if (g.tilesN % 8 == 0) {
-        const int xcd = blockIdx.x & 7, idx = blockIdx.x >> 3, per = g.tilesN >> 3;
+        const int xcd = bid & 7, idx = bid >> 3, per = g.tilesN >> 3;
         tn = xcd + 8 * (idx % per); tm = idx / per;
     } else {
-        tn = blockIdx.x % g.tilesN; tm = blockIdx.x / g.tilesN;
-    }
+        tn = bid % g.tilesN; tm = bid / g.tilesN;
+    }
+}
+
+template <typename T, int EPI, int DEPTH = TL_DEPTH>
+__device__ __forceinline__ void tail_tile(const GemmArgs& g, int m_begin, int tm, int tn, float* slab) {
+    const int lane = threadIdx.x;
     const int row0 = m_begin + tm * TL_BM, col0 = tn * TL_BN;
     const int l15 = lane & 15, lq = lane >> 4;
     const int rows = min(TL_BM, g.M - row0);
@@ -39,9 +41,9 @@
     for (int j = 0; j < 4; ++j) vw[j] = (j * 16 + l15) * (int)g.ldw * 2 + lq * 16;
 
     const int nks = g.K / 32;
-    FragTL<T> fr[TL_DEPTH];
-#pragma unroll
-    for (int d = 0; d < TL_DEPTH; ++d) {
+    FragTL<T> fr[DEPTH];
+#pragma unroll
+    for (int d = 0; d < DEPTH; ++d) {
         load_frag_tl<T>(fr[d], ra, rw, va, vw, d * 64);
         __builtin_amdgcn_sched_barrier(0);
     }
@@ -50,14 +52,14 @@
     for (int i = 0; i < 2; ++i)
 #pragma unroll
         for (int j = 0; j < 4; ++j) acc[i][j] = f32x4{0.f, 0.f, 0.f, 0.f};
-    for (int ks = 0; ks < nks; ks += TL_DEPTH) {
-#pragma unroll
-        for (int d = 0; d < TL_DEPTH; ++d) {
+    for (int ks = 0; ks < nks; ks += DEPTH) {
+#pragma unroll
+        for (int d = 0; d < DEPTH; ++d) {
 #pragma unroll
             for (int i = 0; i < 2; ++i)
 #pragma unroll
                 for (int j = 0; j < 4; ++j) acc[i][j] = T::mfma16(fr[d].b[j], fr[d].a[i], acc[i][j]);
-            const int kn = min(ks + d + TL_DEPTH, nks - 1);
+            const int kn = min(ks + d + DEPTH, nks - 1);
             load_frag_tl<T>(fr[d], ra, rw, va, vw, kn * 64);
             __builtin_amdgcn_sched_barrier(0);
         }
@@ -126,6 +128,56 @@
 }
 
 template <typename T, int EPI>
+__global__ __launch_bounds__(64) void gemm_tail_kernel(GemmArgs g, int m_begin) {
+    __shared__ __attribute__((aligned(16))) float slab[TL_BM * EPI_SLAB_ROWPF];
+    int tn, tm;
+    tail_tile_coords(g, blockIdx.x, tn, tm);
+    tail_tile<T, EPI>(g, m_begin, tm, tn, slab);
+}
+
+struct SeamArgs {
+    float* rowstat;
+    float eps;
+    unsigned long long* alarm;
+    float alarm_sumsq;
+    unsigned* arrive;
+    int tail_blocks;
+};
+
+constexpr int SEAM_FIN_ROWS = 4;
+
+template <typename T, int DEPTH>
+__global__ __launch_bounds__(64) void gemm_seam_kernel(GemmArgs g, int m_begin, SeamArgs f) {
+    __shared__ __attribute__((aligned(16))) float slab[TL_BM * EPI_SLAB_ROWPF];
+    const int lane = threadIdx.x;
+    const int slots = g.tilesN;
+    if ((int)blockIdx.x >= f.tail_blocks) {
+        const int64_t row0 = (int64_t)((int)blockIdx.x - f.tail_blocks) * (64 * SEAM_FIN_ROWS) + lane;
+        if (slots == 16) {
+            rowstat_finalize_rows16<SEAM_FIN_ROWS>(g.ex.statpart, g.ex.stat_rows, row0, 64, m_begin, f.rowstat, f.eps, f.alarm, f.alarm_sumsq);
+        } else {
+            for (int r = 0; r < SEAM_FIN_ROWS; ++r)
+                if (row0 + r * 64 < m_begin)
+                    rowstat_finalize_row(g.ex.statpart, slots, g.ex.stat_rows, row0 + r * 64, f.rowstat, f.eps, f.alarm, f.alarm_sumsq);
+        }
+        return;
+    }
+    int tn, tm;
+    tail_tile_coords(g, blockIdx.x, tn, tm);
+    tail_tile<T, EPI_RESID_STAT, DEPTH>(g, m_begin, tm, tn, slab);
+    __syncthreads();
+    __threadfence();
+    unsigned arrived = 0;
+    if (lane == 0) arrived = atomicAdd(f.arrive + tm, 1u);
+    arrived = (unsigned)__builtin_amdgcn_readfirstlane((int)arrived);
+    if (arrived != (unsigned)(slots - 1)) return;
+    if (lane == 0) atomicExch(f.arrive + tm, 0u);
+    __threadfence();
+    const int64_t row = (int64_t)m_begin + tm * TL_BM + lane;
+    if (lane < TL_BM && row < g.M) rowstat_finalize_row(g.ex.statpart, slots, g.ex.stat_rows, row, f.rowstat, f.eps, f.alarm, f.alarm_sumsq);
+}
+
+template <typename T, int EPI>
 int launch_tail(const GemmArgs& g, int m_begin, int nblk, hipStream_t s) {
     hipLaunchKernelGGL((gemm_tail_kernel<T, EPI>), dim3(nblk), dim3(64), 0, s, g, m_begin);
     return pg_check_launch("gemm_tail");
@@ -163,3 +215,28 @@
     pg_set_error("gemm_tail: operand dtype must be PG_DTYPE_F16 or PG_DTYPE_BF16 (got %d)", dtype);
     return PG_EINVAL;
 }
+
+bool pg_gemm_seam_supported(int N, int K) { return N % TL_BN == 0 && K % 128 == 0; }
+
+int pg_gemm_seam_launch(int dtype, GemmArgs g, int m_begin, float* rowstat, float eps, unsigned long long* alarm, float alarm_sumsq,
+                        unsigned* arrive, hipStream_t s) {
+    if (!pg_gemm_seam_supported(g.N, g.K)) { pg_set_error("gemm_seam: unsupported shape (N=%d K=%d)", g.N, g.K); return PG_EINVAL; }
+    if (!rowstat || !arrive || !g.ex.statpart || !g.ex.x16 || g.ex.stat_rows < g.M) { pg_set_error("gemm_seam: bad argument"); return PG_EINVAL; }
+    if (m_begin < 0 || m_begin >= g.M || g.M - m_begin > PG_SEAM_MAX_ROWS) {
+        pg_set_error("gemm_seam: tail rows [%d, %d) out of range (at most %d)", m_begin, g.M, PG_SEAM_MAX_ROWS);
+        return PG_EINVAL;
+    }
+    if (int rc = pg_gemm_panel_check("gemm_seam", g.lda, g.ldw, TL_BM, TL_BN)) return rc;
+    g.tilesM = (g.M - m_begin + TL_BM - 1) / TL_BM;
+    g.tilesN = g.N / TL_BN;
+    g.ntiles = g.tilesM * g.tilesN;
+    const SeamArgs f = {rowstat, eps, alarm, alarm_sumsq, arrive, g.ntiles};
+    const dim3 grid((unsigned)(g.ntiles + (m_begin + 64 * SEAM_FIN_ROWS - 1) / (64 * SEAM_FIN_ROWS))), block(64);
+    const bool deep = g.K % (32 * TL_DEPTH) == 0;
+    if (dtype == PG_DTYPE_F16 && deep) hipLaunchKernelGGL((gemm_seam_kernel<T_F16, TL_DEPTH>), grid, block, 0, s, g, m_begin, f);
+    else if (dtype == PG_DTYPE_F16) hipLaunchKernelGGL((gemm_seam_kernel<T_F16, 4>), grid, block, 0, s, g, m_begin, f);
+    else if (dtype == PG_DTYPE_BF16 && deep) hipLaunchKernelGGL((gemm_seam_kernel<T_BF16, TL_DEPTH>), grid, block, 0, s, g, m_begin, f);
+    else if (dtype == PG_DTYPE_BF16) hipLaunchKernelGGL((gemm_seam_kernel<T_BF16, 4>), grid, block, 0, s, g, m_begin, f);
+    else { pg_set_error("gemm_seam: operand dtype must be PG_DTYPE_F16 or PG_DTYPE_BF16 (got %d)", dtype); return PG_EINVAL; }
+    return pg_check_launch("gemm_seam");
+}
diff --git a/pigeon_amd/csrc/pigeon_internal.h b/pigeon_amd/csrc/pigeon_internal.h
--- a/pigeon_amd/csrc/pigeon_internal.h
+++ b/pigeon_amd/csrc/pigeon_internal.h
@@ -44,6 +44,11 @@
 int pg_gemm_launch(int dtype, const void* A, int64_t lda, const void* W, int64_t ldw, const float* bias, void* out, int64_t ldc,
                    int M, int N, int K, int epi, float qscale, int qcols, const float* aux, int variant,
                    hipStream_t s, const PgGemmExtra* extra = nullptr);
+#define PG_SEAM_MAX_ROWS 8192
+#define PG_SEAM_STRIPS (PG_SEAM_MAX_ROWS / 32)
+int pg_gemm_resid_stat_launch(int dtype, const void* A, int64_t lda, const void* W, int64_t ldw, const float* bias, float* X, int64_t ldc,
+                              int M, int N, int K, int variant, hipStream_t s, const PgGemmExtra& ex, float* rowstat, float eps,
+                              unsigned long long* alarm, float alarm_sumsq, unsigned* arrive, bool all_tail = false);
 int pg_layernorm_launch(const float* x, const float* gamma, const float* beta, void* y, int out_dtype,
                         int64_t rows, float eps, hipStream_t s);
 int pg_preln_launch(float* x, const float* cls, const float* pos0, const float* gamma, const float* beta,
diff --git a/pigeon_amd/csrc/rowops.hip b/pigeon_amd/csrc/rowops.hip
--- a/pigeon_amd/csrc/rowops.hip
+++ b/pigeon_amd/csrc/rowops.hip
@@ -1,5 +1,6 @@
 #include "common.h"
 #include "pigeon_internal.h"
+#include "rowstat.h"
 
 template <int OUT>
 __global__ __launch_bounds__(256) void layernorm_kernel(const float* __restrict__ x, const float* __restrict__ gamma,
@@ -167,17 +168,7 @@
                                                                float alarm_sumsq) {
     const int64_t row = (int64_t)blockIdx.x * 256 + threadIdx.x;
     if (row >= rows) return;
-    float s1 = 0.f, s2 = 0.f;
-    for (int i = 0; i < slots; ++i) {
-        const f32x2 v = *(const f32x2*)(part + ((int64_t)i * rows + row) * 2);
-        s1 += v[0]; s2 += v[1];
-    }
-    const float mean = s1 * (1.0f / VIT_HIDDEN);
-    const float var = fmaxf(s2 * (1.0f / VIT_HIDDEN) - mean * mean, 0.f);
-    const float rstd = 1.0f / sqrtf(var + eps);
-    rowstat[2 * row] = rstd;
-    rowstat[2 * row + 1] = mean * rstd;
-    if (alarm && !(s2 < alarm_sumsq)) atomicAdd(alarm, 1ull);
+    rowstat_finalize_row(part, slots, rows, row, rowstat, eps, alarm, alarm_sumsq);
 }
 
 int pg_rowstat_finalize_launch(const float* statpart, int slots, float* rowstat, int64_t rows, float eps, hipStream_t s,
diff --git a/pigeon_amd/csrc/rowstat.h b/pigeon_amd/csrc/rowstat.h
--- /dev/null
+++ b/pigeon_amd/csrc/rowstat.h
@@ -0,0 +1,43 @@
+#pragma once
+#include "common.h"
+
+__device__ __forceinline__ void rowstat_finish(float s1, float s2, int64_t row, float* rowstat, float eps, unsigned long long* alarm,
+                                               float alarm_sumsq) {
+    const float mean = s1 * (1.0f / VIT_HIDDEN);
+    const float var = fmaxf(s2 * (1.0f / VIT_HIDDEN) - mean * mean, 0.f);
+    const float rstd = 1.0f / sqrtf(var + eps);
+    rowstat[2 * row] = rstd;
+    rowstat[2 * row + 1] = mean * rstd;
+    if (alarm && !(s2 < alarm_sumsq)) atomicAdd(alarm, 1ull);
+}
+
+__device__ __forceinline__ void rowstat_finalize_row(const float* part, int slots, int64_t stride_rows, int64_t row, float* rowstat,
+                                                     float eps, unsigned long long* alarm, float alarm_sumsq) {
+    float s1 = 0.f, s2 = 0.f;
+    for (int i = 0; i < slots; ++i) {
+        const f32x2 v = *(const f32x2*)(part + ((int64_t)i * stride_rows + row) * 2);
+        s1 += v[0]; s2 += v[1];
+    }
+    rowstat_finish(s1, s2, row, rowstat, eps, alarm, alarm_sumsq);
+}
+
+template <int R>
+__device__ __forceinline__ void rowstat_finalize_rows16(const float* part, int64_t stride_rows, int64_t row0, int64_t step, int64_t rows_end,
+                                                        float* rowstat, float eps, unsigned long long* alarm, float alarm_sumsq) {
+    f32x2 v[R][16];
+#pragma unroll
+    for (int r = 0; r < R; ++r) {
+        const int64_t row = row0 + r * step < rows_end ? row0 + r * step : rows_end - 1;
+#pragma unroll
+        for (int i = 0; i < 16; ++i) v[r][i] = *(const f32x2*)(part + ((int64_t)i * stride_rows + row) * 2);
+    }
+#pragma unroll
+    for (int r = 0; r < R; ++r) {
+        const int64_t row = row0 + r * step;
+        if (row >= rows_end) continue;
+        float s1 = 0.f, s2 = 0.f;
+#pragma unroll
+        for (int i = 0; i < 16; ++i) { s1 += v[r][i][0]; s2 += v[r][i][1]; }
+        rowstat_finish(s1, s2, row, rowstat, eps, alarm, alarm_sumsq);
+    }
+}
diff --git a/pigeon_amd/csrc/vit.hip b/pigeon_amd/csrc/vit.hip
--- a/pigeon_amd/csrc/vit.hip
+++ b/pigeon_amd/csrc/vit.hip
@@ -17,7 +17,7 @@
 }
 #define SAT(buf, rows, cols, ld) do { if (h->sat_check) RC(pg_count_sat16_launch((buf), (rows), (cols), (ld), dt, h->sat_counter, s)); } while (0)
 
-static int vit_forward_body(pg_vit* h, int n, char* ws, hipStream_t s) {
+static int vit_forward_body(pg_vit* h, int n, char* ws, hipStream_t s, int part) {
     const int64_t M = (int64_t)n * VIT_TOKENS;
     const FastWs w = fast_ws((size_t)M, h->ln_fold);
     float* X = (float*)(ws + w.X);
@@ -36,7 +36,11 @@
     if (h->ln_fold) {
         uint16_t* Xn2 = (uint16_t*)(ws + w.Xn2);
         float *statpart = (float*)(ws + w.statpart), *rsA = (float*)(ws + w.rsA), *rsB = (float*)(ws + w.rsB);
-        const int slots = VIT_HIDDEN / 64;
+        unsigned* arrive = h->seam_arrive + part * PG_SEAM_STRIPS;
+        auto gemm_resid_stat = [&](const void* A, const uint16_t* W, const float* bias, int K, uint16_t* x16, float* rs) -> int {
+            PgGemmExtra ex; ex.x16 = x16; ex.ldx = VIT_HIDDEN; ex.statpart = statpart;
+            return pg_gemm_resid_stat_launch(dt, A, K, W, K, bias, X, D, (int)M, D, K, 0, s, ex, rs, eps, h->range_alarm, h->range_alarm_sumsq, arrive);
+        };
         { ProfScope p(h, s, PROF_LAYERNORM); RC(pg_preln_launch(X, h->cls, h->pos, h->preg, h->preb, M, eps, s, Xn, dt, rsA)); }
         SAT(Xn, M, VIT_HIDDEN, VIT_HIDDEN);
         for (int l = 0; l < h->cfg.layers; ++l) {
@@ -48,19 +52,15 @@
             SAT(big, M, 3 * VIT_HIDDEN, 3 * VIT_HIDDEN);
             { ProfScope p(h, s, PROF_ATTENTION); RC(pg_attention_launch(dt, big, Xn, n, s)); }
             SAT(Xn, M, VIT_HIDDEN, VIT_HIDDEN);
-            { ProfScope p(h, s, PROF_GEMM_OUT); ex = PgGemmExtra(); ex.x16 = Xn2; ex.ldx = VIT_HIDDEN; ex.statpart = statpart;
-              RC(gemm(Xn, L.wo, L.bo, X, D, D, EPI_RESID_STAT, &ex)); }
+            { ProfScope p(h, s, PROF_GEMM_OUT); RC(gemm_resid_stat(Xn, L.wo, L.bo, D, Xn2, rsB)); }
             SAT(Xn2, M, VIT_HIDDEN, VIT_HIDDEN);
-            { ProfScope p(h, s, PROF_LAYERNORM); RC(pg_rowstat_finalize_launch(statpart, slots, rsB, M, eps, s, h->range_alarm, h->range_alarm_sumsq)); }
             { ProfScope p(h, s, PROF_GEMM_FC1); ex = PgGemmExtra(); ex.colsum = L.s1; ex.rowstat = rsB;
               RC(gemm(Xn2, L.w1, L.b1, big, F, D, EPI_GELU_LN, &ex)); }
             SAT(big, M, VIT_MLP, VIT_MLP);
             { ProfScope p(h, s, PROF_GEMM_FC2);
               if (last) RC(gemm(big, L.w2, L.b2, X, D, F, EPI_RESID));
-              else { ex = PgGemmExtra(); ex.x16 = Xn; ex.ldx = VIT_HIDDEN; ex.statpart = statpart;
-                     RC(gemm(big, L.w2, L.b2, X, D, F, EPI_RESID_STAT, &ex)); } }
+              else RC(gemm_resid_stat(big, L.w2, L.b2, F, Xn, rsA)); }
             if (!last) SAT(Xn, M, VIT_HIDDEN, VIT_HIDDEN);
-            if (!last) { ProfScope p(h, s, PROF_LAYERNORM); RC(pg_rowstat_finalize_launch(statpart, slots, rsA, M, eps, s, h->range_alarm, h->range_alarm_sumsq)); }
         }
     } else
     for (int l = 0; l < h->cfg.layers; ++l) {
@@ -93,9 +93,9 @@
     ++h->graph_replays;
     return PG_OK;
 }
-static int vit_forward_body_graphed(pg_vit* h, int n, char* ws, hipStream_t s) {
+static int vit_forward_body_graphed(pg_vit* h, int n, char* ws, hipStream_t s, int part) {
     const bool ok = h->use_graph && !h->prof && !h->sat_check && h->streams == 1;
-    if (!ok) return vit_forward_body(h, n, ws, s);
+    if (!ok) return vit_forward_body(h, n, ws, s, part);
     pg_vit::GraphEntry* ent = nullptr;
     for (auto& e : h->graphs) if (e.ws == ws && e.n == n) { ent = &e; break; }
     if (!ent) {
@@ -114,35 +114,35 @@
         ent->seen = 1;
     }
     if (ent->exec) return graph_replay(h, ent, s);
-    if (ent->seen++ == 0) return vit_forward_body(h, n, ws, s);
+    if (ent->seen++ == 0) return vit_forward_body(h, n, ws, s, part);
     if (!h->capture_stream) PG_HIP(hipStreamCreateWithFlags(&h->capture_stream, hipStreamNonBlocking));
     hipGraph_t graph = nullptr;
     hipError_t e = hipStreamBeginCapture(h->capture_stream, hipStreamCaptureModeThreadLocal);
-    if (e != hipSuccess) { (void)hipGetLastError(); h->use_graph = false; return vit_forward_body(h, n, ws, s); }
-    const int rc = vit_forward_body(h, n, ws, h->capture_stream);
+    if (e != hipSuccess) { (void)hipGetLastError(); h->use_graph = false; return vit_forward_body(h, n, ws, s, part); }
+    const int rc = vit_forward_body(h, n, ws, h->capture_stream, part);
     e = hipStreamEndCapture(h->capture_stream, &graph);
     if (rc != PG_OK || e != hipSuccess || !graph) {
         (void)hipGetLastError();
         if (graph) (void)hipGraphDestroy(graph);
         h->use_graph = false;
-        return vit_forward_body(h, n, ws, s);
+        return vit_forward_body(h, n, ws, s, part);
     }
     hipGraphExec_t exec = nullptr;
     e = hipGraphInstantiate(&exec, graph, nullptr, nullptr, 0);
-    if (e != hipSuccess || !exec) { (void)hipGetLastError(); (void)hipGraphDestroy(graph); h->use_graph = false; return vit_forward_body(h, n, ws, s); }
+    if (e != hipSuccess || !exec) { (void)hipGetLastError(); (void)hipGraphDestroy(graph); h->use_graph = false; return vit_forward_body(h, n, ws, s, part); }
     ent->graph = graph; ent->exec = exec; ent->epoch = pg_tune_epoch();
     if (!ent->done) (void)hipEventCreateWithFlags(&ent->done, hipEventDisableTiming);
     ++h->graph_captures;
     return graph_replay(h, ent, s);
 }
 
-static int vit_forward_chunk(pg_vit* h, const void* pixels, int pix_dtype, int n, float* emb_out, float* hidden_out, char* ws, hipStream_t s) {
+static int vit_forward_chunk(pg_vit* h, const void* pixels, int pix_dtype, int n, float* emb_out, float* hidden_out, char* ws, hipStream_t s, int part) {
     const int64_t M = (int64_t)n * VIT_TOKENS;
     const FastWs w = fast_ws((size_t)M, h->ln_fold);
     float* X = (float*)(ws + w.X);
     uint16_t* big = (uint16_t*)(ws + w.big);
     { ProfScope p(h, s, PROF_IM2COL); RC(pg_im2col_launch(pixels, pix_dtype, big, h->cfg.mma_dtype, n, s)); }
-    RC(vit_forward_body_graphed(h, n, ws, s));
+    RC(vit_forward_body_graphed(h, n, ws, s, part));
     { ProfScope p(h, s, PROF_TOKEN_MEAN); RC(pg_token_mean_launch(X, emb_out, n, s)); }
     if (hidden_out) PG_HIP(hipMemcpyAsync(hidden_out, X, (size_t)M * VIT_HIDDEN * 4, hipMemcpyDeviceToDevice, s));
     return PG_OK;
@@ -155,11 +155,11 @@
     RC(vit_forward_check("vit_forward", h, false, pixels, pix_dtype, n_images, emb_out, workspace, workspace_bytes, (size_t)parts * wsp));
     if (n_images == 0) return PG_OK;
     hipStream_t s = (hipStream_t)stream;
-    auto run_range = [&](int first, int last, char* ws, hipStream_t st) -> int {
+    auto run_range = [&](int first, int last, char* ws, hipStream_t st, int part) -> int {
         for (int s0 = first; s0 < last; s0 += h->cfg.max_chunk) {
             const int n = (last - s0) < h->cfg.max_chunk ? (last - s0) : h->cfg.max_chunk;
             const ChunkIO io = chunk_io(pixels, pix_dtype, emb_out, hidden_out, s0);
-            RC(vit_forward_chunk(h, io.pixels, pix_dtype, n, io.emb, io.hidden, ws, st));
+            RC(vit_forward_chunk(h, io.pixels, pix_dtype, n, io.emb, io.hidden, ws, st, part));
         }
         return PG_OK;
     };
@@ -171,7 +171,7 @@
         for (int i = 0; i < parts && rc == PG_OK; ++i) {
             const int first = i * per, last = (i + 1) * per < n_images ? (i + 1) * per : n_images;
             if (first >= last) continue;
-            rc = run_range(first, last, (char*)workspace + (size_t)i * wsp, i == 0 ? s : h->sx[i - 1]);
+            rc = run_range(first, last, (char*)workspace + (size_t)i * wsp, i == 0 ? s : h->sx[i - 1], i);
         }
         for (int i = 0; i + 1 < parts; ++i) {
             hipError_t e = hipEventRecord(h->ev_join[i], h->sx[i]);
@@ -180,7 +180,7 @@
         }
         return rc;
     }
-    return run_range(0, n_images, (char*)workspace, s);
+    return run_range(0, n_images, (char*)workspace, s, 0);
 }
 
 extern "C" int pg_vit_forward(pg_vit* h, const void* pixels, int pix_dtype, int n_images, float* emb_out, void* workspace, size_t workspace_bytes, void* stream) {
@@ -205,6 +205,20 @@
 extern "C" int pg_vit_range_alarm_read(pg_vit* h, int64_t* rows, int reset) {
     return read_counter(h, h ? h->range_alarm : nullptr, reset, "range_alarm_read", rows);
 }
+extern "C" int pg_vit_seam_pending(pg_vit* h, int64_t* nonzero) {
+    if (!h || !nonzero) { pg_set_error("seam_pending: null argument"); return PG_EINVAL; }
+    *nonzero = 0;
+    if (!h->seam_arrive) return PG_OK;
+    unsigned host[4 * PG_SEAM_STRIPS];
+    int cur = 0; PG_HIP(hipGetDevice(&cur));
+    PG_HIP(hipSetDevice(h->device));
+    hipError_t e = hipDeviceSynchronize();
+    if (e == hipSuccess) e = hipMemcpy(host, h->seam_arrive, sizeof(host), hipMemcpyDeviceToHost);
+    (void)hipSetDevice(cur);
+    if (e != hipSuccess) { pg_set_error("seam_pending: %s", hipGetErrorString(e)); return PG_EHIP; }
+    for (unsigned v : host) *nonzero += v != 0;
+    return PG_OK;
+}
 extern "C" int pg_vit_saturation_check(pg_vit* h, int on) {
     if (!h) { pg_set_error("saturation_check: null handle"); return PG_EINVAL; }
     if (on && !h->sat_counter) {
diff --git a/pigeon_amd/csrc/vit_handle.h b/pigeon_amd/csrc/vit_handle.h
--- a/pigeon_amd/csrc/vit_handle.h
+++ b/pigeon_amd/csrc/vit_handle.h
@@ -33,6 +33,7 @@
     unsigned long long* sat_counter = nullptr;
     unsigned long long* range_alarm = nullptr;
     float range_alarm_sumsq = 0.f;
+    unsigned* seam_arrive = nullptr;
     struct GraphEntry { const void* ws; int n; int seen; hipGraph_t graph; hipGraphExec_t exec; unsigned long long last_use, epoch; hipEvent_t done; };
     std::vector<GraphEntry> graphs;
     bool use_graph = true;
diff --git a/pigeon_amd/csrc/vit_weights.hip b/pigeon_amd/csrc/vit_weights.hip
--- a/pigeon_amd/csrc/vit_weights.hip
+++ b/pigeon_amd/csrc/vit_weights.hip
@@ -46,6 +46,12 @@
         h->allocs.push_back(h->range_alarm);
         PG_HIP(hipMemset(h->range_alarm, 0, sizeof(unsigned long long)));
         h->range_alarm_sumsq = 65504.0f * 65504.0f;
+    }
+    if (h->ln_fold) {
+        PG_HIP(hipSetDevice(device));
+        PG_HIP(hipMalloc((void**)&h->seam_arrive, 4 * PG_SEAM_STRIPS * sizeof(unsigned)));
+        h->allocs.push_back(h->seam_arrive);
+        PG_HIP(hipMemset(h->seam_arrive, 0, 4 * PG_SEAM_STRIPS * sizeof(unsigned)));
     }
     { const char* e = getenv("PIGEON_VIT_GRAPH"); h->use_graph = !(e && e[0] == '0'); }
     { const char* e = getenv("PIGEON_VIT_STREAMS"); h->streams = e ? atoi(e) : PG_DEFAULT_VIT_STREAMS; }
diff --git a/pigeon_amd/hip_ops.py b/pigeon_amd/hip_ops.py
--- a/pigeon_amd/hip_ops.py
+++ b/pigeon_amd/hip_ops.py
@@ -103,6 +103,45 @@
     if Xr is not X:
         X.copy_(Xr)
     return x16, part
+
+
+SEAM_STRIPS = 256
+
+
+def gemm16_resid_stat_seam(A: torch.Tensor, W: torch.Tensor, bias: torch.Tensor, X: torch.Tensor, variant: int = 0, eps: float = 1e-5,
+                           alarm: Optional[torch.Tensor] = None, alarm_sumsq: float = 0.0, arrive: Optional[torch.Tensor] = None,
+                           all_tail: bool = False):
+    M, K = A.shape
+    N = W.shape[0]
+    x16 = torch.empty((M, N), dtype=A.dtype, device=A.device)
+    part = torch.empty((N // 64, M, 2), dtype=torch.float32, device=A.device)
+    rs = torch.empty((M, 2), dtype=torch.float32, device=A.device)
+    if arrive is None:
+        arrive = torch.zeros(SEAM_STRIPS, dtype=torch.int32, device=A.device)
+    if arrive.numel() < SEAM_STRIPS or arrive.dtype != torch.int32 or (alarm is not None and alarm.dtype != torch.int64):
+        raise _lib.PigeonHipError("gemm16_resid_stat_seam: arrive is SEAM_STRIPS int32, alarm one int64")
+    have = X.untyped_storage().nbytes() - X.storage_offset() * X.element_size()
+    Xr = X
+    if have < (M + 384) * X.stride(0) * X.element_size():
+        Xr = torch.zeros((M + 384, N), dtype=X.dtype, device=X.device)[:M]
+        Xr.copy_(X)
+    check(load().pg_op_gemm16_resid_stat_seam(_dt16(A), _p(A), A.stride(0), _p(W), W.stride(0), _p(bias), _p(Xr), Xr.stride(0), _p(x16),
+                                              x16.stride(0), _p(part), _p(rs), float(eps), _p(alarm) if alarm is not None else None,
+                                              float(alarm_sumsq), _p(arrive), M, N, K, variant, 1 if all_tail else 0, _stream()),
+          "pg_op_gemm16_resid_stat_seam")
+    if Xr is not X:
+        X.copy_(Xr)
+    return x16, part, rs
+
+
+def tune_gemm_seam(on: int) -> None:
+    check(load().pg_tune_gemm_seam(int(on)), "pg_tune_gemm_seam")
+
+
+def gemm_seam_plan(M: int, N: int, K: int, variant: int = 0) -> dict:
+    k, r, sm = C.c_int(), C.c_int(), C.c_int()
+    check(load().pg_gemm_seam_plan(int(variant), int(M), int(N), int(K), C.byref(k), C.byref(r), C.byref(sm)), "pg_gemm_seam_plan")
+    return dict(kernel=k.value, rows_main=r.value, seam=bool(sm.value))
 
 
 def rowstat_finalize(part: torch.Tensor, eps: float = 1e-5) -> torch.Tensor:
@@ -510,6 +549,11 @@
         check(load().pg_vit_saturation_read(self._h, C.byref(n), 1 if reset else 0), "pg_vit_saturation_read")
         return int(n.value)
 
+    def seam_pending(self) -> int:
+        n = C.c_int64()
+        check(load().pg_vit_seam_pending(self._h, C.byref(n)), "pg_vit_seam_pending")
+        return int(n.value)
+
     def range_alarm_read(self, reset: bool = True) -> int:
         n = C.c_int64()
         check(load().pg_vit_range_alarm_read(self._h, C.byref(n), 1 if reset else 0), "pg_vit_range_alarm_read")
```

After: 2532. No clear change (-0.1%).
